# ImChouOWO/A-lightweight-Unsupervised-Feature-Extractor-

Hardware: NVIDIA B200
Metric: tracked frames/sec at N=64 boxes; ROIAlign achieved HBM GB/s vs B200 peak (higher is better)
Workload: dtype f32

## Files before the change

### a-lightweight-unsupervised-feature-extractor-_b200/csrc/app_cost_tc.cu

```cuda
#include <cuda_bf16.h>

#include "assoc_cost.cuh"

namespace b200 {
namespace {

constexpr int kRows = 128;
constexpr int kTrackRows = 32;
constexpr int kChunks = cost::kD / 8;
constexpr int kSplitBytes = kChunks * kRows * 16;
constexpr int kImageBytes = 3 * kSplitBytes;
constexpr int kLBO = kRows * 16;
constexpr int kSBO = 8 * 16;
constexpr int kTcSmem = 2 * kImageBytes + 64;

__device__ __forceinline__ void split3(float x, __nv_bfloat16* hi, __nv_bfloat16* mid, __nv_bfloat16* lo) {
    *hi = __float2bfloat16_rn(x);
    const float r1 = __fsub_rn(x, __bfloat162float(*hi));
    *mid = __float2bfloat16_rn(r1);
    const float r2 = __fsub_rn(r1, __bfloat162float(*mid));
    *lo = __float2bfloat16_rn(r2);
}

template <int RB>
__global__ void __launch_bounds__(256)
app_tc_prep_kernel(const float* __restrict__ bank, const int32_t* __restrict__ bank_len, const float* __restrict__ fallback,
                   const float* __restrict__ det, int M, int N, int T, unsigned char* __restrict__ imgA,
                   unsigned char* __restrict__ imgB, int m_tiles, int n_tiles) {
    const int lane = threadIdx.x & 31;
    const long long rowsA = (long long)m_tiles * kRows, rowsB = (long long)n_tiles * RB;
    for (long long item = (long long)blockIdx.x * 8 + (threadIdx.x >> 5); item < rowsA + rowsB; item += (long long)gridDim.x * 8) {
        float4 v = make_float4(0.0f, 0.0f, 0.0f, 0.0f);
        unsigned char* img;
        int row, tile_rows = kRows;
        if (item < rowsA) {
            const int m = (int)(item / kTrackRows), t = (int)(item % kTrackRows);
            img = imgA + (size_t)(item / kRows) * kImageBytes;
            row = (int)(item % kRows);
            if (m < M) {
                const int len = min(bank_len[m], T);
                if (t < len) v = reinterpret_cast<const float4*>(bank + ((size_t)m * T + t) * cost::kD)[lane];
                else if (len <= 0 && fallback && t == 0) v = reinterpret_cast<const float4*>(fallback + (size_t)m * cost::kD)[lane];
            }
        } else {
            const long long j = item - rowsA;
            img = imgB + (size_t)(j / RB) * (3 * kChunks * RB * 16);
            row = (int)(j % RB);
            tile_rows = RB;
            if (j < N) v = reinterpret_cast<const float4*>(det + (size_t)j * cost::kD)[lane];
        }
        v = cost::unit_row(v);
        __nv_bfloat16 h[3][4];
        split3(v.x, &h[0][0], &h[1][0], &h[2][0]);
        split3(v.y, &h[0][1], &h[1][1], &h[2][1]);
        split3(v.z, &h[0][2], &h[1][2], &h[2][2]);
        split3(v.w, &h[0][3], &h[1][3], &h[2][3]);
        unsigned char* dst = img + (size_t)(lane >> 1) * (tile_rows * 16) + (size_t)row * 16 + (lane & 1) * 8;
#pragma unroll
        for (int s = 0; s < 3; ++s)
            *reinterpret_cast<uint2*>(dst + (size_t)s * (kChunks * tile_rows * 16)) = *reinterpret_cast<const uint2*>(&h[s][0]);
    }
}

__device__ __forceinline__ unsigned smem_u32(const void* p) { return (unsigned)__cvta_generic_to_shared(p); }
__device__ __forceinline__ void tc_mbar_init(unsigned bar, unsigned count) {
    asm volatile("mbarrier.init.shared::cta.b64 [%0], %1;\n" ::"r"(bar), "r"(count) : "memory");
}
__device__ __forceinline__ void tc_mbar_expect_tx(unsigned bar, unsigned bytes) {
    asm volatile("mbarrier.arrive.expect_tx.shared::cta.b64 _, [%0], %1;\n" ::"r"(bar), "r"(bytes) : "memory");
}
__device__ __forceinline__ void tc_mbar_wait(unsigned bar, unsigned parity) {
    asm volatile(
        "{\n\t.reg .pred p;\n\t"
        "WAIT_%=:\n\t"
        "mbarrier.try_wait.parity.shared::cta.b64 p, [%0], %1;\n\t"
        "@p bra DONE_%=;\n\t"
        "bra WAIT_%=;\n\t"
        "DONE_%=:\n\t}\n" ::"r"(bar), "r"(parity) : "memory");
}
__device__ __forceinline__ void tc_bulk_load(unsigned dst, const void* src, unsigned bytes, unsigned bar) {
    asm volatile("cp.async.bulk.shared::cluster.global.mbarrier::complete_tx::bytes [%0], [%1], %2, [%3];\n"
                 ::"r"(dst), "l"(src), "r"(bytes), "r"(bar) : "memory");
}
__device__ __forceinline__ unsigned long long umma_desc(unsigned smem_addr, int lbo = kLBO) {
    return (unsigned long long)((smem_addr >> 4) & 0x3fffu) | ((unsigned long long)((lbo >> 4) & 0x3fff) << 16) |
           ((unsigned long long)((kSBO >> 4) & 0x3fff) << 32) | (1ull << 46);
}
constexpr unsigned kIdesc = (1u << 4) | (1u << 7) | (1u << 10) | ((unsigned)(kRows >> 3) << 17) | ((unsigned)(kRows >> 4) << 24);

__global__ void __launch_bounds__(128, 1)
app_tc_kernel(const unsigned char* __restrict__ imgA, const unsigned char* __restrict__ imgB,
              const int32_t* __restrict__ bank_len, int has_fallback, int M, int N, int T, int topk, int topk_mean,
              float* __restrict__ C_app, int ldc) {
    extern __shared__ __align__(128) unsigned char smem[];
    unsigned char* sA = smem;
    unsigned char* sB = smem + kImageBytes;
    const unsigned bar_load = smem_u32(smem + 2 * kImageBytes), bar_mma = bar_load + 8;
    unsigned* tmem_slot = reinterpret_cast<unsigned*>(smem + 2 * kImageBytes + 16);
    const int warp = threadIdx.x >> 5, lane = threadIdx.x & 31;
    const int tile_n = blockIdx.x, tile_m = blockIdx.y;

    if (warp == 0) {
        asm volatile("tcgen05.alloc.cta_group::1.sync.aligned.shared::cta.b32 [%0], %1;\n" ::"r"(smem_u32(tmem_slot)), "r"(128u) : "memory");
        asm volatile("tcgen05.relinquish_alloc_permit.cta_group::1.sync.aligned;\n" ::: "memory");
    }
    if (threadIdx.x == 32) {
        tc_mbar_init(bar_load, 1);
        tc_mbar_init(bar_mma, 1);
        asm volatile("fence.mbarrier_init.release.cluster;\n" ::: "memory");
    }
    asm volatile("tcgen05.fence::before_thread_sync;\n" ::: "memory");
    __syncthreads();
    asm volatile("tcgen05.fence::after_thread_sync;\n" ::: "memory");
    const unsigned tmem = *tmem_slot;

    if (threadIdx.x == 0) {
        tc_mbar_expect_tx(bar_load, 2u * kImageBytes);
        tc_bulk_load(smem_u32(sA), imgA + (size_t)tile_m * kImageBytes, kImageBytes, bar_load);
        tc_bulk_load(smem_u32(sB), imgB + (size_t)tile_n * kImageBytes, kImageBytes, bar_load);
        tc_mbar_wait(bar_load, 0);
        asm volatile("tcgen05.fence::after_thread_sync;\n" ::: "memory");
        const int pa[6] = {2, 0, 1, 1, 0, 0}, pb[6] = {0, 2, 1, 0, 1, 0};
        unsigned accumulate = 0;
#pragma unroll
        for (int p = 0; p < 6; ++p) {
            const unsigned a0 = smem_u32(sA) + pa[p] * kSplitBytes, b0 = smem_u32(sB) + pb[p] * kSplitBytes;
#pragma unroll
            for (int ks = 0; ks < kChunks / 2; ++ks) {
                const unsigned long long da = umma_desc(a0 + ks * 2 * kLBO), db = umma_desc(b0 + ks * 2 * kLBO);
                asm volatile(
                    "{\n\t.reg .pred p;\n\t"
                    "setp.ne.b32 p, %4, 0;\n\t"
                    "tcgen05.mma.cta_group::1.kind::f16 [%0], %1, %2, %3, p;\n\t}\n"
                    ::"r"(tmem), "l"(da), "l"(db), "r"(kIdesc), "r"(accumulate) : "memory");
                accumulate = 1;
            }
        }
        asm volatile("tcgen05.commit.cta_group::1.mbarrier::arrive::one.shared::cluster.b64 [%0];\n" ::"r"(bar_mma) : "memory");
    }
    __syncwarp();
    tc_mbar_wait(bar_mma, 0);
    asm volatile("tcgen05.fence::after_thread_sync;\n" ::: "memory");

    const int m = tile_m * (kRows / kTrackRows) + warp;
    int len = 0;
    if (m < M) {
        len = min(bank_len[m], T);
        if (len <= 0 && has_fallback) len = 1;
    }
    const int kk = topk_mean ? min(topk, len) : min(1, len);
    const float kNegInf = -__int_as_float(0x7f800000);
    float* tile = reinterpret_cast<float*>(smem) + warp * (32 * 33);
    for (int c0 = 0; c0 < kRows; c0 += 32) {
        unsigned r[32];
        const unsigned taddr = tmem + ((unsigned)(warp * 32) << 16) + (unsigned)c0;
        asm volatile(
            "tcgen05.ld.sync.aligned.32x32b.x32.b32"
            "{%0, %1, %2, %3, %4, %5, %6, %7, %8, %9, %10, %11, %12, %13, %14, %15,"
            " %16, %17, %18, %19, %20, %21, %22, %23, %24, %25, %26, %27, %28, %29, %30, %31}, [%32];\n"
            : "=r"(r[0]), "=r"(r[1]), "=r"(r[2]), "=r"(r[3]), "=r"(r[4]), "=r"(r[5]), "=r"(r[6]), "=r"(r[7]), "=r"(r[8]),
              "=r"(r[9]), "=r"(r[10]), "=r"(r[11]), "=r"(r[12]), "=r"(r[13]), "=r"(r[14]), "=r"(r[15]), "=r"(r[16]),
              "=r"(r[17]), "=r"(r[18]), "=r"(r[19]), "=r"(r[20]), "=r"(r[21]), "=r"(r[22]), "=r"(r[23]), "=r"(r[24]),
              "=r"(r[25]), "=r"(r[26]), "=r"(r[27]), "=r"(r[28]), "=r"(r[29]), "=r"(r[30]), "=r"(r[31])
            : "r"(taddr)
            : "memory");
        asm volatile("tcgen05.wait::ld.sync.aligned;\n" ::: "memory");
        __syncwarp();
#pragma unroll
        for (int j = 0; j < 32; ++j) tile[lane * 33 + j] = __uint_as_float(r[j]);
        __syncwarp();
        float c = 1.0f;
        if (kk > 0 && kk <= 5) {
            float t0 = kNegInf, t1 = kNegInf, t2 = kNegInf, t3 = kNegInf, t4 = kNegInf;
#pragma unroll
            for (int t = 0; t < 32; ++t) {
                float x = t < len ? tile[t * 33 + lane] : kNegInf;
                float hi;
                hi = fmaxf(t0, x); x = fminf(t0, x); t0 = hi;
                hi = fmaxf(t1, x); x = fminf(t1, x); t1 = hi;
                hi = fmaxf(t2, x); x = fminf(t2, x); t2 = hi;
                hi = fmaxf(t3, x); x = fminf(t3, x); t3 = hi;
                t4 = fmaxf(t4, x);
            }
            float sum = t0;
            if (kk > 1) sum = __fadd_rn(sum, t1);
            if (kk > 2) sum = __fadd_rn(sum, t2);
            if (kk > 3) sum = __fadd_rn(sum, t3);
            if (kk > 4) sum = __fadd_rn(sum, t4);
            c = __fsub_rn(1.0f, __fdiv_rn(sum, (float)kk));
        } else if (kk > 5) {
            unsigned taken = 0u;
            float sum = 0.0f;
            for (int q = 0; q < kk; ++q) {
                float best = kNegInf;
                int arg = 0;
                for (int t = 0; t < len; ++t) {
                    const float x = tile[t * 33 + lane];
                    if (!((taken >> t) & 1u) && x > best) { best = x; arg = t; }
                }
                taken |= 1u << arg;
                sum = __fadd_rn(sum, best);
            }
            c = __fsub_rn(1.0f, __fdiv_rn(sum, (float)kk));
        }
        const int n = tile_n * kRows + c0 + lane;
        if (m < M && n < N) C_app[(size_t)m * ldc + n] = c;
    }
    asm volatile("tcgen05.fence::before_thread_sync;\n" ::: "memory");
    __syncthreads();
    if (warp == 0) asm volatile("tcgen05.dealloc.cta_group::1.sync.aligned.b32 %0, %1;\n" ::"r"(tmem), "r"(128u) : "memory");
}

constexpr int kWalkCols = 64;
constexpr int kWalkLBO = kWalkCols * 16;
constexpr int kWalkSplitBytes = kChunks * kWalkCols * 16;
constexpr int kWalkImageBytes = 3 * kWalkSplitBytes;
constexpr int kWalkEpiWarps = 8;
constexpr int kWalkThreads = (kWalkEpiWarps + 1) * 32;
constexpr int kWalkScratch = kWalkEpiWarps * 32 * 33 * 4;
constexpr int kWalkSmem = kImageBytes + 2 * kWalkImageBytes + kWalkScratch + 96;
constexpr unsigned kIdescWalk = (1u << 4) | (1u << 7) | (1u << 10) | ((unsigned)(kWalkCols >> 3) << 17) | ((unsigned)(kRows >> 4) << 24);

__device__ __forceinline__ void tc_mbar_arrive(unsigned bar) {
    asm volatile("mbarrier.arrive.shared::cta.b64 _, [%0];\n" ::"r"(bar) : "memory");
}

__global__ void __launch_bounds__(kWalkThreads, 1)
app_tc_walk_kernel(const unsigned char* __restrict__ imgA, const unsigned char* __restrict__ imgB,
                   const int32_t* __restrict__ bank_len, int has_fallback, int M, int N, int T, int topk, int topk_mean,
                   float* __restrict__ C_app, int ldc, int n_steps) {
    extern __shared__ __align__(128) unsigned char smem[];
    unsigned char* sA = smem;
    unsigned char* sB = smem + kImageBytes;
    float* scratch = reinterpret_cast<float*>(smem + kImageBytes + 2 * kWalkImageBytes);
    const unsigned bar0 = smem_u32(smem + kImageBytes + 2 * kWalkImageBytes + kWalkScratch);
    unsigned* tmem_slot = reinterpret_cast<unsigned*>(smem + kImageBytes + 2 * kWalkImageBytes + kWalkScratch + 72);
    unsigned rank, nrank;
    asm volatile("mov.u32 %0, %%cluster_ctarank;" : "=r"(rank));
    asm volatile("mov.u32 %0, %%cluster_nctarank;" : "=r"(nrank));
    const unsigned short cta_mask = (unsigned short)((1u << nrank) - 1u);

    const int tid = threadIdx.x, warp = tid >> 5, lane = tid & 31;
    const int tile_m = blockIdx.x;
    const int first_tile = (int)((unsigned)tile_m / nrank) % n_steps;

    if (warp == 0) {
        asm volatile("tcgen05.alloc.cta_group::1.sync.aligned.shared::cta.b32 [%0], %1;\n" ::"r"(smem_u32(tmem_slot)), "r"(128u) : "memory");
        asm volatile("tcgen05.relinquish_alloc_permit.cta_group::1.sync.aligned;\n" ::: "memory");
    }
    if (tid == 32) {
        tc_mbar_init(bar0, 1);
        tc_mbar_init(bar0 + 8, 1); tc_mbar_init(bar0 + 16, 1);
        tc_mbar_init(bar0 + 24, 1); tc_mbar_init(bar0 + 32, 1);
        tc_mbar_init(bar0 + 40, kWalkEpiWarps); tc_mbar_init(bar0 + 48, kWalkEpiWarps);
        tc_mbar_init(bar0 + 56, nrank); tc_mbar_init(bar0 + 64, nrank);
        asm volatile("fence.mbarrier_init.release.cluster;\n" ::: "memory");
    }
    asm volatile("tcgen05.fence::before_thread_sync;\n" ::: "memory");
    __syncthreads();
    if (nrank > 1)
        asm volatile("barrier.cluster.arrive.release.aligned;\n\tbarrier.cluster.wait.acquire.aligned;" ::: "memory");
    asm volatile("tcgen05.fence::after_thread_sync;\n" ::: "memory");
    const unsigned tmem = *tmem_slot;

    if (warp == kWalkEpiWarps) {
        const bool leader = lane == 0;
        const unsigned tm = __shfl_sync(0xffffffffu, tmem, 0);
        auto load_b = [&](int step) {
            const int buf = step & 1;
            const int tile_n = (first_tile + step) % n_steps;
            tc_mbar_expect_tx(bar0 + 8 + 8 * buf, (unsigned)kWalkImageBytes);
            if (nrank > 1) {
                const unsigned part = (unsigned)kWalkImageBytes / nrank;
                const unsigned dst = smem_u32(sB + buf * kWalkImageBytes) + rank * part;
                const unsigned char* src = imgB + (size_t)tile_n * kWalkImageBytes + (size_t)rank * part;
                asm volatile("cp.async.bulk.shared::cluster.global.mbarrier::complete_tx::bytes.multicast::cluster [%0], [%1], %2, [%3], %4;\n"
                             ::"r"(dst), "l"(src), "r"(part), "r"(bar0 + 8 + 8 * buf), "h"(cta_mask) : "memory");
            } else {
                tc_bulk_load(smem_u32(sB + buf * kWalkImageBytes), imgB + (size_t)tile_n * kWalkImageBytes, kWalkImageBytes,
                             bar0 + 8 + 8 * buf);
            }
        };
        if (leader) {
            tc_mbar_expect_tx(bar0, (unsigned)kImageBytes);
            tc_bulk_load(smem_u32(sA), imgA + (size_t)tile_m * kImageBytes, kImageBytes, bar0);
            load_b(0);
            if (n_steps > 1) load_b(1);
        }
        __syncwarp();
        tc_mbar_wait(bar0, 0);
        const unsigned long long dA = umma_desc(smem_u32(sA));
        for (int step = 0; step < n_steps; ++step) {
            const int buf = step & 1;
            const unsigned use = (unsigned)((step >> 1) & 1);
            if (step >= 2) tc_mbar_wait(bar0 + 40 + 8 * buf, use ^ 1u);
            tc_mbar_wait(bar0 + 8 + 8 * buf, use);
            asm volatile("tcgen05.fence::after_thread_sync;\n" ::: "memory");
            const int pa[6] = {2, 0, 1, 1, 0, 0}, pb[6] = {0, 2, 1, 0, 1, 0};
            const unsigned acc = tm + (unsigned)(buf * kWalkCols);
            const unsigned long long dB = umma_desc(smem_u32(sB + buf * kWalkImageBytes), kWalkLBO);
            if (leader) {
                unsigned accumulate = 0;
#pragma unroll
                for (int p = 0; p < 6; ++p) {
#pragma unroll
                    for (int ks = 0; ks < kChunks / 2; ++ks) {
                        const unsigned long long da = dA + (unsigned long long)((pa[p] * kSplitBytes + ks * 2 * kLBO) >> 4);
                        const unsigned long long db = dB + (unsigned long long)((pb[p] * kWalkSplitBytes + ks * 2 * kWalkLBO) >> 4);
                        asm volatile(
                            "{\n\t.reg .pred p;\n\t"
                            "setp.ne.b32 p, %4, 0;\n\t"
                            "tcgen05.mma.cta_group::1.kind::f16 [%0], %1, %2, %3, p;\n\t}\n"
                            ::"r"(acc), "l"(da), "l"(db), "r"(kIdescWalk), "r"(accumulate) : "memory");
                        accumulate = 1;
                    }
                }
                asm volatile("tcgen05.commit.cta_group::1.mbarrier::arrive::one.shared::cluster.b64 [%0];\n"
                             ::"r"(bar0 + 24 + 8 * buf) : "memory");
                if (nrank > 1)
                    asm volatile("tcgen05.commit.cta_group::1.mbarrier::arrive::one.shared::cluster.multicast::cluster.b64 [%0], %1;\n"
                                 ::"r"(bar0 + 56 + 8 * buf), "h"(cta_mask) : "memory");
            }
            __syncwarp();
            if (step >= 1 && step + 1 < n_steps) {
                if (nrank > 1) tc_mbar_wait(bar0 + 56 + 8 * (buf ^ 1), (unsigned)(((step - 1) >> 1) & 1));
                else tc_mbar_wait(bar0 + 24 + 8 * (buf ^ 1), (unsigned)(((step - 1) >> 1) & 1));
                if (leader) load_b(step + 1);
                __syncwarp();
            }
        }
    } else {
        const int q = warp & 3, half = warp >> 2;
        const int m = tile_m * (kRows / kTrackRows) + q;
        int len = 0;
        if (m < M) {
            len = min(bank_len[m], T);
            if (len <= 0 && has_fallback) len = 1;
        }
        const int kk = topk_mean ? min(topk, len) : min(1, len);
        const float kNegInf = -__int_as_float(0x7f800000);
        float* tile = scratch + warp * (32 * 33);
        for (int step = 0; step < n_steps; ++step) {
            const int buf = step & 1;
            tc_mbar_wait(bar0 + 24 + 8 * buf, (unsigned)((step >> 1) & 1));
            asm volatile("tcgen05.fence::after_thread_sync;\n" ::: "memory");
            unsigned r[32];
            const unsigned taddr = tmem + ((unsigned)(q * 32) << 16) + (unsigned)(buf * kWalkCols + half * 32);
            asm volatile(
                "tcgen05.ld.sync.aligned.32x32b.x32.b32"
                "{%0, %1, %2, %3, %4, %5, %6, %7, %8, %9, %10, %11, %12, %13, %14, %15,"
                " %16, %17, %18, %19, %20, %21, %22, %23, %24, %25, %26, %27, %28, %29, %30, %31}, [%32];\n"
                : "=r"(r[0]), "=r"(r[1]), "=r"(r[2]), "=r"(r[3]), "=r"(r[4]), "=r"(r[5]), "=r"(r[6]), "=r"(r[7]), "=r"(r[8]),
                  "=r"(r[9]), "=r"(r[10]), "=r"(r[11]), "=r"(r[12]), "=r"(r[13]), "=r"(r[14]), "=r"(r[15]), "=r"(r[16]),
                  "=r"(r[17]), "=r"(r[18]), "=r"(r[19]), "=r"(r[20]), "=r"(r[21]), "=r"(r[22]), "=r"(r[23]), "=r"(r[24]),
                  "=r"(r[25]), "=r"(r[26]), "=r"(r[27]), "=r"(r[28]), "=r"(r[29]), "=r"(r[30]), "=r"(r[31])
                : "r"(taddr)
                : "memory");
            asm volatile("tcgen05.wait::ld.sync.aligned;\n" ::: "memory");
            asm volatile("tcgen05.fence::before_thread_sync;\n" ::: "memory");
            __syncwarp();
            if (lane == 0) tc_mbar_arrive(bar0 + 40 + 8 * buf);
#pragma unroll
            for (int j = 0; j < 32; ++j) tile[lane * 33 + j] = __uint_as_float(r[j]);
            __syncwarp();
            float c = 1.0f;
            if (kk > 0 && kk <= 5) {
                float t0 = kNegInf, t1 = kNegInf, t2 = kNegInf, t3 = kNegInf, t4 = kNegInf;
#pragma unroll
                for (int t = 0; t < 32; ++t) {
                    float x = t < len ? tile[t * 33 + lane] : kNegInf;
                    float hi;
                    hi = fmaxf(t0, x); x = fminf(t0, x); t0 = hi;
                    hi = fmaxf(t1, x); x = fminf(t1, x); t1 = hi;
                    hi = fmaxf(t2, x); x = fminf(t2, x); t2 = hi;
                    hi = fmaxf(t3, x); x = fminf(t3, x); t3 = hi;
                    t4 = fmaxf(t4, x);
                }
                float sum = t0;
                if (kk > 1) sum = __fadd_rn(sum, t1);
                if (kk > 2) sum = __fadd_rn(sum, t2);
                if (kk > 3) sum = __fadd_rn(sum, t3);
                if (kk > 4) sum = __fadd_rn(sum, t4);
                c = __fsub_rn(1.0f, __fdiv_rn(sum, (float)kk));
            } else if (kk > 5) {
                unsigned taken = 0u;
                float sum = 0.0f;
                for (int qq = 0; qq < kk; ++qq) {
                    float best = kNegInf;
                    int arg = 0;
                    for (int t = 0; t < len; ++t) {
                        const float x = tile[t * 33 + lane];
                        if (!((taken >> t) & 1u) && x > best) { best = x; arg = t; }
                    }
                    taken |= 1u << arg;
                    sum = __fadd_rn(sum, best);
                }
                c = __fsub_rn(1.0f, __fdiv_rn(sum, (float)kk));
            }
            const int n = ((first_tile + step) % n_steps) * kWalkCols + half * 32 + lane;
            if (m < M && n < N) C_app[(size_t)m * ldc + n] = c;
        }
    }
    asm volatile("tcgen05.fence::before_thread_sync;\n" ::: "memory");
    __syncthreads();
    if (nrank > 1)
        asm volatile("barrier.cluster.arrive.release.aligned;\n\tbarrier.cluster.wait.acquire.aligned;" ::: "memory");
    if (warp == 0) asm volatile("tcgen05.dealloc.cta_group::1.sync.aligned.b32 %0, %1;\n" ::"r"(tmem), "r"(128u) : "memory");
}

}

int app_cost_tc(const float* bank, const int32_t* bank_len, const float* fallback, const float* det, int M, int N, int T,
                int topk, int use_topk_mean, float* C_app, int ldc, cudaStream_t st) {
    if (T > kTrackRows || (long long)M * N < 64 * 64) return 1;
    static bool configured[64];
    int dev = 0;
    if (cudaGetDevice(&dev) != cudaSuccess || dev < 0 || dev >= 64) dev = 0;
    if (!configured[dev]) {
        B200_CUDA(cudaFuncSetAttribute(app_tc_kernel, cudaFuncAttributeMaxDynamicSharedMemorySize, kTcSmem));
        B200_CUDA(cudaFuncSetAttribute(app_tc_walk_kernel, cudaFuncAttributeMaxDynamicSharedMemorySize, kWalkSmem));
        configured[dev] = true;
    }
    const int m_tiles = (M * kTrackRows + kRows - 1) / kRows;
    bool walk = m_tiles >= 100;
    if (const char* e = getenv("B200TRACK_TC_KERNEL")) walk = atoi(e) == 2;
    const int rb = walk ? kWalkCols : kRows;
    const int n_tiles = (N + rb - 1) / rb;
    const size_t imgB_bytes = (size_t)n_tiles * (walk ? kWalkImageBytes : kImageBytes);
    cudaMemPool_t pool = nullptr;
    int rc = scratch_pool(&pool);
    if (rc) return rc;
    unsigned char* img = nullptr;
    B200_CUDA(cudaMallocFromPoolAsync(reinterpret_cast<void**>(&img), (size_t)m_tiles * kImageBytes + imgB_bytes, pool, st));
    unsigned char* imgA = img;
    unsigned char* imgB = img + (size_t)m_tiles * kImageBytes;
    const long long rows = (long long)m_tiles * kRows + (long long)n_tiles * rb;
    const unsigned blocks = (unsigned)((rows + 7) / 8 < 148 * 8 ? (rows + 7) / 8 : 148 * 8);
    if (walk) app_tc_prep_kernel<kWalkCols><<<blocks, 256, 0, st>>>(bank, bank_len, fallback, det, M, N, T, imgA, imgB, m_tiles, n_tiles);
    else app_tc_prep_kernel<kRows><<<blocks, 256, 0, st>>>(bank, bank_len, fallback, det, M, N, T, imgA, imgB, m_tiles, n_tiles);
    rc = check_launch("app_tc_prep_kernel");
    if (rc == B200_OK) {
        if (walk) {
            int cl = 1;
            if (const char* e = getenv("B200TRACK_TC_CLUSTER")) cl = (atoi(e) == 2 && m_tiles % 2 == 0) ? 2 : 1;
            cudaLaunchConfig_t cfg = {};
            cfg.gridDim = dim3((unsigned)m_tiles);
            cfg.blockDim = dim3(kWalkThreads);
            cfg.dynamicSmemBytes = kWalkSmem;
            cfg.stream = st;
            cudaLaunchAttribute attr[1];
            attr[0].id = cudaLaunchAttributeClusterDimension;
            attr[0].val.clusterDim.x = cl; attr[0].val.clusterDim.y = 1; attr[0].val.clusterDim.z = 1;
            cfg.attrs = attr;
            cfg.numAttrs = 1;
            (void)cudaLaunchKernelEx(&cfg, app_tc_walk_kernel, (const unsigned char*)imgA, (const unsigned char*)imgB, bank_len,
                                     (int)(fallback != nullptr), M, N, T, topk, use_topk_mean, C_app, ldc, n_tiles);
            rc = check_launch("app_tc_walk_kernel");
        } else {
            app_tc_kernel<<<dim3(n_tiles, m_tiles), 128, kTcSmem, st>>>(imgA, imgB, bank_len, fallback != nullptr, M, N, T, topk,
                                                                       use_topk_mean, C_app, ldc);
            rc = check_launch("app_tc_kernel");
        }
    }
    B200_CUDA(cudaFreeAsync(img, st));
    return rc;
}

}
```

### a-lightweight-unsupervised-feature-extractor-_b200/csrc/common.cuh

```cuda
#pragma once
#include <cuda_runtime.h>
#include <stdint.h>
#include <stdio.h>

#include <atomic>

#include "b200track.h"

namespace b200 {

extern thread_local char g_err[512];
extern std::atomic<int64_t> g_launches;

int fail(int code, const char* fmt, ...);
int scratch_pool(cudaMemPool_t* out);

inline int check_launch(const char* what) {
    g_launches.fetch_add(1, std::memory_order_relaxed);
    cudaError_t e = cudaGetLastError();
    if (e != cudaSuccess) return fail(B200_ECUDA, "%s: %s", what, cudaGetErrorString(e));
    return B200_OK;
}

#define B200_CUDA(expr)                                                                  \
    do {                                                                                 \
        cudaError_t _e = (expr);                                                         \
        if (_e != cudaSuccess)                                                           \
            return ::b200::fail(B200_ECUDA, "%s: %s", #expr, cudaGetErrorString(_e));    \
    } while (0)

#define B200_REQUIRE(cond, ...)                                                          \
    do {                                                                                 \
        if (!(cond)) return ::b200::fail(B200_EINVAL, __VA_ARGS__);                      \
    } while (0)

inline cudaStream_t as_stream(void* s) { return reinterpret_cast<cudaStream_t>(s); }

constexpr int kWarp = 32;
constexpr int kSMs = 148;

__device__ __forceinline__ float warp_sum(float v) {
#pragma unroll
    for (int o = 16; o > 0; o >>= 1) v += __shfl_xor_sync(0xffffffffu, v, o);
    return v;
}
__device__ __forceinline__ int warp_min(int v) {
#pragma unroll
    for (int o = 16; o > 0; o >>= 1) v = min(v, __shfl_xor_sync(0xffffffffu, v, o));
    return v;
}
__device__ __forceinline__ int warp_max(int v) {
#pragma unroll
    for (int o = 16; o > 0; o >>= 1) v = max(v, __shfl_xor_sync(0xffffffffu, v, o));
    return v;
}


#ifdef B200_TRK_TIMING
static __device__ unsigned long long g_span[128];
__device__ __forceinline__ unsigned long long gtime() {
    unsigned long long t;
    asm volatile("mov.u64 %0, %%globaltimer;" : "=l"(t));
    return t;
}
#define B200_SPAN_BEGIN(k) do { if (threadIdx.x == 0) atomicMin(&::b200::g_span[2 * (k)], ::b200::gtime()); } while (0)
#define B200_SPAN_END(k) do { if (threadIdx.x == 0) atomicMax(&::b200::g_span[2 * (k) + 1], ::b200::gtime()); } while (0)
#define B200_SPAN_GETTER(name)                                                                          \
    extern "C" int name(unsigned long long* out64, int reset) {                                         \
        if (out64 && cudaMemcpyFromSymbol(out64, ::b200::g_span, sizeof(unsigned long long) * 128) != cudaSuccess) return -2; \
        if (reset) {                                                                                    \
            unsigned long long init[128];                                                                \
            for (int i = 0; i < 128; ++i) init[i] = (i & 1) ? 0ull : ~0ull;                              \
            if (cudaMemcpyToSymbol(::b200::g_span, init, sizeof(init)) != cudaSuccess) return -2;       \
        }                                                                                               \
        return 0;                                                                                       \
    }
#else
#define B200_SPAN_GETTER(name)
#define B200_SPAN_BEGIN(k) do { } while (0)
#define B200_SPAN_END(k) do { } while (0)
#endif

}
```

### a-lightweight-unsupervised-feature-extractor-_b200/csrc/kalman.cuh

```cuda
#pragma once
#include "common.cuh"

namespace b200 {
namespace kf {

__device__ __forceinline__ void box_to_z(const double* b, float* z) {
    const double w = fmax(1.0, b[2] - b[0]), h = fmax(1.0, b[3] - b[1]);
    z[0] = (float)(b[0] + 0.5 * w);
    z[1] = (float)(b[1] + 0.5 * h);
    z[2] = (float)(w / h);
    z[3] = (float)h;
}

__device__ __forceinline__ void x_to_box(const double* x, double* b) {
    const double h = fmax(x[3], 1.0), a = fmax(x[2], 1e-3), w = fmax(a * h, 1.0);
    b[0] = x[0] - 0.5 * w;
    b[1] = x[1] - 0.5 * h;
    b[2] = x[0] + 0.5 * w;
    b[3] = x[1] + 0.5 * h;
}

__device__ __forceinline__ void init_state(const double* box, double* x, double* P) {
    float z[4];
    box_to_z(box, z);
#pragma unroll
    for (int i = 0; i < 4; ++i) { x[i] = (double)z[i]; x[i + 4] = 0.0; }
#pragma unroll
    for (int i = 0; i < 64; ++i) P[i] = 0.0;
#pragma unroll
    for (int i = 0; i < 4; ++i) { P[i * 9] = 10.0; P[(i + 4) * 9] = 1000.0; }
}

template <typename TX, typename TP>
__device__ __forceinline__ void predict_t(double* x, double* P, const float* q) {
#pragma unroll
    for (int i = 0; i < 4; ++i) x[i] = (double)((TX)x[i] + (TX)x[i + 4]);
#pragma unroll
    for (int i = 0; i < 4; ++i)
#pragma unroll
        for (int j = 0; j < 8; ++j) P[i * 8 + j] = (double)((TP)P[i * 8 + j] + (TP)P[(i + 4) * 8 + j]);
#pragma unroll
    for (int i = 0; i < 8; ++i)
#pragma unroll
        for (int j = 0; j < 4; ++j) P[i * 8 + j] = (double)((TP)P[i * 8 + j] + (TP)P[i * 8 + j + 4]);
#pragma unroll
    for (int i = 0; i < 8; ++i) P[i * 9] = (double)((TP)P[i * 9] + (TP)q[i]);
}

__device__ __forceinline__ void predict(double* x, double* P, int stage, const float* q) {
    if (stage == 0) predict_t<float, float>(x, P, q);
    else if (stage == 1) predict_t<float, double>(x, P, q);
    else predict_t<double, double>(x, P, q);
}

template <typename T>
__device__ __forceinline__ void inv4(const T* S, T* SI) {
    T a[4][4], b[4][4], rinv[4];
#pragma unroll
    for (int i = 0; i < 4; ++i)
#pragma unroll
        for (int j = 0; j < 4; ++j) { a[i][j] = S[i * 4 + j]; b[i][j] = (i == j) ? (T)1 : (T)0; }
#pragma unroll
    for (int j = 0; j < 4; ++j) {
        int p = j;
        T best = fabs(a[j][j]);
#pragma unroll
        for (int i = j + 1; i < 4; ++i) {
            const T v = fabs(a[i][j]);
            if (v > best) { best = v; p = i; }
        }
#pragma unroll
        for (int i = j + 1; i < 4; ++i)
            if (p == i) {
#pragma unroll
                for (int k = 0; k < 4; ++k) {
                    T t = a[j][k]; a[j][k] = a[i][k]; a[i][k] = t;
                    t = b[j][k]; b[j][k] = b[i][k]; b[i][k] = t;
                }
            }
        rinv[j] = (T)1 / a[j][j];
#pragma unroll
        for (int i = j + 1; i < 4; ++i) {
            a[i][j] *= rinv[j];
#pragma unroll
            for (int k = j + 1; k < 4; ++k) a[i][k] -= a[i][j] * a[j][k];
        }
    }
#pragma unroll
    for (int c = 0; c < 4; ++c) {
#pragma unroll
        for (int i = 1; i < 4; ++i)
#pragma unroll
            for (int k = 0; k < i; ++k) b[i][c] -= a[i][k] * b[k][c];
#pragma unroll
        for (int i = 3; i >= 0; --i) {
#pragma unroll
            for (int k = i + 1; k < 4; ++k) b[i][c] -= a[i][k] * b[k][c];
            b[i][c] *= rinv[i];
        }
    }
#pragma unroll
    for (int i = 0; i < 4; ++i)
#pragma unroll
        for (int j = 0; j < 4; ++j) SI[i * 4 + j] = b[i][j];
}

template <typename A, typename B> struct Promote { using type = double; };
template <> struct Promote<float, float> { using type = float; };

template <typename TX, typename TP>
__device__ __forceinline__ void update_t(double* x, double* P, const float* z, const float* r) {
    using TXN = typename Promote<TX, TP>::type;
    TX y[4];
#pragma unroll
    for (int i = 0; i < 4; ++i) y[i] = (TX)z[i] - (TX)x[i];
    TP S[16], SI[16], K[32];
#pragma unroll
    for (int i = 0; i < 4; ++i)
#pragma unroll
        for (int j = 0; j < 4; ++j) S[i * 4 + j] = (TP)P[i * 8 + j] + (i == j ? (TP)r[i] : (TP)0);
    inv4<TP>(S, SI);
#pragma unroll
    for (int i = 0; i < 8; ++i)
#pragma unroll
        for (int j = 0; j < 4; ++j) {
            TP s = (TP)P[i * 8] * SI[j];
#pragma unroll
            for (int k = 1; k < 4; ++k) s = fma((TP)P[i * 8 + k], SI[k * 4 + j], s);
            K[i * 4 + j] = s;
        }
#pragma unroll
    for (int i = 0; i < 8; ++i) {
        TXN s = (TXN)K[i * 4] * (TXN)y[0];
#pragma unroll
        for (int k = 1; k < 4; ++k) s = fma((TXN)K[i * 4 + k], (TXN)y[k], s);
        x[i] = (double)((TXN)(TX)x[i] + s);
    }
    double ikd[4];
#pragma unroll
    for (int i = 0; i < 4; ++i) ikd[i] = 1.0 - (double)K[i * 4 + i];
#define B200_IK(i, k) ((i) == (k) ? ikd[(k)] : -(double)K[(i) * 4 + (k)])
#pragma unroll
    for (int i = 4; i < 8; ++i)
#pragma unroll
        for (int j = 0; j < 8; ++j) {
            double s = B200_IK(i, 0) * P[j];
#pragma unroll
            for (int k = 1; k < 4; ++k) s = fma(B200_IK(i, k), P[k * 8 + j], s);
            P[i * 8 + j] = s + P[i * 8 + j];
        }
#pragma unroll
    for (int j = 0; j < 8; ++j) {
        const double p0 = P[j], p1 = P[8 + j], p2 = P[16 + j], p3 = P[24 + j];
#pragma unroll
        for (int i = 0; i < 4; ++i)
            P[i * 8 + j] = fma(B200_IK(i, 3), p3, fma(B200_IK(i, 2), p2, fma(B200_IK(i, 1), p1, B200_IK(i, 0) * p0)));
    }
#pragma unroll
    for (int i = 0; i < 8; ++i) {
        const double a0 = P[i * 8], a1 = P[i * 8 + 1], a2 = P[i * 8 + 2], a3 = P[i * 8 + 3];
#pragma unroll
        for (int j = 0; j < 8; ++j) {
            const double s = fma(a3, B200_IK(j, 3), fma(a2, B200_IK(j, 2), fma(a1, B200_IK(j, 1), a0 * B200_IK(j, 0))));
            TP d = (K[i * 4] * (TP)r[0]) * K[j * 4];
#pragma unroll
            for (int k = 1; k < 4; ++k) d = fma(K[i * 4 + k] * (TP)r[k], K[j * 4 + k], d);
            P[i * 8 + j] = (j < 4 ? s : s + P[i * 8 + j]) + (double)d;
        }
    }
#undef B200_IK
}

__device__ __forceinline__ int update(double* x, double* P, int stage, const float* z, const float* r) {
    if (stage == 0) update_t<float, float>(x, P, z, r);
    else if (stage == 1) update_t<float, double>(x, P, z, r);
    else update_t<double, double>(x, P, z, r);
    return stage < 2 ? stage + 1 : 2;
}

struct Gate {
    double SI[16];
    double xs[4];
    int stage;
};

__device__ __forceinline__ void gate_prepare(const double* x, const double* P, int stage, const float* r,
                                             Gate* g) {
    g->stage = stage;
#pragma unroll
    for (int i = 0; i < 4; ++i) g->xs[i] = x[i];
    if (stage == 0) {
        float S[16], SI[16];
#pragma unroll
        for (int i = 0; i < 4; ++i)
#pragma unroll
            for (int j = 0; j < 4; ++j) {
                const float hph = (float)P[i * 8 + j] + (i == j ? r[i] : 0.0f);
                S[i * 4 + j] = hph + (i == j ? 1e-9f : 0.0f);
            }
        inv4<float>(S, SI);
#pragma unroll
        for (int i = 0; i < 16; ++i) g->SI[i] = (double)SI[i];
    } else {
        double S[16];
#pragma unroll
        for (int i = 0; i < 4; ++i)
#pragma unroll
            for (int j = 0; j < 4; ++j) {
                const double hph = P[i * 8 + j] + (i == j ? (double)r[i] : 0.0);
                S[i * 4 + j] = hph + (i == j ? (double)1e-9f : 0.0);
            }
        inv4<double>(S, g->SI);
    }
}

__device__ __forceinline__ double gate_d2(const double* SI, const double* xs, int stage, const float* z) {
    if (stage == 0) {
        float y[4], t[4];
#pragma unroll
        for (int i = 0; i < 4; ++i) y[i] = z[i] - (float)xs[i];
#pragma unroll
        for (int j = 0; j < 4; ++j) {
            float s = y[0] * (float)SI[j];
#pragma unroll
            for (int i = 1; i < 4; ++i) s = fmaf(y[i], (float)SI[i * 4 + j], s);
            t[j] = s;
        }
        float d = t[0] * y[0];
#pragma unroll
        for (int j = 1; j < 4; ++j) d = fmaf(t[j], y[j], d);
        return (double)d;
    }
    double y[4], t[4];
#pragma unroll
    for (int i = 0; i < 4; ++i)
        y[i] = stage == 1 ? (double)(z[i] - (float)xs[i]) : (double)z[i] - xs[i];
#pragma unroll
    for (int j = 0; j < 4; ++j) {
        double s = y[0] * SI[j];
#pragma unroll
        for (int i = 1; i < 4; ++i) s = fma(y[i], SI[i * 4 + j], s);
        t[j] = s;
    }
    double d = t[0] * y[0];
#pragma unroll
    for (int j = 1; j < 4; ++j) d = fma(t[j], y[j], d);
    return d;
}

template <typename TX, typename TP>
__device__ __forceinline__ double update_rows_t(double* gx, double* gP, const float* z, const float* r, double* sP,
                                                double* sK, int i, unsigned mask, int new_stage, bool want_d2) {
    using TXN = typename Promote<TX, TP>::type;
    double Pr[8];
    {
        const double2* p2 = reinterpret_cast<const double2*>(gP + i * 8);
#pragma unroll
        for (int k = 0; k < 4; ++k) { const double2 v = p2[k]; Pr[2 * k] = v.x; Pr[2 * k + 1] = v.y; }
    }
#pragma unroll
    for (int j = 0; j < 8; ++j) sP[i * 8 + j] = Pr[j];
    double xg[4];
#pragma unroll
    for (int k = 0; k < 4; ++k) xg[k] = gx[k];
    const double xi = gx[i];
    __syncwarp(mask);
    TP S[16], SI[16], Kr[4];
#pragma unroll
    for (int a = 0; a < 4; ++a)
#pragma unroll
        for (int b = 0; b < 4; ++b) S[a * 4 + b] = (TP)sP[a * 8 + b] + (a == b ? (TP)r[a] : (TP)0);
    inv4<TP>(S, SI);
#pragma unroll
    for (int j = 0; j < 4; ++j) {
        TP acc = (TP)Pr[0] * SI[j];
#pragma unroll
        for (int k = 1; k < 4; ++k) acc = fma((TP)Pr[k], SI[k * 4 + j], acc);
        Kr[j] = acc;
    }
    TX y[4];
#pragma unroll
    for (int k = 0; k < 4; ++k) y[k] = (TX)z[k] - (TX)xg[k];
    TXN sx = (TXN)Kr[0] * (TXN)y[0];
#pragma unroll
    for (int k = 1; k < 4; ++k) sx = fma((TXN)Kr[k], (TXN)y[k], sx);
    const double xn = (double)((TXN)(TX)xi + sx);
#pragma unroll
    for (int j = 0; j < 4; ++j) sK[i * 4 + j] = (double)Kr[j];
    __syncwarp(mask);
    gx[i] = xn;
    double ik[4], A[8];
#pragma unroll
    for (int k = 0; k < 4; ++k) ik[k] = (i == k) ? 1.0 - (double)Kr[k] : -(double)Kr[k];
#pragma unroll
    for (int j = 0; j < 8; ++j) {
        double a = ik[0] * sP[j];
#pragma unroll
        for (int k = 1; k < 4; ++k) a = fma(ik[k], sP[k * 8 + j], a);
        A[j] = i >= 4 ? a + Pr[j] : a;
    }
    double Pn[8];
#pragma unroll
    for (int j = 0; j < 8; ++j) {
        double ikj[4];
#pragma unroll
        for (int k = 0; k < 4; ++k) ikj[k] = (j == k) ? 1.0 - sK[j * 4 + k] : -sK[j * 4 + k];
        const double b = fma(A[3], ikj[3], fma(A[2], ikj[2], fma(A[1], ikj[1], A[0] * ikj[0])));
        TP dd = (Kr[0] * (TP)r[0]) * (TP)sK[j * 4];
#pragma unroll
        for (int k = 1; k < 4; ++k) dd = fma(Kr[k] * (TP)r[k], (TP)sK[j * 4 + k], dd);
        Pn[j] = (j < 4 ? b : b + A[j]) + (double)dd;
    }
    {
        double2* p2 = reinterpret_cast<double2*>(gP + i * 8);
#pragma unroll
        for (int k = 0; k < 4; ++k) p2[k] = make_double2(Pn[2 * k], Pn[2 * k + 1]);
    }
    if (!want_d2) return 0.0;
    __syncwarp(mask);
    if (i < 4) {
#pragma unroll
        for (int j = 0; j < 4; ++j) sP[i * 8 + j] = Pn[j];
        sK[i] = xn;
    }
    __syncwarp(mask);
    Gate g;
    double x4[4];
#pragma unroll
    for (int k = 0; k < 4; ++k) x4[k] = sK[k];
    gate_prepare(x4, sP, new_stage, r, &g);
    return gate_d2(g.SI, g.xs, new_stage, z);
}

}
}
```

### a-lightweight-unsupervised-feature-extractor-_b200/csrc/roi_align.cu

```cuda
#include <cuda.h>
#include <cuda_fp16.h>

#include "common.cuh"
#include <type_traits>

namespace b200 {
namespace {

#ifndef B200_ROI_WARPS
#define B200_ROI_WARPS 2
#endif
constexpr int kWarpsPerCta = B200_ROI_WARPS;
constexpr int kFootCap = 8;
constexpr int kCellCap = kFootCap * kFootCap;

template <typename T> __device__ __forceinline__ float ldf(const T* p);
template <> __device__ __forceinline__ float ldf<float>(const float* p) { return __ldg(p); }
template <> __device__ __forceinline__ float ldf<__half>(const __half* p) { return __half2float(__ldg(p)); }
__device__ __forceinline__ float to_f32(float v) { return v; }
__device__ __forceinline__ float to_f32(__half v) { return __half2float(v); }
template <typename T> __device__ __forceinline__ T from_f(float v);
template <> __device__ __forceinline__ float from_f<float>(float v) { return v; }
template <> __device__ __forceinline__ __half from_f<__half>(float v) { return __float2half_rn(v); }

// ... 421 lines not shown
    }
}

template <int PH, int PW, bool NHWC, typename T, bool PREP, bool OCL>
__global__ void __launch_bounds__(kWarpsPerCta * 32, (B200_ROI_MIN_CTAS * 2 + kWarpsPerCta - 1) / kWarpsPerCta)
roi_align_tile_kernel(const T* __restrict__ feat, int B, int C, int H, int W,
                      const float* __restrict__ rois, long long K, float scale, int sr, int aligned,
                      T* __restrict__ out, int ctiles, const RoiPrep* __restrict__ prep,
                      const float* __restrict__ prep_tabs) {
    using L = TileSmem<PH, PW>;
    extern __shared__ __align__(16) float smem[];
    const int warp = threadIdx.x >> 5, lane = threadIdx.x & 31;
    const long long wi = (long long)blockIdx.x * kWarpsPerCta + warp;
    if (wi >= K * ctiles) return;
    const int span_slot = (int)((reinterpret_cast<uintptr_t>(rois) / (size_t)(K * 20)) & 7);
    B200_SPAN_BEGIN(span_slot);
    float* sMain = smem + (size_t)warp * L::kFloatsPerWarp;
    const unsigned wi32 = (unsigned)wi;
    const long long k = wi32 / (unsigned)ctiles;
    const int c0 = (int)(wi32 % (unsigned)ctiles) * 32;
    process_tile<PH, PW, NHWC, T, PREP, OCL>(feat, B, C, H, W, rois, scale, sr, aligned, out, k, c0, min(32, C - c0),
                                             prep, prep_tabs, sMain, sMain + L::kMainFloats, lane);
    B200_SPAN_END(span_slot);
}

#ifndef B200_ROI_MULTI_TILES
#define B200_ROI_MULTI_TILES 8
#endif
template <int PH, int PW, bool NHWC, typename T, bool OCL>
__global__ void __launch_bounds__(kWarpsPerCta * 32, (B200_ROI_MIN_CTAS * 2 + kWarpsPerCta - 1) / kWarpsPerCta)
roi_align_multi_kernel(const T* __restrict__ feat, int B, int C, int H, int W, const float* __restrict__ rois,
                       long long K, float scale, int sr, int aligned, T* __restrict__ out, int ctiles,
                       const RoiPrep* __restrict__ prep, const float* __restrict__ prep_tabs, int group_warps,
                       int tiles_per_warp) {
    using L = TileSmem<PH, PW>;
    extern __shared__ __align__(16) float smem[];
    const int warp = threadIdx.x >> 5, lane = threadIdx.x & 31;
    const unsigned gw = blockIdx.x * kWarpsPerCta + warp, grp = gw / (unsigned)group_warps;
    const unsigned stride = (unsigned)group_warps, window = stride * (unsigned)tiles_per_warp;
    unsigned t = grp * window + (gw - grp * stride);
    const unsigned total = (unsigned)min((long long)(grp + 1) * window, K * ctiles);
    if (t >= total) return;
    asm volatile("griddepcontrol.wait;" ::: "memory");
    const int span_slot = (int)((reinterpret_cast<uintptr_t>(rois) / (size_t)(K * 20)) & 7);
    B200_SPAN_BEGIN(span_slot);
    float* sMain = smem + (size_t)warp * L::kFloatsPerWarp;
    unsigned k = t / (unsigned)ctiles;
    int4 h0 = reinterpret_cast<const int4*>(prep + k)[0], h1 = reinterpret_cast<const int4*>(prep + k)[1];
    bool pending = false;
    for (;;) {
        const unsigned tn = t + stride;
        const bool have_next = tn < total;
        unsigned kn = 0;
        int4 n0 = make_int4(0, 0, 0, 0), n1 = n0;
        if (have_next) {
            kn = tn / (unsigned)ctiles;
            n0 = reinterpret_cast<const int4*>(prep + kn)[0];
            n1 = reinterpret_cast<const int4*>(prep + kn)[1];
        }
        const int c0 = (int)(t - k * (unsigned)ctiles) * 32;
        process_tile<PH, PW, NHWC, T, true, OCL, true>(feat, B, C, H, W, rois, scale, sr, aligned, out, (long long)k, c0,
                                                       min(32, C - c0), prep, prep_tabs, sMain, sMain + L::kMainFloats,
                                                       lane, h0, h1, &pending);
        if (!have_next) break;
        t = tn; k = kn; h0 = n0; h1 = n1;
    }
    if (pending && lane == 0) bulk_store_wait_read();
    B200_SPAN_END(span_slot);
}

constexpr int kPipeWarps = 2;
#ifndef B200_ROI_PIPE_TILES
#define B200_ROI_PIPE_TILES 8
#endif
constexpr int kPipeTilesPerWarp = B200_ROI_PIPE_TILES;

template <int PH, int PW>
struct PipeSmem {
    using L = TileSmem<PH, PW>;
    static constexpr int kBufFloats = kCellCap * 32 + L::kTabFloats;
    static constexpr int kFloatsPerWarp = 2 * kBufFloats;
    static constexpr int kBytesPerCta = kFloatsPerWarp * 4 * kPipeWarps;
    static_assert(kFloatsPerWarp >= L::kFloatsPerWarp, "the fallback path needs an output tile + tables");
};

template <int PH, int PW, typename T>
__device__ __forceinline__ void pipe_issue(const T* __restrict__ feat, int C, int H, int W, const int4 h0,
                                           const int4 h1, long long k, int c0, int cn, bool vec16,
                                           const float* __restrict__ prep_tabs, unsigned sv, int lane) {
    using L = TileSmem<PH, PW>;
    constexpr int kEs = (int)sizeof(T), kLpc = 32 * kEs / 16, kCpi = 32 / kLpc;
    const int b = h0.x, ymin = h0.y, xmin = h0.z, FY = h0.w, FX = h1.x;
    const float* tsrc = prep_tabs + (size_t)k * L::kTabFloats;
    for (int i = lane; i < L::kTabFloats / 4; i += 32) cp_async16_s(sv + 4u * (kCellCap * 32) + 16u * i, tsrc + 4 * i);
    const int cells = FY * FX;
    if (vec16 && cn == 32) {
        int m = lane / kLpc, x = m, r = 0;
        while (x >= FX && r < FY) { x -= FX; ++r; }
        const T* src = feat + (((size_t)b * H + ymin + r) * W + xmin + x) * C + c0 + (lane % kLpc) * (16 / kEs);
        const size_t step = (size_t)kCpi * C, wrap = (size_t)(W - FX) * C;
        unsigned dst = sv + (unsigned)(32 * kEs) * m + 16u * (lane % kLpc);
        for (; m < cells; m += kCpi, dst += (unsigned)(32 * kEs * kCpi)) {
            cp_async16_s(dst, src);
            x += kCpi;
            src += step;
            while (x >= FX) { x -= FX; src += wrap; }
        }
    } else if (kEs == 4 && lane < cn) {
        const T* row = feat + (((size_t)b * H + ymin) * W + xmin) * C + c0 + lane;
        unsigned dst = sv + 4u * lane;
        for (int r = 0; r < FY; ++r, row += (size_t)W * C) {
            const T* src = row;
#pragma unroll 4
            for (int x = 0; x < FX; ++x, src += C, dst += 128) cp_async4_s(dst, src);
        }
    }
}

template <typename T>
__device__ __forceinline__ bool pipe_can_stage(const int4 rec1, bool vec16, int cn) {
    return rec1.y != 0 && (sizeof(T) == 4 || (vec16 && cn == 32));
}

template <int PH, int PW, bool OCL, typename T>
__global__ void __launch_bounds__(kPipeWarps * 32, (B200_ROI_MIN_CTAS * 2 + kPipeWarps - 1) / kPipeWarps)
roi_align_pipe_kernel(const T* __restrict__ feat, int B, int C, int H, int W, const float* __restrict__ rois,
                      long long K, float scale, int sr, int aligned, T* __restrict__ out, int ctiles,
                      const RoiPrep* __restrict__ prep, const float* __restrict__ prep_tabs, int group_warps,
                      int tiles_per_warp) {
    using L = TileSmem<PH, PW>;
    using P = PipeSmem<PH, PW>;
    constexpr int PHP = L::kPHP, NB = PH * PW, kEs = (int)sizeof(T);
    static_assert(OCL || (NB * kEs) % (kEs == 4 ? 16 : 4) == 0, "vector stores of a lane's output row");
    extern __shared__ __align__(16) float smem[];
    const int warp = threadIdx.x >> 5, lane = threadIdx.x & 31;
    float* base = smem + (size_t)warp * P::kFloatsPerWarp;
    const unsigned sbase = (unsigned)__cvta_generic_to_shared(base);
    const unsigned gw = blockIdx.x * kPipeWarps + warp, grp = gw / (unsigned)group_warps;
    const unsigned stride = (unsigned)group_warps, window = stride * (unsigned)tiles_per_warp;
    unsigned t = grp * window + (gw - grp * stride);
    const unsigned total = (unsigned)min((long long)(grp + 1) * window, K * ctiles);
    if (t >= total) return;
    asm volatile("griddepcontrol.wait;" ::: "memory");
    const int span_slot = (int)((reinterpret_cast<uintptr_t>(rois) / (size_t)(K * 20)) & 7);
    B200_SPAN_BEGIN(span_slot);

    unsigned ka = t / (unsigned)ctiles;
    int ca = (int)(t - ka * (unsigned)ctiles) * 32;
    int4 a0 = reinterpret_cast<const int4*>(prep + ka)[0], a1 = reinterpret_cast<const int4*>(prep + ka)[1];
    const bool vec16 = ((C * kEs) & 15) == 0 && (reinterpret_cast<uintptr_t>(feat) & 15) == 0;
    if (pipe_can_stage<T>(a1, vec16, min(32, C - ca)))
        pipe_issue<PH, PW, T>(feat, C, H, W, a0, a1, ka, ca, min(32, C - ca), vec16, prep_tabs, sbase, lane);
    asm volatile("cp.async.commit_group;\n" ::: "memory");
    unsigned tn = t + stride, kn = 0;
    int cnx = 0;
    int4 n0 = make_int4(0, 0, 0, 0), n1 = n0;
    if (tn < total) {
        kn = tn / (unsigned)ctiles;
        cnx = (int)(tn - kn * (unsigned)ctiles) * 32;
        n0 = reinterpret_cast<const int4*>(prep + kn)[0];
        n1 = reinterpret_cast<const int4*>(prep + kn)[1];
    }
    int par = 0;
    for (;;) {
        const bool have_next = tn < total;
        const int cn = min(32, C - ca);
        if (!pipe_can_stage<T>(a1, vec16, cn)) {
            process_tile<PH, PW, true, T, false, OCL>(feat, B, C, H, W, rois, scale, sr, aligned, out, (long long)ka,
                                                      ca, cn, nullptr, nullptr, base, base + L::kMainFloats, lane);
            __syncwarp();
        }
        if (have_next && pipe_can_stage<T>(n1, vec16, min(32, C - cnx)))
            pipe_issue<PH, PW, T>(feat, C, H, W, n0, n1, kn, cnx, min(32, C - cnx), vec16, prep_tabs,
                                  sbase + 4u * (unsigned)((par ^ 1) * P::kBufFloats), lane);
        asm volatile("cp.async.commit_group;\n" ::: "memory");
        const unsigned tm = tn + stride;
        unsigned km = 0;
        int cm = 0;
        int4 m0 = make_int4(0, 0, 0, 0), m1 = m0;
        auto load_after_next = [&]() {
            if (have_next && tm < total) {
                km = tm / (unsigned)ctiles;
                cm = (int)(tm - km * (unsigned)ctiles) * 32;
                m0 = reinterpret_cast<const int4*>(prep + km)[0];
                m1 = reinterpret_cast<const int4*>(prep + km)[1];
            }
        };
        if (pipe_can_stage<T>(a1, vec16, cn)) {
            asm volatile("cp.async.wait_group 1;\n" ::: "memory");
            __syncwarp();
            const T* sV = reinterpret_cast<const T*>(base + par * P::kBufFloats);
            const float* sWy = base + par * P::kBufFloats + kCellCap * 32;
            const int FY = a0.w, FX = a1.x;
            float acc[PH][PW];
#pragma unroll
            for (int a = 0; a < PH; ++a)
#pragma unroll
                for (int bq = 0; bq < PW; ++bq) acc[a][bq] = 0.0f;
            separable_accumulate<PH, PW>(acc, sWy, sWy + kFootCap * PHP, FY, FX, [&](int r, int x) {
                return to_f32(sV[(r * FX + x) * 32 + lane]);
            });
            load_after_next();
            if (OCL) {
                T* gl = out + (size_t)ka * NB * C + ca + lane;
                if (lane < cn) {
#pragma unroll
                    for (int a = 0; a < PH; ++a)
#pragma unroll
                        for (int bq = 0; bq < PW; ++bq) gl[(size_t)(a * PW + bq) * C] = from_f<T>(acc[a][bq]);
                }
            }
            __syncwarp();
            T* so = reinterpret_cast<T*>(base + par * P::kBufFloats);
#pragma unroll
            for (int h = 0; h < (OCL ? 0 : 2); ++h) {
                if ((lane >> 4) == h) {
                    if (kEs == 4) {
                        float4* row = reinterpret_cast<float4*>(so + (lane & 15) * NB);
#pragma unroll
                        for (int q = 0; q < NB / 4; ++q)
                            row[q] = make_float4(acc[(4 * q) / PW][(4 * q) % PW], acc[(4 * q + 1) / PW][(4 * q + 1) % PW],
                                                 acc[(4 * q + 2) / PW][(4 * q + 2) % PW],
                                                 acc[(4 * q + 3) / PW][(4 * q + 3) % PW]);
                    } else {
                        __half2* row = reinterpret_cast<__half2*>(so + (lane & 15) * NB);
#pragma unroll
                        for (int q = 0; q < NB / 2; ++q)
                            row[q] = __floats2half2_rn(acc[(2 * q) / PW][(2 * q) % PW], acc[(2 * q + 1) / PW][(2 * q + 1) % PW]);
                    }
                }
                __syncwarp();
                const int nch = min(16, cn - 16 * h);
                float4* g4 = reinterpret_cast<float4*>(out + ((size_t)ka * C + ca + 16 * h) * NB);
                const float4* s4 = reinterpret_cast<const float4*>(so);
                if (nch == 16) {
                    constexpr int kN4 = 16 * NB * kEs / 16, kIt = (kN4 + 31) / 32;
#pragma unroll
                    for (int i0 = 0; i0 < kIt; i0 += 4) {
                        float4 v[4];
#pragma unroll
                        for (int u = 0; u < 4; ++u)
                            if (i0 + u < kIt && (32 * (i0 + u + 1) <= kN4 || lane + 32 * (i0 + u) < kN4))
                                v[u] = s4[lane + 32 * (i0 + u)];
#pragma unroll
                        for (int u = 0; u < 4; ++u)
                            if (i0 + u < kIt && (32 * (i0 + u + 1) <= kN4 || lane + 32 * (i0 + u) < kN4))
                                __stcs(g4 + lane + 32 * (i0 + u), v[u]);
                    }
                } else {
                    for (int i = lane; i < nch * NB * kEs / 16; i += 32) __stcs(g4 + i, s4[i]);
                }
                __syncwarp();
            }
            __syncwarp();
        } else {
            load_after_next();
        }
        if (!have_next) break;
        t = tn; ka = kn; ca = cnx; a0 = n0; a1 = n1;
        tn = tm; kn = km; cnx = cm; n0 = m0; n1 = m1;
        par ^= 1;
    }
    B200_SPAN_END(span_slot);
}


constexpr int kTmaRows = 5;
constexpr int kTmaCols = 8;
constexpr int kTmaRowBytes = kTmaCols * 4 * 32;
constexpr int kTmaVRows = 10;
constexpr int kTmaVBytes = kTmaVRows * kTmaRowBytes;
struct TmaMaps {
    CUtensorMap m[3];
};
__device__ __forceinline__ int tma_box_rows(int rows) { return rows <= 1 ? 1 : rows <= 3 ? 3 : 5; }
#ifndef B200_ROI_TMA_WARPS
#define B200_ROI_TMA_WARPS 2
#endif
#ifndef B200_ROI_TMA_CTAS
#define B200_ROI_TMA_CTAS 3
#endif
#ifndef B200_ROI_TMA_TILES
#define B200_ROI_TMA_TILES 16
#endif
#ifndef B200_ROI_TMA_REGS
#define B200_ROI_TMA_REGS 216
#endif
#ifndef B200_ROI_TMA_MAX_CTAS
#define B200_ROI_TMA_MAX_CTAS 0
#endif
constexpr int kTmaWarps = B200_ROI_TMA_WARPS;

template <int PH, int PW>
struct TmaSmem {
    using L = TileSmem<PH, PW>;
    static constexpr int kTabBytes = L::kTabFloats * 4;
    static constexpr int kOutBytes = L::kMainFloats * 4;
    static constexpr int kOffTab = kTmaVBytes, kOffOut = kOffTab + 2 * kTabBytes, kOffBar = kOffOut + kOutBytes;
    static constexpr int kBytesPerWarp = (kOffBar + 16 + 127) & ~127;
    static constexpr int kBytesPerCta = kBytesPerWarp * kTmaWarps;
    static_assert(kTabBytes % 16 == 0 && kOffOut % 16 == 0 && kOffBar % 8 == 0, "bulk-copy alignment");
};

__device__ __forceinline__ void mbar_init(unsigned bar, unsigned count) {
    asm volatile("mbarrier.init.shared::cta.b64 [%0], %1;\n" ::"r"(bar), "r"(count) : "memory");
}
__device__ __forceinline__ void mbar_expect_tx(unsigned bar, unsigned bytes) {
    asm volatile("mbarrier.arrive.expect_tx.shared::cta.b64 _, [%0], %1;\n" ::"r"(bar), "r"(bytes) : "memory");
}
__device__ __forceinline__ void mbar_wait(unsigned bar, unsigned parity) {
    asm volatile(
        "{\n\t.reg .pred p;\n\t"
        "WAIT_%=:\n\t"
        "mbarrier.try_wait.parity.shared::cta.b64 p, [%0], %1;\n\t"
        "@p bra DONE_%=;\n\t"
        "bra WAIT_%=;\n\t"
        "DONE_%=:\n\t}\n" ::"r"(bar), "r"(parity) : "memory");
}
__device__ __forceinline__ void tma_box_4d(unsigned dst, const CUtensorMap* tm, int x, int y, int c, int b, unsigned bar) {
#if B200_ROI_L2_HINT >= 2
    asm volatile("cp.async.bulk.tensor.4d.shared::cluster.global.tile.mbarrier::complete_tx::bytes.L2::cache_hint [%0], [%1, {%2, %3, %4, %5}], [%6], %7;\n"
                 ::"r"(dst), "l"(tm), "r"(x), "r"(y), "r"(c), "r"(b), "r"(bar), "l"(l2_evict_first_policy()) : "memory");
#else
    asm volatile("cp.async.bulk.tensor.4d.shared::cluster.global.tile.mbarrier::complete_tx::bytes [%0], [%1, {%2, %3, %4, %5}], [%6];\n"
                 ::"r"(dst), "l"(tm), "r"(x), "r"(y), "r"(c), "r"(b), "r"(bar) : "memory");
#endif
}
__device__ __forceinline__ void bulk_load(unsigned dst, const void* src, unsigned bytes, unsigned bar) {
    asm volatile("cp.async.bulk.shared::cluster.global.mbarrier::complete_tx::bytes [%0], [%1], %2, [%3];\n"
                 ::"r"(dst), "l"(src), "r"(bytes), "r"(bar) : "memory");
}

__device__ __forceinline__ int tma_tile_rows(const int4 h0, const int4 h1) {
    const int FY = h0.w, FX = h1.x;
    if (FY == 0 || FX == 0) return 0;
    return FY > kTmaRows ? kTmaRows + tma_box_rows(FY - kTmaRows) : tma_box_rows(FY);
}

__device__ __forceinline__ bool elect_one() {
    unsigned p;
    asm volatile("{\n\t.reg .pred P;\n\telect.sync _|P, 0xffffffff;\n\tselp.u32 %0, 1, 0, P;\n\t}\n" : "=r"(p)::"memory");
    return p != 0;
}
__device__ __forceinline__ int bcast0(int v) { return __shfl_sync(0xffffffffu, v, 0); }

template <int PH, int PW, typename T>
__device__ __forceinline__ void tma_issue(const TmaMaps* tm, const int4 h0, const int4 h1, unsigned k, int c0,
                                          const float* __restrict__ prep_tabs, unsigned sv, unsigned stab, unsigned bar) {
    using S = TmaSmem<PH, PW>;
    const int b = bcast0(h0.x), ymin = bcast0(h0.y), xmin = bcast0(h0.z), FY = bcast0(h0.w), FX = bcast0(h1.x);
    const unsigned ku = (unsigned)bcast0((int)k);
    const int cu = bcast0(c0);
    const unsigned svu = (unsigned)bcast0((int)sv), stabu = (unsigned)bcast0((int)stab), baru = (unsigned)bcast0((int)bar);
    const bool any = FY != 0 && FX != 0;
    const int r0 = FY > kTmaRows ? kTmaRows : tma_box_rows(FY);
    const int r1 = FY > kTmaRows ? tma_box_rows(FY - kTmaRows) : 0;
    if (elect_one()) {
#ifdef B200_ROI_TMA_NOLOAD
        mbar_expect_tx(baru, (unsigned)S::kTabBytes);
        bulk_load(stabu, prep_tabs + (size_t)ku * S::L::kTabFloats, S::kTabBytes, baru);
        if (false) {
#else
        mbar_expect_tx(baru, (unsigned)(S::kTabBytes + (any ? (r0 + r1) * kTmaRowBytes : 0)));
        bulk_load(stabu, prep_tabs + (size_t)ku * S::L::kTabFloats, S::kTabBytes, baru);
        if (any) {
#endif
            tma_box_4d(svu, &tm->m[r0 >> 1], xmin, ymin, cu, b, baru);
            if (r1) tma_box_4d(svu + kTmaRows * kTmaRowBytes, &tm->m[r1 >> 1], xmin, ymin + kTmaRows, cu, b, baru);
        }
    }
    __syncwarp();
}

template <int PH, int PW, typename T>
__device__ __forceinline__ void tma_accumulate(float (&acc)[PH][PW], const unsigned char* sV, const float* sWy,
                                               const float* sWx, int FY, int FX, int xmask, int lane) {
    static_assert(sizeof(T) == 4, "float32 maps only");
    constexpr int PHP = (PH + 3) & ~3, PWP = (PW + 3) & ~3;
    const int nrb = FY > kTmaRows ? 2 : 1, ncb = FX > 4 ? 2 : 1;
    for (int rb = 0; rb < nrb; ++rb) {
        const int rows = FY - rb * kTmaRows;
        const int brow = rb ? tma_box_rows(rows) : (nrb == 2 ? kTmaRows : tma_box_rows(rows));
        const unsigned char* mine = sV + rb * (kTmaRows * kTmaRowBytes) + lane * (brow * 32);
        const float* wy0 = sWy + rb * kTmaRows * PHP;
        for (int cb = 0; cb < ncb; ++cb) {
            float v[kTmaRows][4];
#pragma unroll
            for (int i = 0; i < kTmaRows; ++i) {
                float4 q = make_float4(0.0f, 0.0f, 0.0f, 0.0f);
                if (i < rows) q = *reinterpret_cast<const float4*>(mine + i * 32 + cb * 16);
                v[i][0] = q.x; v[i][1] = q.y; v[i][2] = q.z; v[i][3] = q.w;
            }
            const int bits = (xmask >> (4 * cb)) & 15;
#pragma unroll
            for (int xi = 0; xi < 4; ++xi) {
                if ((bits >> xi) & 1) {
                    float ty[PH];
#pragma unroll
                    for (int a = 0; a < PH; ++a) ty[a] = 0.0f;
#pragma unroll
                    for (int i = 0; i < kTmaRows; ++i) {
                        const int r = (rb * kTmaRows + i < kFootCap) ? i : 0;
                        const float4* w4 = reinterpret_cast<const float4*>(wy0 + r * PHP);
#pragma unroll
                        for (int q = 0; q < PHP / 4; ++q) {
                            const float4 w = w4[q];
                            if (4 * q + 0 < PH) ty[4 * q + 0] = fmaf(w.x, v[i][xi], ty[4 * q + 0]);
                            if (4 * q + 1 < PH) ty[4 * q + 1] = fmaf(w.y, v[i][xi], ty[4 * q + 1]);
                            if (4 * q + 2 < PH) ty[4 * q + 2] = fmaf(w.z, v[i][xi], ty[4 * q + 2]);
                            if (4 * q + 3 < PH) ty[4 * q + 3] = fmaf(w.w, v[i][xi], ty[4 * q + 3]);
                        }
                    }
                    const float4* w4 = reinterpret_cast<const float4*>(sWx + (4 * cb + xi) * PWP);
#pragma unroll
                    for (int q = 0; q < PWP / 4; ++q) {
                        const float4 w = w4[q];
                        const float wv[4] = {w.x, w.y, w.z, w.w};
#pragma unroll
                        for (int e = 0; e < 4; ++e)
                            if (4 * q + e < PW) {
#pragma unroll
                                for (int a2 = 0; a2 < PH; ++a2) acc[a2][4 * q + e] = fmaf(wv[e], ty[a2], acc[a2][4 * q + e]);
                            }
                    }
                }
            }
        }
    }
}

template <int PH, int PW, typename T, bool OCL>
__global__ void __maxnreg__(B200_ROI_TMA_REGS)
roi_align_tma_kernel(const __grid_constant__ TmaMaps tmap, const T* __restrict__ feat, int B, int C, int H, int W,
                     const float* __restrict__ rois, long long K, float scale, int sr, int aligned, T* __restrict__ out,
                     int ctiles, const RoiPrep* __restrict__ prep, const float* __restrict__ prep_tabs, int group_warps,
                     int tiles_per_warp) {
    using L = TileSmem<PH, PW>;
    using S = TmaSmem<PH, PW>;
    constexpr int PHP = L::kPHP, NB = PH * PW;
    extern __shared__ __align__(128) unsigned char smem_tma[];
    const int warp = __shfl_sync(0xffffffffu, (int)(threadIdx.x >> 5), 0), lane = threadIdx.x & 31;
    unsigned char* base = smem_tma + (size_t)warp * S::kBytesPerWarp;
    const unsigned sbase = (unsigned)__cvta_generic_to_shared(base);
    const unsigned sbar = sbase + S::kOffBar;
    float* sOut = reinterpret_cast<float*>(base + S::kOffOut);
    const unsigned gw = blockIdx.x * kTmaWarps + warp, grp = gw / (unsigned)group_warps;
    const unsigned stride = (unsigned)group_warps, window = stride * (unsigned)tiles_per_warp;
    unsigned t = grp * window + (gw - grp * stride);
    const unsigned total = (unsigned)min((long long)(grp + 1) * window, K * ctiles);
    if (t >= total) return;
    asm volatile("griddepcontrol.wait;" ::: "memory");
    const int span_slot = (int)((reinterpret_cast<uintptr_t>(rois) / (size_t)(K * 20)) & 7);
    B200_SPAN_BEGIN(span_slot);
    if (lane == 0) {
        mbar_init(sbar, 1);
        mbar_init(sbar + 8, 1);
        asm volatile("fence.mbarrier_init.release.cluster;\n" ::: "memory");
    }
    __syncwarp();

    unsigned ka = t / (unsigned)ctiles;
    int ca = (int)(t - ka * (unsigned)ctiles) * 32;
    int4 a0 = reinterpret_cast<const int4*>(prep + ka)[0], a1 = reinterpret_cast<const int4*>(prep + ka)[1];
    unsigned tn = t + stride, kn = 0;
    int cnx = 0;
    int4 n0 = make_int4(0, 0, 0, 0), n1 = n0;
    if (tn < total) {
        kn = tn / (unsigned)ctiles;
        cnx = (int)(tn - kn * (unsigned)ctiles) * 32;
        n0 = reinterpret_cast<const int4*>(prep + kn)[0];
        n1 = reinterpret_cast<const int4*>(prep + kn)[1];
    }
    int par = 0;
    unsigned phase = 0;
    bool pending = false;
    bool cur_issued = false;
    auto v_off = [&](int p, int nr) { return p ? (unsigned)(kTmaVBytes - nr * kTmaRowBytes) : 0u; };
    if (a1.y) {
        tma_issue<PH, PW, T>(&tmap, a0, a1, ka, ca, prep_tabs, sbase + v_off(0, tma_tile_rows(a0, a1)),
                             sbase + S::kOffTab, sbar);
        cur_issued = true;
    }
    for (;;) {
        const bool have_next = tn < total;
        const int cn = min(32, C - ca);
        const int nba = a1.y ? tma_tile_rows(a0, a1) : 0;
        const int nbn = (have_next && n1.y) ? tma_tile_rows(n0, n1) : 0;
        bool next_issued = false;
        if (have_next && n1.y && nba + nbn <= kTmaVRows) {
            tma_issue<PH, PW, T>(&tmap, n0, n1, kn, cnx, prep_tabs, sbase + v_off(par ^ 1, nbn),
                                 sbase + S::kOffTab + (par ^ 1) * S::kTabBytes, sbar + 8 * (par ^ 1));
            next_issued = true;
        }
        const unsigned tm = tn + stride;
        unsigned km = 0;
        int cm = 0;
        int4 m0 = make_int4(0, 0, 0, 0), m1 = m0;
        auto load_after_next = [&]() {
            if (have_next && tm < total) {
                km = tm / (unsigned)ctiles;
                cm = (int)(tm - km * (unsigned)ctiles) * 32;
                m0 = reinterpret_cast<const int4*>(prep + km)[0];
                m1 = reinterpret_cast<const int4*>(prep + km)[1];
            }
        };
        if (a1.y) {
            if (!cur_issued) {
                tma_issue<PH, PW, T>(&tmap, a0, a1, ka, ca, prep_tabs, sbase + v_off(par, nba),
                                     sbase + S::kOffTab + par * S::kTabBytes, sbar + 8 * par);
            }
            mbar_wait(sbar + 8 * par, (phase >> par) & 1u);
            phase ^= 1u << par;
            const float* sWy = reinterpret_cast<const float*>(base + S::kOffTab + par * S::kTabBytes);
            const int FY = a0.w, FX = a1.x;
            float acc[PH][PW];
#pragma unroll
            for (int a = 0; a < PH; ++a)
#pragma unroll
                for (int bq = 0; bq < PW; ++bq) acc[a][bq] = 0.0f;
            if (nba) tma_accumulate<PH, PW, T>(acc, base + v_off(par, nba), sWy, sWy + kFootCap * PHP, FY, FX, a1.z, lane);
            load_after_next();
            __syncwarp();
            if (have_next && n1.y && !next_issued && nbn <= kTmaVRows) {
                tma_issue<PH, PW, T>(&tmap, n0, n1, kn, cnx, prep_tabs, sbase + v_off(par ^ 1, nbn),
                                     sbase + S::kOffTab + (par ^ 1) * S::kTabBytes, sbar + 8 * (par ^ 1));
                next_issued = true;
            }
            if (OCL) {
                T* gl = out + (size_t)ka * NB * C + ca + lane;
                if (lane < cn) {
#pragma unroll
                    for (int a = 0; a < PH; ++a)
#pragma unroll
                        for (int bq = 0; bq < PW; ++bq) gl[(size_t)(a * PW + bq) * C] = from_f<T>(acc[a][bq]);
                }
            } else {
                if (pending && lane == 0) bulk_store_wait_read();
                pending = false;
                __syncwarp();
                if (sizeof(T) == 4) {
                    float* myrow = sOut + lane * NB;
                    if ((NB & 3) == 0) {
#pragma unroll
                        for (int q = 0; q < NB / 4; ++q)
                            reinterpret_cast<float4*>(myrow)[q] =
                                make_float4(acc[(4 * q) / PW][(4 * q) % PW], acc[(4 * q + 1) / PW][(4 * q + 1) % PW],
                                            acc[(4 * q + 2) / PW][(4 * q + 2) % PW], acc[(4 * q + 3) / PW][(4 * q + 3) % PW]);
                    } else {
#pragma unroll
                        for (int i = 0; i < NB; ++i) myrow[i] = acc[i / PW][i % PW];
                    }
                } else {
                    __half* myrow = reinterpret_cast<__half*>(sOut) + lane * NB;
                    if ((NB & 1) == 0) {
#pragma unroll
                        for (int q = 0; q < NB / 2; ++q)
                            reinterpret_cast<__half2*>(myrow)[q] = __floats2half2_rn(acc[(2 * q) / PW][(2 * q) % PW],
                                                                                     acc[(2 * q + 1) / PW][(2 * q + 1) % PW]);
                    } else {
#pragma unroll
                        for (int i = 0; i < NB; ++i) myrow[i] = __float2half_rn(acc[i / PW][i % PW]);
                    }
                }
                T* gdst = out + ((size_t)ka * C + ca) * NB;
                const unsigned bytes = (unsigned)cn * NB * (unsigned)sizeof(T);
                if (((reinterpret_cast<uintptr_t>(gdst) & 15) == 0) && (bytes & 15u) == 0) {
                    asm volatile("fence.proxy.async.shared::cta;\n" ::: "memory");
                    __syncwarp();
                    if (lane == 0) bulk_store_issue(gdst, sOut, bytes);
                    pending = true;
                } else {
                    __syncwarp();
                    const T* tile = reinterpret_cast<const T*>(sOut);
                    for (int i = lane; i < cn * NB; i += 32) gdst[i] = tile[i];
                    __syncwarp();
                }
            }
        } else {
            process_tile<PH, PW, false, T, true, OCL, true>(feat, B, C, H, W, rois, scale, sr, aligned, out, (long long)ka, ca,
                                                            cn, prep, prep_tabs, sOut,
                                                            reinterpret_cast<float*>(base + S::kOffTab + par * S::kTabBytes),
                                                            lane, a0, a1, &pending);
            load_after_next();
            __syncwarp();
            if (have_next && n1.y && !next_issued && nbn <= kTmaVRows) {
                tma_issue<PH, PW, T>(&tmap, n0, n1, kn, cnx, prep_tabs, sbase + v_off(par ^ 1, nbn),
                                     sbase + S::kOffTab + (par ^ 1) * S::kTabBytes, sbar + 8 * (par ^ 1));
                next_issued = true;
            }
        }
        if (!have_next) break;
        t = tn; ka = kn; ca = cnx; a0 = n0; a1 = n1;
        tn = tm; kn = km; cnx = cm; n0 = m0; n1 = m1;
        cur_issued = next_issued;
        par ^= 1;
    }
    if (pending && lane == 0) bulk_store_wait_read();
    B200_SPAN_END(span_slot);
}

template <bool NHWC, typename T>
__global__ void __launch_bounds__(256)
roi_align_generic_kernel(const T* __restrict__ feat, int B, int C, int H, int W,
                         const float* __restrict__ rois, long long total, int PH, int PW, float scale,
                         int sr, int aligned, T* __restrict__ out, int out_cl) {
    for (long long idx = (long long)blockIdx.x * blockDim.x + threadIdx.x; idx < total;
         idx += (long long)gridDim.x * blockDim.x) {
        int pw, ph, c;
        if (out_cl) {
            c = (int)(idx % C); pw = (int)((idx / C) % PW); ph = (int)((idx / ((long long)C * PW)) % PH);
        } else {
            pw = (int)(idx % PW); ph = (int)((idx / PW) % PH); c = (int)((idx / ((long long)PW * PH)) % C);
        }
        const long long k = idx / ((long long)PW * PH * C);
        const Geom g = roi_geometry(rois + 5 * k, scale, sr, aligned, PH, PW);
        float s = 0.0f;
        if (g.b >= 0 && g.b < B) {
            const size_t ps = NHWC ? (size_t)C : 1;
            const T* base = feat + (NHWC ? (size_t)g.b * H * W * C + c : ((size_t)g.b * C + c) * H * W);
            for (int iy = 0; iy < g.gh; ++iy) {
                const Tap ty = make_tap(sample_pos(g.sh, ph, g.bh, iy, g.gh), H);
                for (int ix = 0; ix < g.gw; ++ix) {
                    const Tap tx = make_tap(sample_pos(g.sw, pw, g.bw, ix, g.gw), W);
                    if (ty.valid && tx.valid) {
                        const float v1 = ldf<T>(base + ((size_t)ty.lo * W + tx.lo) * ps);
                        const float v2 = ldf<T>(base + ((size_t)ty.lo * W + tx.hi) * ps);
                        const float v3 = ldf<T>(base + ((size_t)ty.hi * W + tx.lo) * ps);
                        const float v4 = ldf<T>(base + ((size_t)ty.hi * W + tx.hi) * ps);
                        s += ty.wlo * tx.wlo * v1 + ty.wlo * tx.whi * v2 + ty.whi * tx.wlo * v3 +
                             ty.whi * tx.whi * v4;
                    }
                }
            }
// ... 313 lines not shown
```

### a-lightweight-unsupervised-feature-extractor-_b200/csrc/tracker.cu

```cuda
#include <stdlib.h>
#include <string.h>

#include <new>

#include "assoc_cost.cuh"
#include "kalman.cuh"
#include "lsap.cuh"

namespace b200 {
namespace trk {

struct Span {
    int k;
    __device__ explicit Span(int kk) : k(kk) { B200_SPAN_BEGIN(k); }
    __device__ ~Span() { B200_SPAN_END(k); }
};

#ifdef B200_TRK_TIMING
__device__ long long g_timing[32];
#define TRK_STAMP(k) do { __syncthreads(); if (threadIdx.x == 0 && blockIdx.x == 0) g_timing[k] = clock64(); } while (0)
#define TRK_GSTAMP(k) do { __syncthreads(); if (threadIdx.x == 0 && blockIdx.x == 0 && blockIdx.y == 0) g_timing[16 + (k)] = (long long)::b200::gtime(); } while (0)
#else
#define TRK_STAMP(k) do { } while (0)
#define TRK_GSTAMP(k) do { } while (0)
#endif

#define TRK_PDL_PROLOGUE()                                        \
    do {                                                          \
        asm volatile("griddepcontrol.launch_dependents;");        \
        asm volatile("griddepcontrol.wait;" ::: "memory");        \
    } while (0)

constexpr int kThreads = 256;
constexpr int kHdr = 8;
enum { H_NLIVE = 0, H_NEXT = 1, H_NFREE = 2 };
enum { C_M1 = 0, C_M2 = 1, C_NU = 2, C_MODE = 3, C_NMATCH = 4, C_NUT = 5, C_STATUS = 6 };
enum { MODE_SKIP = 0, MODE_EMPTY = 1, MODE_NORMAL = 2, MODE_FAILED = 3 };
enum { R_NMATCH = 0, R_NUT = 1, R_NUD = 2, R_NLIVE = 3, R_NEXT = 4, R_STATUS = 5, R_M1 = 6, R_M2 = 7, R_HDR = 8 };

struct Dev {
    int S, MT, MD, HIST, res_stride;
    double *kf_x, *kf_P, *last_bbox, *last_conf, *last_cost;
    uint8_t* kf_stage;
    float *ema, *bank;
    int *bank_len, *bank_head, *tid, *miss, *age, *last_frame, *order, *free_list, *hdr;
    float *det_unit, *det_z, *det_boxf, *det_conff, *prev_boxf, *prev_conff, *C1, *C1T, *C2, *C2T;
    double* gate_SI;
    int* row_fc;
    float* row_fv;
    int *rows_main, *rows_reid, *cnt, *ud1, *det_used, *m_row, *m_det, *m_app, *tmp;
    int* born;
    int2 *work1, *work2;
    int* wcount;
    int *upd_slot, *upd_det;
    float* upd_cost;
    uint8_t* upd_flag;
    cost::PairWeights pw;
    double maha_thr, cost_max, conf_update_min, cost_update_max, reid_only_cost_max, init_conf_min;
    float ema_a, ema_b;
    int topk, max_age, lost_reid_after;
    const int* n_det;
    const double *boxes, *confs;
    const float* embs;
    const int* frame_id;
    int* result;
};

__device__ __forceinline__ int* res_matches(const Dev& d, int* res) { return res + R_HDR; }
__device__ __forceinline__ int* res_ut(const Dev& d, int* res) { return res + R_HDR + 2 * d.MD; }
__device__ __forceinline__ int* res_ud(const Dev& d, int* res) { return res + R_HDR + 2 * d.MD + d.MT; }

template <typename Pred, typename Emit>
__device__ inline int block_compact(int n, Pred pred, Emit emit, int* scratch) {
    int base = 0;
    const int lane = threadIdx.x & 31, w = threadIdx.x >> 5, nw = blockDim.x >> 5;
    for (int i0 = 0; i0 < n; i0 += blockDim.x) {
        const int i = i0 + threadIdx.x;
        const bool p = i < n && pred(i);
        const unsigned m = __ballot_sync(0xffffffffu, p);
        if (lane == 0) scratch[w] = __popc(m);
        __syncthreads();
        int off = 0, tot = 0;
        for (int k = 0; k < nw; ++k) {
            const int c = scratch[k];
            if (k < w) off += c;
            tot += c;
        }
        if (p) emit(base + off + __popc(m & ((1u << lane) - 1u)), i);
        base += tot;
        __syncthreads();
    }
    return base;
}

__device__ __forceinline__ void load_kf(const Dev& d, size_t slot, double* x, double* P) {
    const double2* px = reinterpret_cast<const double2*>(d.kf_x + slot * 8);
    const double2* pP = reinterpret_cast<const double2*>(d.kf_P + slot * 64);
#pragma unroll
    for (int k = 0; k < 4; ++k) { const double2 v = px[k]; x[2 * k] = v.x; x[2 * k + 1] = v.y; }
#pragma unroll
    for (int k = 0; k < 32; ++k) { const double2 v = pP[k]; P[2 * k] = v.x; P[2 * k + 1] = v.y; }
}
__device__ __forceinline__ void store_kf(const Dev& d, size_t slot, const double* x, const double* P) {
    double2* px = reinterpret_cast<double2*>(d.kf_x + slot * 8);
    double2* pP = reinterpret_cast<double2*>(d.kf_P + slot * 64);
#pragma unroll
    for (int k = 0; k < 4; ++k) px[k] = make_double2(x[2 * k], x[2 * k + 1]);
#pragma unroll
    for (int k = 0; k < 32; ++k) pP[k] = make_double2(P[2 * k], P[2 * k + 1]);
}

__device__ inline void purge(const Dev& d, int s, int nl, int* scratch) {
    int* order = d.order + (size_t)s * d.MT;
    int* tmp = d.tmp + (size_t)s * d.MT;
    int* fl = d.free_list + (size_t)s * d.MT;
    int* hdr = d.hdr + s * kHdr;
    const size_t sb = (size_t)s * d.MT;
    for (int i = threadIdx.x; i < nl; i += blockDim.x) tmp[i] = order[i];
    __syncthreads();
    const int nfree = hdr[H_NFREE];
    const int keep = block_compact(nl, [&](int i) { return d.miss[sb + tmp[i]] <= d.max_age; },
                                   [&](int pos, int i) { order[pos] = tmp[i]; }, scratch);
    const int dead = block_compact(nl, [&](int i) { return d.miss[sb + tmp[i]] > d.max_age; },
                                   [&](int pos, int i) { fl[nfree + pos] = tmp[i]; }, scratch);
    if (threadIdx.x == 0) { hdr[H_NLIVE] = keep; hdr[H_NFREE] = nfree + dead; }
    __syncthreads();
}

__device__ inline void enqueue_cost_work(int2* work, int* counter, int s, int M, int N, int* scratch) {
    const int tiles = (N + cost::kTileN - 1) / cost::kTileN, total = M * tiles;
    if (total <= 0) return;
    __syncthreads();
    if (threadIdx.x == 0) scratch[0] = atomicAdd(counter, total);
    __syncthreads();
    const int base = scratch[0];
    for (int i = threadIdx.x; i < total; i += blockDim.x) work[base + i] = make_int2(s, (i / tiles) * 64 + i % tiles);
}

__device__ inline void prep_detections(const Dev& d, int s, int n, int part = 0, int nparts = 1) {
    const size_t db = (size_t)s * d.MD;
    const int tid = threadIdx.x;
    const int nw = blockDim.x >> 5, nt = blockDim.x;
    for (int j = part * nw + (tid >> 5); j < n; j += nparts * nw) {
        const float4 v = reinterpret_cast<const float4*>(d.embs + (db + j) * cost::kD)[tid & 31];
        reinterpret_cast<float4*>(d.det_unit + (db + j) * cost::kD)[tid & 31] = cost::unit_row(v);
    }
    for (int j = part * nt + tid; j < n; j += nparts * nt) {
        double b[4];
        float z[4];
#pragma unroll
        for (int k = 0; k < 4; ++k) { b[k] = d.boxes[(db + j) * 4 + k]; d.det_boxf[(db + j) * 4 + k] = (float)b[k]; }
        kf::box_to_z(b, z);
#pragma unroll
        for (int k = 0; k < 4; ++k) d.det_z[(db + j) * 4 + k] = z[k];
        d.det_conff[db + j] = (float)d.confs[db + j];
        d.det_used[db + j] = 0;
    }
}

__device__ inline void predict_slot(const Dev& d, size_t slot) {
    const float q[8] = {1.f, 1.f, 1.f, 1.f, 100.f, 100.f, 100.f, 100.f};
    const float rdiag[4] = {1.f, 1.f, 1.f, 1.f};
    double x[8], P[64], b[4];
    load_kf(d, slot, x, P);
    const int st = d.kf_stage[slot];
    kf::predict(x, P, st, q);
    store_kf(d, slot, x, P);
    kf::x_to_box(x, b);
#pragma unroll
    for (int k = 0; k < 4; ++k) { d.last_bbox[slot * 4 + k] = b[k]; d.prev_boxf[slot * 4 + k] = (float)b[k]; }
    d.prev_conff[slot] = (float)d.last_conf[slot];
    kf::Gate g;
    kf::gate_prepare(x, P, st, rdiag, &g);
#pragma unroll
    for (int k = 0; k < 16; ++k) d.gate_SI[slot * 16 + k] = g.SI[k];
}

__global__ void __launch_bounds__(kThreads) begin_kernel(Dev d) {
    Span span((d.frame_id[0] & 7) * 6 + 0);
    __shared__ int scratch[kThreads / 32];
    const int s = blockIdx.x, tid = threadIdx.x;
    int* hdr = d.hdr + s * kHdr;
    int* cnt = d.cnt + s * kHdr;
    int* res = d.result + (size_t)s * d.res_stride;
    const size_t sb = (size_t)s * d.MT, db = (size_t)s * d.MD;
    const int n = d.n_det[s], nl = hdr[H_NLIVE];
    int* order = d.order + sb;
    if (blockIdx.y == 1) {
        if (n <= 0) return;
        prep_detections(d, s, n);
        return;
    }
    if (s == 0 && tid == 0) d.wcount[2] = 0;
    if (n < 0) {
        if (tid == 0) {
            cnt[C_MODE] = MODE_SKIP;
            res[R_NMATCH] = res[R_NUT] = res[R_NUD] = res[R_STATUS] = res[R_M1] = res[R_M2] = 0;
            res[R_NLIVE] = nl;
            res[R_NEXT] = hdr[H_NEXT];
        }
        return;
    }
    if (n == 0) {
        int* ut = res_ut(d, res);
        for (int p = tid; p < nl; p += blockDim.x) {
            const size_t slot = sb + order[p];
            d.miss[slot] += 1;
            ut[p] = d.tid[slot];
        }
        __syncthreads();
        purge(d, s, nl, scratch);
        if (tid == 0) {
            cnt[C_MODE] = MODE_EMPTY;
            res[R_NMATCH] = 0; res[R_NUT] = nl; res[R_NUD] = 0; res[R_STATUS] = 0; res[R_M1] = res[R_M2] = 0;
            res[R_NLIVE] = hdr[H_NLIVE];
            res[R_NEXT] = hdr[H_NEXT];
        }
        return;
    }
    for (int p = tid; p < nl; p += blockDim.x) predict_slot(d, sb + order[p]);
    int* rm = d.rows_main + sb;
    int* rr = d.rows_reid + sb;
    const int M1 = block_compact(nl, [&](int i) { return d.miss[sb + order[i]] <= d.lost_reid_after; },
                                 [&](int pos, int i) { rm[pos] = order[i]; }, scratch);
    const int M2 = block_compact(nl, [&](int i) { return d.miss[sb + order[i]] > d.lost_reid_after; },
                                 [&](int pos, int i) { rr[pos] = order[i]; }, scratch);
    if (tid == 0) {
        cnt[C_M1] = M1; cnt[C_M2] = M2; cnt[C_NU] = 0; cnt[C_MODE] = MODE_NORMAL;
        cnt[C_NMATCH] = 0; cnt[C_NUT] = 0; cnt[C_STATUS] = 0;
    }
    enqueue_cost_work(d.work1, d.wcount + 0, s, M1, 1, scratch);
}

__device__ inline void cost2_item(const Dev& d, int s, int r, int j0, float* smem, int* s_idx) {
    const int tid = threadIdx.x, warp = tid >> 5, lane = tid & 31;
    const int N = d.cnt[s * kHdr + C_NU];
    const size_t sb = (size_t)s * d.MT, db = (size_t)s * d.MD;
    const size_t slot = sb + d.rows_reid[sb + r];
    int T = d.bank_len[slot];
    const float* rows = d.bank + slot * d.HIST * cost::kD;
    if (T <= 0) { rows = d.ema + slot * cost::kD; T = 1; }
    if (tid < cost::kTileN) {
        const int j = j0 + tid;
        s_idx[tid] = j < N ? d.ud1[db + j] : 0;
    }
    __syncthreads();
    const int tc = cost::bank_cap(T);
    float* sBank = smem;
    float* sDet = sBank + tc * cost::kD;
    float* sSim = sDet + cost::kTileN * cost::kDetStride;
    for (int t = warp; t < tc; t += cost::kThreads / 32) {
        float4 v = make_float4(0, 0, 0, 0);
        if (t < T) v = cost::unit_row(reinterpret_cast<const float4*>(rows + (size_t)t * cost::kD)[lane]);
        reinterpret_cast<float4*>(sBank + t * cost::kD)[lane] = v;
    }
    for (int j = warp; j < cost::kTileN; j += cost::kThreads / 32) {
        float4 v = make_float4(0, 0, 0, 0);
        if (j0 + j < N) v = reinterpret_cast<const float4*>(d.det_unit + (db + s_idx[j]) * cost::kD)[lane];
        reinterpret_cast<float4*>(sDet + j * cost::kDetStride)[lane] = v;
    }
    __syncthreads();
    const float c_app = cost::sims_and_topk(sBank, sDet, sSim, tc, T, d.topk, true);
    const int j = j0 + tid;
    if (tid < cost::kTileN && j < N) {
        d.C2[(sb + r) * d.MD + j] = c_app;
        d.C2T[(db + j) * d.MT + r] = c_app;
    }
}

__global__ void __launch_bounds__(cost::kThreads) cost2_kernel(Dev d) {
    Span span((d.frame_id[0] & 7) * 6 + 3);
    TRK_PDL_PROLOGUE();
    extern __shared__ __align__(16) float smem[];
    __shared__ int s_idx[cost::kTileN];
    const int total = d.wcount[1];
    for (int wi = blockIdx.x; wi < total; wi += gridDim.x) {
        const int2 item = d.work2[wi];
        cost2_item(d, item.x, item.y >> 6, (item.y & 63) * cost::kTileN, smem, s_idx);
    }
}

struct RowMin {
    float m = __builtin_huge_valf(), first = 0.0f;
    int mj = -1, cnt = 0, bad = 0;
    __device__ __forceinline__ void see(float c, int j) {
        if (c != c || c == -__builtin_huge_valf()) bad = 1;
        if (c < m) { m = c; mj = j; cnt = 1; first = c; }
        else if (c == m) ++cnt;
    }
    __device__ __forceinline__ void finish(int* fc, float* fv, int lane) const {
        const unsigned kFull = 0xffffffffu;
        const unsigned bits = (unsigned)__float_as_int(m + 0.0f);
        const unsigned key = bits ^ ((unsigned)((int)bits >> 31) | 0x80000000u);
        const unsigned kmin = __reduce_min_sync(kFull, key);
        const unsigned eq = __ballot_sync(kFull, key == kmin && mj >= 0);
        const bool any_bad = __any_sync(kFull, bad);
        const int total = __reduce_add_sync(kFull, (key == kmin && mj >= 0) ? cnt : 0);
        if (any_bad) { if (lane == 0) *fc = -2; return; }
        if (eq && lane == __ffs(eq) - 1) {
            *fc = (total == 1 && m < __builtin_huge_valf()) ? mj : -1;
            *fv = first;
        }
        if (!eq && lane == 0) *fc = -1;
    }
};

#ifndef B200_COST1_WARPS
#define B200_COST1_WARPS 4
#endif
constexpr int kCost1Warps = B200_COST1_WARPS;

__device__ __forceinline__ unsigned fkey(float f) {
    const unsigned b = __float_as_uint(f);
    return b ^ ((b >> 31) ? 0xffffffffu : 0x80000000u);
}

__global__ void __launch_bounds__(kCost1Warps * 32) cost1_sparse_kernel(Dev d) {
    Span span((d.frame_id[0] & 7) * 6 + 1);
    TRK_PDL_PROLOGUE();
    const int total = d.wcount[0];
    const int warp = threadIdx.x >> 5, lane = threadIdx.x & 31;
    const float kNegInf = -__int_as_float(0x7f800000);
    for (int wi = blockIdx.x * kCost1Warps + warp; wi < total; wi += gridDim.x * kCost1Warps) {
        const int2 item = d.work1[wi];
        const int s = item.x, r = item.y >> 6;
        const int N = d.n_det[s];
        const size_t sb = (size_t)s * d.MT, db = (size_t)s * d.MD;
        const size_t slot = sb + d.rows_main[sb + r];
        int T = d.bank_len[slot];
        const float* rows = d.bank + slot * d.HIST * cost::kD;
        if (T <= 0) { rows = d.ema + slot * cost::kD; T = 1; }
        const int kk = min(d.topk, T);
        double SI[16], xs[4];
#pragma unroll
        for (int k = 0; k < 16; ++k) SI[k] = d.gate_SI[slot * 16 + k];
#pragma unroll
        for (int k = 0; k < 4; ++k) xs[k] = d.kf_x[slot * 8 + k];
        const int stage = d.kf_stage[slot];
        float pb[4];
#pragma unroll
        for (int k = 0; k < 4; ++k) pb[k] = d.prev_boxf[slot * 4 + k];
        const float pconf = d.prev_conff[slot];
        float inv0 = 0.0f, inv1 = 0.0f;
        bool have_norm = false;
        RowMin rmin;
        for (int j0 = 0; j0 < N; j0 += 32) {
            const int j = j0 + lane;
            bool alive = false;
            if (j < N) alive = !(kf::gate_d2(SI, xs, stage, d.det_z + (db + j) * 4) > d.maha_thr);
            unsigned todo = __ballot_sync(0xffffffffu, alive);
            float c_app = 0.0f;
            while (todo) {
                const int jl = __ffs(todo) - 1;
                todo &= todo - 1;
                const float4 dv = reinterpret_cast<const float4*>(d.det_unit + (db + j0 + jl) * cost::kD)[lane];
                float s0 = kNegInf, s1 = kNegInf;
                for (int t0 = 0; t0 < T; t0 += 8) {
                    float4 bv[8];
#pragma unroll
                    for (int u = 0; u < 8; ++u)
                        if (t0 + u < T) bv[u] = reinterpret_cast<const float4*>(rows + (size_t)(t0 + u) * cost::kD)[lane];
#pragma unroll
                    for (int u = 0; u < 8; ++u) {
                        const int t = t0 + u;
                        if (t >= T) break;
                        float p = bv[u].x * dv.x;
                        p = fmaf(bv[u].y, dv.y, p); p = fmaf(bv[u].z, dv.z, p); p = fmaf(bv[u].w, dv.w, p);
                        p = warp_sum(p);
                        if (!have_norm) {
                            float q = bv[u].x * bv[u].x;
                            q = fmaf(bv[u].y, bv[u].y, q); q = fmaf(bv[u].z, bv[u].z, q); q = fmaf(bv[u].w, bv[u].w, q);
                            q = warp_sum(q);
                            const float iv = __fdiv_rn(1.0f, __fadd_rn(sqrtf(q), 1e-12f));
                            if (lane == (t & 31)) { if (t < 32) inv0 = iv; else inv1 = iv; }
                        }
                        if (lane == (t & 31)) { if (t < 32) s0 = p; else s1 = p; }
                    }
                }
                have_norm = true;
                if (lane < T) s0 *= inv0;
                if (lane + 32 < T) s1 *= inv1;
                float sum = 0.0f;
                for (int q = 0; q < kk; ++q) {
                    const float mine = fmaxf(s0, s1);
                    const unsigned m = __reduce_max_sync(0xffffffffu, fkey(mine));
                    const unsigned who = __ballot_sync(0xffffffffu, fkey(mine) == m);
                    if (lane == __ffs(who) - 1) {
                        if (s0 >= s1) s0 = kNegInf; else s1 = kNegInf;
                    }
                    const unsigned bits = m ^ ((m >> 31) ? 0x80000000u : 0xffffffffu);
                    sum = __fadd_rn(sum, __uint_as_float(bits));
                }
                const float ca = __fsub_rn(1.0f, __fdiv_rn(sum, (float)kk));
                if (lane == jl) c_app = ca;
            }
            if (j < N) {
                float total_c = 1e9f;
                if (alive)
                    total_c = cost::pair_cost(pb, d.det_boxf + (db + j) * 4, pconf, d.det_conff[db + j], d.pw, c_app).total;
                d.C1[(sb + r) * d.MD + j] = total_c;
                d.C1T[(db + j) * d.MT + r] = total_c;
                rmin.see(total_c, j);
            }
        }
        rmin.finish(d.row_fc + sb + r, d.row_fv + sb + r, lane);
    }
}

__device__ __forceinline__ void transpose_reduce32(float (&p)[32]) {
    const int lane = threadIdx.x & 31;
#pragma unroll
    for (int o = 16; o > 0; o >>= 1) {
        const bool up = lane & o;
#pragma unroll
        for (int i = 0; i < o; ++i) {
            const float keep = up ? p[i + o] : p[i], send = up ? p[i] : p[i + o];
            p[i] = keep + __shfl_xor_sync(0xffffffffu, send, o);
        }
    }
}

template <bool FLY>
__device__ __forceinline__ void cost1_row32(const Dev& d, int s, int r, size_t slot, int N, int lane) {
    const float kNegInf = -__int_as_float(0x7f800000);
    const size_t sb = (size_t)s * d.MT, db = (size_t)s * d.MD;
    int T = d.bank_len[slot];
    const float* rows = d.bank + slot * d.HIST * cost::kD;
    if (T <= 0) { rows = d.ema + slot * cost::kD; T = 1; }
    const int kk = min(d.topk, T);
    double SI[16], xs[4];
#pragma unroll
    for (int k = 0; k < 16; ++k) SI[k] = d.gate_SI[slot * 16 + k];
#pragma unroll
    for (int k = 0; k < 4; ++k) xs[k] = d.kf_x[slot * 8 + k];
    const int stage = d.kf_stage[slot];
    float pb[4];
#pragma unroll
    for (int k = 0; k < 4; ++k) pb[k] = d.prev_boxf[slot * 4 + k];
    const float pconf = d.prev_conff[slot];
    float4 bv[32];
    float inv = 0.0f;
    bool have_bank = false;
    RowMin rmin;
    for (int j0 = 0; j0 < N; j0 += 32) {
        const int j = j0 + lane;
        bool alive = false;
        float zl[4], bf[4];
        float cf = 0.0f;
        if (j < N) {
            if (FLY) {
                double b[4];
#pragma unroll
                for (int k = 0; k < 4; ++k) { b[k] = d.boxes[(db + j) * 4 + k]; bf[k] = (float)b[k]; }
                kf::box_to_z(b, zl);
                cf = (float)d.confs[db + j];
                alive = !(kf::gate_d2(SI, xs, stage, zl) > d.maha_thr);
            } else {
                alive = !(kf::gate_d2(SI, xs, stage, d.det_z + (db + j) * 4) > d.maha_thr);
            }
        }
        unsigned todo = __ballot_sync(0xffffffffu, alive);
        float c_app = 0.0f;
        float4 dv_first = make_float4(0, 0, 0, 0);
        if (todo) {
            const int jf = __ffs(todo) - 1;
            if (FLY) dv_first = reinterpret_cast<const float4*>(d.embs + (db + j0 + jf) * cost::kD)[lane];
            else dv_first = reinterpret_cast<const float4*>(d.det_unit + (db + j0 + jf) * cost::kD)[lane];
        }
        if (todo && !have_bank) {
            float q[32];
#pragma unroll
            for (int t = 0; t < 32; ++t)
                bv[t] = t < T ? reinterpret_cast<const float4*>(rows + (size_t)t * cost::kD)[lane] : make_float4(0, 0, 0, 0);
#pragma unroll
            for (int t = 0; t < 32; ++t) {
                float a = bv[t].x * bv[t].x;
                a = fmaf(bv[t].y, bv[t].y, a); a = fmaf(bv[t].z, bv[t].z, a); a = fmaf(bv[t].w, bv[t].w, a);
                q[t] = a;
            }
            transpose_reduce32(q);
            inv = __fdiv_rn(1.0f, __fadd_rn(sqrtf(q[0]), 1e-12f));
            have_bank = true;
        }
        bool first = true;
        while (todo) {
            const int jl = __ffs(todo) - 1;
            todo &= todo - 1;
            float4 dv = dv_first;
            if (!first) {
                if (FLY) dv = reinterpret_cast<const float4*>(d.embs + (db + j0 + jl) * cost::kD)[lane];
                else dv = reinterpret_cast<const float4*>(d.det_unit + (db + j0 + jl) * cost::kD)[lane];
            }
            first = false;
            if (FLY) dv = cost::unit_row(dv);
            float p[32];
#pragma unroll
            for (int t = 0; t < 32; ++t) {
                float a = bv[t].x * dv.x;
                a = fmaf(bv[t].y, dv.y, a); a = fmaf(bv[t].z, dv.z, a); a = fmaf(bv[t].w, dv.w, a);
                p[t] = a;
            }
            transpose_reduce32(p);
            float sim = lane < T ? p[0] * inv : kNegInf;
            float sum = 0.0f;
            for (int q = 0; q < kk; ++q) {
                const unsigned m = __reduce_max_sync(0xffffffffu, fkey(sim));
                const unsigned who = __ballot_sync(0xffffffffu, fkey(sim) == m);
                if (lane == __ffs(who) - 1) sim = kNegInf;
                const unsigned bits = m ^ ((m >> 31) ? 0x80000000u : 0xffffffffu);
                sum = __fadd_rn(sum, __uint_as_float(bits));
            }
            const float ca = __fsub_rn(1.0f, __fdiv_rn(sum, (float)kk));
            if (lane == jl) c_app = ca;
        }
        if (j < N) {
            float total_c = 1e9f;
            if (alive) {
                if (FLY) total_c = cost::pair_cost(pb, bf, pconf, cf, d.pw, c_app).total;
                else total_c = cost::pair_cost(pb, d.det_boxf + (db + j) * 4, pconf, d.det_conff[db + j], d.pw, c_app).total;
            }
            d.C1[(sb + r) * d.MD + j] = total_c;
            d.C1T[(db + j) * d.MT + r] = total_c;
            rmin.see(total_c, j);
        }
    }
    rmin.finish(d.row_fc + sb + r, d.row_fv + sb + r, lane);
}

__global__ void __launch_bounds__(kCost1Warps * 32, 2) cost1_sparse32_kernel(Dev d) {
    Span span((d.frame_id[0] & 7) * 6 + 1);
    TRK_PDL_PROLOGUE();
    const int total = d.wcount[0];
    const int warp = threadIdx.x >> 5, lane = threadIdx.x & 31;
    for (int wi = blockIdx.x * kCost1Warps + warp; wi < total; wi += gridDim.x * kCost1Warps) {
        const int2 item = d.work1[wi];
        const int s = item.x, r = item.y >> 6;
        const size_t sb = (size_t)s * d.MT;
        cost1_row32<false>(d, s, r, sb + d.rows_main[sb + r], d.n_det[s], lane);
    }
}

__device__ inline void note_matches(const Dev& d, int s, int nm, const int* rows, const float* C, int ldc,
                                    const int* m_col, int reid_stage, int* scratch, int queue_base = -1) {
    if (nm <= 0) return;
    const size_t sb = (size_t)s * d.MT, db = (size_t)s * d.MD;
    const int frame = d.frame_id[s];
    int base = queue_base;
    if (queue_base < 0) {
        __syncthreads();
        if (threadIdx.x == 0) scratch[0] = atomicAdd(d.wcount + 2, nm);
        __syncthreads();
        base = scratch[0];
    }
    for (int qd = threadIdx.x; qd < nm; qd += blockDim.x) {
        const int r = d.m_row[sb + qd], j = d.m_det[sb + qd];
        const size_t slot = sb + rows[r];
        const float c = C[(size_t)r * ldc + m_col[qd]];
#pragma unroll
        for (int k = 0; k < 4; ++k) d.last_bbox[slot * 4 + k] = d.boxes[(db + j) * 4 + k];
        d.last_conf[slot] = d.confs[db + j];
        d.last_frame[slot] = frame;
        d.age[slot] += 1;
        d.miss[slot] = 0;
        d.last_cost[slot] = (double)c;
        d.upd_slot[base + qd] = (int)slot;
        d.upd_det[base + qd] = (int)(db + j);
        d.upd_cost[base + qd] = c;
        d.upd_flag[base + qd] = (uint8_t)reid_stage;
    }
}

constexpr int kUpdWarps = 4;

__device__ __forceinline__ void update_entries(const Dev& d, int first, int total, int wq, int nwq, double* scratch) {
    const int lane = threadIdx.x & 31, sub = lane & 7, grp = lane >> 3;
    double* sP = scratch + (size_t)grp * 96;
    double* sK = sP + 64;
    const float rdiag[4] = {1.f, 1.f, 1.f, 1.f};
    for (int w0 = wq * 4; w0 < total; w0 += nwq * 4) {
        const int idx = first + w0 + grp;
        const bool on = w0 + grp < total;
        size_t slot = 0, det = 0;
        int st = -1, reid = 0;
        double c = 0.0, conf = 0.0;
        if (on) {
            slot = (size_t)d.upd_slot[idx];
            det = (size_t)d.upd_det[idx];
            c = (double)d.upd_cost[idx];
            reid = d.upd_flag[idx];
            st = d.kf_stage[slot];
            conf = d.confs[det];
        }
        const float* z = d.det_z + det * 4;
        const double cmax = reid ? d.reid_only_cost_max : d.cost_update_max;
        int app = on && !(conf < d.conf_update_min) && !(c > cmax);
        const int nst = st < 2 ? st + 1 : 2;
        float4 e[4], o[4];
        size_t slots[4];
        int len[4], head[4];
#pragma unroll
        for (int u = 0; u < 4; ++u) {
            const bool on_u = __shfl_sync(0xffffffffu, (int)on, u * 8) != 0;
            const unsigned long long sl = __shfl_sync(0xffffffffu, (unsigned long long)slot, u * 8);
            const unsigned long long dt = __shfl_sync(0xffffffffu, (unsigned long long)det, u * 8);
            slots[u] = (size_t)sl;
            if (on_u) {
                e[u] = reinterpret_cast<const float4*>(d.det_unit + (size_t)dt * cost::kD)[lane];
                o[u] = reinterpret_cast<const float4*>(d.ema + slots[u] * cost::kD)[lane];
                len[u] = d.bank_len[slots[u]];
                head[u] = d.bank_head[slots[u]];
            }
        }
        double d2 = 0.0;
#pragma unroll
        for (int v = 0; v < 6; ++v) {
            const bool mine = on && st == (v >> 1) && reid == (v & 1);
            const unsigned mask = __ballot_sync(0xffffffffu, mine);
            if (mine) {
                double* gx = d.kf_x + slot * 8;
                double* gP = d.kf_P + slot * 64;
                const bool want = !(v & 1);
                if ((v >> 1) == 0) d2 = kf::update_rows_t<float, float>(gx, gP, z, rdiag, sP, sK, sub, mask, nst, want);
                else if ((v >> 1) == 1) d2 = kf::update_rows_t<float, double>(gx, gP, z, rdiag, sP, sK, sub, mask, nst, want);
                else d2 = kf::update_rows_t<double, double>(gx, gP, z, rdiag, sP, sK, sub, mask, nst, want);
            }
        }
        if (on && sub == 0) d.kf_stage[slot] = (uint8_t)nst;
        if (app && !reid && d2 > d.maha_thr) app = 0;
        bool go[4];
#pragma unroll
        for (int u = 0; u < 4; ++u) go[u] = __shfl_sync(0xffffffffu, app, u * 8) != 0;
#pragma unroll
        for (int u = 0; u < 4; ++u) {
            if (!go[u]) continue;
            float4 f;
            f.x = __fadd_rn(__fmul_rn(d.ema_a, o[u].x), __fmul_rn(d.ema_b, e[u].x));
            f.y = __fadd_rn(__fmul_rn(d.ema_a, o[u].y), __fmul_rn(d.ema_b, e[u].y));
            f.z = __fadd_rn(__fmul_rn(d.ema_a, o[u].z), __fmul_rn(d.ema_b, e[u].z));
            f.w = __fadd_rn(__fmul_rn(d.ema_a, o[u].w), __fmul_rn(d.ema_b, e[u].w));
            reinterpret_cast<float4*>(d.ema + slots[u] * cost::kD)[lane] = cost::unit_row(f);
            int pos;
            if (len[u] < d.HIST) { pos = head[u] + len[u]; if (pos >= d.HIST) pos -= d.HIST; ++len[u]; }
            else { pos = head[u]; head[u] = head[u] + 1 == d.HIST ? 0 : head[u] + 1; }
            reinterpret_cast<float4*>(d.bank + (slots[u] * d.HIST + pos) * cost::kD)[lane] = e[u];
            __syncwarp();
            if (lane == 0) { d.bank_len[slots[u]] = len[u]; d.bank_head[slots[u]] = head[u]; }
        }
        __syncwarp();
    }
}

__global__ void __launch_bounds__(kUpdWarps * 32) update_kernel(Dev d) {
    Span span((d.frame_id[0] & 7) * 6 + 5);
    TRK_PDL_PROLOGUE();
    __shared__ double scratch[kUpdWarps * 4 * 96];
    const int warp = threadIdx.x >> 5;
    update_entries(d, 0, d.wcount[2], blockIdx.x * kUpdWarps + warp, gridDim.x * kUpdWarps, scratch + (size_t)warp * 4 * 96);
}

__device__ inline int spawn_tracks(const Dev& d, int s, const int* born, int want) {
    const int tid = threadIdx.x;
    int* hdr = d.hdr + s * kHdr;
    int* cnt = d.cnt + s * kHdr;
    const size_t sb = (size_t)s * d.MT, db = (size_t)s * d.MD;
    const int nl = hdr[H_NLIVE], nfree = hdr[H_NFREE], next_id = hdr[H_NEXT];
    int* order = d.order + sb;
    const int* fl = d.free_list + sb;
    const int nb = min(want, nfree);
    const int frame = d.frame_id[s];
    __syncthreads();
    for (int b = tid; b < nb; b += blockDim.x) {
        const int j = born[b], sl = fl[nfree - 1 - b];
        const size_t slot = sb + sl;
        double x[8], P[64], box[4];
#pragma unroll
        for (int k = 0; k < 4; ++k) { box[k] = d.boxes[(db + j) * 4 + k]; d.last_bbox[slot * 4 + k] = box[k]; }
        kf::init_state(box, x, P);
        store_kf(d, slot, x, P);
        d.kf_stage[slot] = 0;
        d.last_conf[slot] = d.confs[db + j];
        d.last_cost[slot] = __longlong_as_double(0x7ff8000000000000LL);
        d.last_frame[slot] = frame;
        d.tid[slot] = next_id + b;
        d.miss[slot] = 0;
        d.age[slot] = 1;
        d.bank_len[slot] = 1;
        d.bank_head[slot] = 0;
        order[nl + b] = sl;
    }
    for (int i = tid; i < nb * (cost::kD / 4); i += blockDim.x) {
        const int b = i / (cost::kD / 4), k = i % (cost::kD / 4);
        const size_t slot = sb + fl[nfree - 1 - b];
        const float4 e = reinterpret_cast<const float4*>(d.det_unit + (db + born[b]) * cost::kD)[k];
        reinterpret_cast<float4*>(d.ema + slot * cost::kD)[k] = e;
        reinterpret_cast<float4*>(d.bank + slot * d.HIST * cost::kD)[k] = e;
    }
    __syncthreads();
    if (tid == 0) {
        hdr[H_NLIVE] = nl + nb;
        hdr[H_NFREE] = nfree - nb;
        hdr[H_NEXT] = next_id + nb;
        if (want > nb && cnt[C_STATUS] == 0) cnt[C_STATUS] = B200_ECAPACITY;
    }
    __syncthreads();
    return nb;
}

template <int STAGE, bool INLINE, bool OWNQ>
__device__ inline bool assign_body(const Dev& d, int s, unsigned char* smem_raw, int smem_matrix_floats) {
    __shared__ int scratch[kThreads / 32];
    __shared__ int s_rc;
    const int tid = threadIdx.x;
    int* cnt = d.cnt + s * kHdr;
    if (!INLINE && STAGE == 2 && s == 0 && tid == 0) { d.wcount[0] = 0; d.wcount[1] = 0; }
    int* hdr = d.hdr + s * kHdr;
    int* res = d.result + (size_t)s * d.res_stride;
    if (STAGE == 2 && cnt[C_MODE] == MODE_FAILED) {
        if (tid == 0) {
            res[R_NMATCH] = res[R_NUT] = res[R_NUD] = 0;
            res[R_NLIVE] = hdr[H_NLIVE]; res[R_NEXT] = hdr[H_NEXT]; res[R_STATUS] = cnt[C_STATUS];
            res[R_M1] = cnt[C_M1]; res[R_M2] = cnt[C_M2];
        }
        return true;
    }
    if (cnt[C_MODE] != MODE_NORMAL) return true;
    const size_t sb = (size_t)s * d.MT, db = (size_t)s * d.MD;
    const int M = STAGE == 1 ? cnt[C_M1] : cnt[C_M2];
    const int N = STAGE == 1 ? d.n_det[s] : cnt[C_NU];
    const int* rows = (STAGE == 1 ? d.rows_main : d.rows_reid) + sb;
    const float* C = (STAGE == 1 ? d.C1 : d.C2) + sb * d.MD;
    const float* CT = (STAGE == 1 ? d.C1T : d.C2T) + db * d.MT;
    const double cmax = STAGE == 1 ? d.cost_max : d.reid_only_cost_max;
    const int match0 = STAGE == 1 ? 0 : cnt[C_NMATCH], ut0 = STAGE == 1 ? 0 : cnt[C_NUT];
    int* out_m = res_matches(d, res);
    int* out_ut = res_ut(d, res);
    int* m_col = d.tmp + sb;
    int n_match = 0, n_ut = 0, n_left = N;
    bool failed = false;
    if (STAGE == 1) TRK_STAMP(0);

    if (M > 0 && N > 0) {
        const bool tall = M > N;
        const int R = tall ? N : M, Cc = tall ? M : N;
        const float* costp = tall ? CT : C;
        const int ld = tall ? d.MT : d.MD;
        const lsap::Work w = lsap::carve(smem_raw, R, Cc);
        float* stage = (size_t)R * Cc <= (size_t)smem_matrix_floats
                           ? reinterpret_cast<float*>(smem_raw + lsap::work_bytes(R, Cc)) : nullptr;
        const bool pre = STAGE == 1 && !tall;
        const int rc = lsap::solve_block(costp, R, Cc, ld, w, stage, pre ? d.row_fc + sb : nullptr,
                                         pre ? d.row_fv + sb : nullptr);
        if (tid == 0) s_rc = rc;
        __syncthreads();
        if (STAGE == 1) TRK_STAMP(1);
        if (s_rc != B200_OK) {
            failed = true;
            if (tid == 0) { cnt[C_STATUS] = s_rc; if (STAGE == 1) cnt[C_MODE] = MODE_FAILED; }
        } else {
            const int* col = tall ? w.r4c : w.c4r;
            auto is_match = [&](int r) {
                const int j = col[r];
                return j >= 0 && (double)C[(size_t)r * d.MD + j] <= cmax;
            };
            n_match = block_compact(M, is_match, [&](int pos, int r) {
                const int jl = col[r], j = STAGE == 1 ? jl : d.ud1[db + jl];
                d.m_row[sb + pos] = r;
                d.m_det[sb + pos] = j;
                m_col[pos] = jl;
                d.det_used[db + j] = 1;
                out_m[2 * (match0 + pos)] = d.tid[sb + rows[r]];
                out_m[2 * (match0 + pos) + 1] = j;
            }, scratch);
            n_ut = block_compact(M, [&](int r) { return !is_match(r); }, [&](int pos, int r) {
                const size_t slot = sb + rows[r];
                d.miss[slot] += 1;
                out_ut[ut0 + pos] = d.tid[slot];
            }, scratch);
            __syncthreads();
            note_matches(d, s, n_match, rows, C, d.MD, m_col, STAGE == 2, scratch, OWNQ ? (int)sb + match0 : -1);
        }
    } else if (M > 0) {
        for (int r = tid; r < M; r += blockDim.x) {
            const size_t slot = sb + rows[r];
            d.miss[slot] += 1;
            out_ut[ut0 + r] = d.tid[slot];
        }
        n_ut = M;
        __syncthreads();
    }

    if (STAGE == 1) {
        if (failed) {
            if (tid == 0) { cnt[C_NU] = 0; cnt[C_NMATCH] = 0; cnt[C_NUT] = 0; }
            return true;
        }
        n_left = block_compact(N, [&](int j) { return d.det_used[db + j] == 0; },
                               [&](int pos, int j) { d.ud1[db + pos] = j; }, scratch);
        if (tid == 0) { cnt[C_NU] = n_left; cnt[C_NMATCH] = n_match; cnt[C_NUT] = n_ut; }
        if (!INLINE) enqueue_cost_work(d.work2, d.wcount + 1, s, n_left > 0 ? cnt[C_M2] : 0, n_left, scratch);
        TRK_STAMP(5);
        __syncthreads();
        return false;
    }

    if (failed) {
        if (tid == 0) {
            res[R_NMATCH] = match0; res[R_NUT] = ut0; res[R_NUD] = 0;
            res[R_NLIVE] = hdr[H_NLIVE]; res[R_NEXT] = hdr[H_NEXT]; res[R_STATUS] = cnt[C_STATUS];
            res[R_M1] = cnt[C_M1]; res[R_M2] = cnt[C_M2];
        }
        return true;
    }
    int* out_ud = res_ud(d, res);
    n_left = block_compact(N, [&](int jl) { return d.det_used[db + d.ud1[db + jl]] == 0; },
                           [&](int pos, int jl) { out_ud[pos] = d.ud1[db + jl]; }, scratch);
    int* born = d.born + db;
    const int want = block_compact(n_left, [&](int k) { return !(d.confs[db + out_ud[k]] < d.init_conf_min); },
                                   [&](int pos, int k) { born[pos] = out_ud[k]; }, scratch);
    const int nl = hdr[H_NLIVE];
    const int nb = spawn_tracks(d, s, born, want);
    purge(d, s, nl + nb, scratch);
    if (tid == 0) {
        res[R_NMATCH] = match0 + n_match;
        res[R_NUT] = ut0 + n_ut;
        res[R_NUD] = n_left;
        res[R_NLIVE] = hdr[H_NLIVE];
        res[R_NEXT] = hdr[H_NEXT];
        res[R_STATUS] = cnt[C_STATUS];
        res[R_M1] = cnt[C_M1];
        res[R_M2] = cnt[C_M2];
    }
    return true;
}

template <int STAGE>
__global__ void __launch_bounds__(kThreads) assign_kernel(Dev d, int smem_matrix_floats) {
    Span span((d.frame_id[0] & 7) * 6 + (STAGE == 1 ? 2 : 4));
    TRK_PDL_PROLOGUE();
    extern __shared__ __align__(16) unsigned char smem_raw[];
    assign_body<STAGE, false, false>(d, blockIdx.x, smem_raw, smem_matrix_floats);
}

#ifndef B200_TRK_FRONT_WARPS
#define B200_TRK_FRONT_WARPS 4
#endif
constexpr int kFrontWarps = B200_TRK_FRONT_WARPS;

__global__ void __launch_bounds__(kFrontWarps * 32, 2) front_kernel(Dev d) {
    Span span((d.frame_id[0] & 7) * 6 + 0);
    extern __shared__ __align__(16) int s_rows[];
    __shared__ int scratch[kThreads / 32];
    const int s = blockIdx.y, g = blockIdx.x, G = gridDim.x, tid = threadIdx.x, warp = tid >> 5, lane = tid & 31;
    TRK_GSTAMP(0);
    int* hdr = d.hdr + s * kHdr;
    int* cnt = d.cnt + s * kHdr;
    int* res = d.result + (size_t)s * d.res_stride;
    const size_t sb = (size_t)s * d.MT;
    const int n = d.n_det[s], nl = hdr[H_NLIVE];
    const int* order = d.order + sb;
    if (s == 0 && g == 0 && tid == 0) d.wcount[2] = 0;
    if (n < 0) {
        if (g == 0 && tid == 0) {
            cnt[C_MODE] = MODE_SKIP;
            res[R_NMATCH] = res[R_NUT] = res[R_NUD] = res[R_STATUS] = res[R_M1] = res[R_M2] = 0;
            res[R_NLIVE] = nl;
            res[R_NEXT] = hdr[H_NEXT];
        }
        return;
    }
    if (n == 0) {
        if (g != 0) return;
        int* ut = res_ut(d, res);
        for (int p = tid; p < nl; p += blockDim.x) {
            const size_t slot = sb + order[p];
            d.miss[slot] += 1;
            ut[p] = d.tid[slot];
        }
        __syncthreads();
        purge(d, s, nl, scratch);
        if (tid == 0) {
            cnt[C_MODE] = MODE_EMPTY;
            res[R_NMATCH] = 0; res[R_NUT] = nl; res[R_NUD] = 0; res[R_STATUS] = 0; res[R_M1] = res[R_M2] = 0;
            res[R_NLIVE] = hdr[H_NLIVE];
            res[R_NEXT] = hdr[H_NEXT];
        }
        return;
    }
    int* rm = s_rows;
    int* rr = s_rows + d.MT;
    const int M1 = block_compact(nl, [&](int i) { return d.miss[sb + order[i]] <= d.lost_reid_after; },
                                 [&](int pos, int i) { rm[pos] = order[i]; }, scratch);
    const int M2 = block_compact(nl, [&](int i) { return d.miss[sb + order[i]] > d.lost_reid_after; },
                                 [&](int pos, int i) { rr[pos] = order[i]; }, scratch);
    if (g == 0) {
        for (int i = tid; i < M1; i += blockDim.x) d.rows_main[sb + i] = rm[i];
        for (int i = tid; i < M2; i += blockDim.x) d.rows_reid[sb + i] = rr[i];
        if (tid == 0) {
            cnt[C_M1] = M1; cnt[C_M2] = M2; cnt[C_NU] = 0; cnt[C_MODE] = MODE_NORMAL;
            cnt[C_NMATCH] = 0; cnt[C_NUT] = 0; cnt[C_STATUS] = 0;
        }
    }
    TRK_GSTAMP(1);
    prep_detections(d, s, n, g, G);
    const int own1 = M1 > g ? (M1 - g + G - 1) / G : 0, own2 = M2 > g ? (M2 - g + G - 1) / G : 0;
    for (int i = tid; i < own1 + own2; i += blockDim.x)
        predict_slot(d, sb + (i < own1 ? rm[g + i * G] : rr[g + (i - own1) * G]));
    __syncthreads();
    TRK_GSTAMP(2);
    for (int i = warp; i < own1; i += kFrontWarps) {
        const int r = g + i * G;
        cost1_row32<true>(d, s, r, sb + rm[r], n, lane);
    }
    TRK_GSTAMP(3);
}

#ifndef B200_TRK_BACK_CLUSTER
#define B200_TRK_BACK_CLUSTER 4
#endif
constexpr int kBackCluster = B200_TRK_BACK_CLUSTER;

__device__ __forceinline__ unsigned cluster_ctarank() {
    unsigned r;
    asm volatile("mov.u32 %0, %%cluster_ctarank;" : "=r"(r));
    return r;
}
__device__ __forceinline__ unsigned cluster_nctarank() {
    unsigned r;
    asm volatile("mov.u32 %0, %%cluster_nctarank;" : "=r"(r));
    return r;
}
__device__ __forceinline__ void cluster_sync_all() {
    asm volatile("barrier.cluster.arrive.release.aligned;\n\tbarrier.cluster.wait.acquire.aligned;" ::: "memory");
}

template <bool UPDATES>
__global__ void __launch_bounds__(kThreads, UPDATES ? 1 : 2) back_kernel(Dev d, int smem_matrix_floats) {
    Span span((d.frame_id[0] & 7) * 6 + 2);
    TRK_PDL_PROLOGUE();
    extern __shared__ __align__(16) unsigned char smem_raw[];
    __shared__ int s_idx[cost::kTileN];
    const unsigned rank = cluster_ctarank(), nrank = cluster_nctarank();
    const int s = blockIdx.x / nrank, tid = threadIdx.x;
    const int* cnt = d.cnt + s * kHdr;
    TRK_GSTAMP(4);
    if (rank == 0) {
        if (!assign_body<1, true, UPDATES>(d, s, smem_raw, smem_matrix_floats)) {
            TRK_GSTAMP(5);
            const int M2 = cnt[C_M2], NU = cnt[C_NU];
            if (M2 > 0 && NU > 0) {
                const int tiles = (NU + cost::kTileN - 1) / cost::kTileN;
                for (int it = 0; it < M2 * tiles; ++it)
                    cost2_item(d, s, it / tiles, (it % tiles) * cost::kTileN, reinterpret_cast<float*>(smem_raw), s_idx);
            }
            __syncthreads();
        }
        TRK_GSTAMP(6);
        assign_body<2, true, UPDATES>(d, s, smem_raw, smem_matrix_floats);
        __syncthreads();
        TRK_GSTAMP(7);
    }
    if (!UPDATES) return;
    if (nrank > 1) cluster_sync_all();
    if (cnt[C_MODE] != MODE_NORMAL) return;
    const int total = d.result[(size_t)s * d.res_stride + R_NMATCH];
    const int warp = tid >> 5;
    update_entries(d, (int)((size_t)s * d.MT), total, (int)rank * (kThreads / 32) + warp, (int)nrank * (kThreads / 32),
                   reinterpret_cast<double*>(smem_raw) + (size_t)warp * 4 * 96);
    TRK_GSTAMP(8);
}


__device__ inline int find_slot(const Dev& d, int s, int nl, int track_id) {
    const size_t sb = (size_t)s * d.MT;
    int lo = 0, hi = nl - 1;
    while (lo <= hi) {
        const int mid = (lo + hi) >> 1, sl = d.order[sb + mid], t = d.tid[sb + sl];
        if (t == track_id) return sl;
        if (t < track_id) lo = mid + 1; else hi = mid - 1;
    }
    return -1;
}

__global__ void __launch_bounds__(kThreads) op_predict_kernel(Dev d, int s) {
    const size_t sb = (size_t)s * d.MT;
    const int nl = d.hdr[s * kHdr + H_NLIVE];
    for (int p = threadIdx.x; p < nl; p += blockDim.x) predict_slot(d, sb + d.order[sb + p]);
}

__global__ void __launch_bounds__(kThreads) op_mark_missed_kernel(Dev d, int s, const int* tids, int n) {
    const size_t sb = (size_t)s * d.MT;
    const int nl = d.hdr[s * kHdr + H_NLIVE];
    if (threadIdx.x == 0)
        for (int i = 0; i < n; ++i) {
            const int sl = find_slot(d, s, nl, tids[i]);
            if (sl >= 0) d.miss[sb + sl] += 1;
        }
}

__global__ void __launch_bounds__(kThreads) op_purge_kernel(Dev d, int s) {
    __shared__ int scratch[kThreads / 32];
    purge(d, s, d.hdr[s * kHdr + H_NLIVE], scratch);
}

__global__ void __launch_bounds__(kThreads) op_create_kernel(Dev d, int s, const int* det_ids, int n_ids, int n_det, int* out) {
    __shared__ int scratch[kThreads / 32];
    const size_t db = (size_t)s * d.MD;
    if (threadIdx.x == 0) d.cnt[s * kHdr + C_STATUS] = 0;
    prep_detections(d, s, n_det);
    __syncthreads();
    int* born = d.born + db;
    const int want = block_compact(n_ids, [&](int k) { return !(d.confs[db + det_ids[k]] < d.init_conf_min); },
                                   [&](int pos, int k) { born[pos] = det_ids[k]; }, scratch);
    const int nb = spawn_tracks(d, s, born, want);
    if (threadIdx.x == 0) { out[0] = nb; out[1] = d.cnt[s * kHdr + C_STATUS]; }
}

__global__ void __launch_bounds__(kThreads) op_queue_matches_kernel(Dev d, int s, const int* tids, const int* dets,
                                                                     const float* costs, int n, int n_det, int* out) {
    const size_t sb = (size_t)s * d.MT, db = (size_t)s * d.MD;
    const int nl = d.hdr[s * kHdr + H_NLIVE], frame = d.frame_id[s];
    __shared__ int bad;
    if (threadIdx.x == 0) bad = 0;
    prep_detections(d, s, n_det);
    __syncthreads();
    for (int q = threadIdx.x; q < n; q += blockDim.x)
        if (find_slot(d, s, nl, tids[q]) < 0 || dets[q] < 0 || dets[q] >= n_det) bad = 1;
    __syncthreads();
    if (bad) {
        if (threadIdx.x == 0) { out[1] = B200_EINVAL; d.wcount[2] = 0; }
        return;
    }
    for (int q = threadIdx.x; q < n; q += blockDim.x) {
        const size_t slot = sb + find_slot(d, s, nl, tids[q]);
        const int j = dets[q];
#pragma unroll
        for (int k = 0; k < 4; ++k) d.last_bbox[slot * 4 + k] = d.boxes[(db + j) * 4 + k];
        d.last_conf[slot] = d.confs[db + j];
        d.last_frame[slot] = frame;
        d.age[slot] += 1;
        d.miss[slot] = 0;
        d.last_cost[slot] = (double)costs[q];
        d.upd_slot[q] = (int)slot;
        d.upd_det[q] = (int)(db + j);
        d.upd_cost[q] = costs[q];
        d.upd_flag[q] = 0;
    }
    if (threadIdx.x == 0) { out[1] = 0; d.wcount[2] = n; }
}

__global__ void export_kernel(Dev d, int s, int* ids, double* x, double* P, uint8_t* stage, float* ema, float* bank,
                              int* bank_len, int* miss, int* age, double* last_bbox, double* last_conf,
                              double* last_cost) {
    const size_t sb = (size_t)s * d.MT;
    const int nl = d.hdr[s * kHdr + H_NLIVE];
    for (int p = blockIdx.x; p < nl; p += gridDim.x) {
        const size_t slot = sb + d.order[sb + p];
        const int t = threadIdx.x;
        if (t == 0) {
            ids[p] = d.tid[slot]; stage[p] = d.kf_stage[slot]; bank_len[p] = d.bank_len[slot];
            miss[p] = d.miss[slot]; age[p] = d.age[slot]; last_conf[p] = d.last_conf[slot];
            last_cost[p] = d.last_cost[slot];
        }
        if (t < 8) x[(size_t)p * 8 + t] = d.kf_x[slot * 8 + t];
        if (t < 4) last_bbox[(size_t)p * 4 + t] = d.last_bbox[slot * 4 + t];
        if (t < 64) P[(size_t)p * 64 + t] = d.kf_P[slot * 64 + t];
        if (t < cost::kD) ema[(size_t)p * cost::kD + t] = d.ema[slot * cost::kD + t];
        const int len = d.bank_len[slot], head = d.bank_head[slot];
        for (int i = t; i < d.HIST * cost::kD; i += blockDim.x) {
            const int row = i / cost::kD, k = i % cost::kD;
            bank[((size_t)p * d.HIST + row) * cost::kD + k] =
                row < len ? d.bank[(slot * d.HIST + (head + row) % d.HIST) * cost::kD + k] : 0.0f;
        }
    }
}

__global__ void import_finish_kernel(Dev d, int s, int n, int next_id) {
    const size_t sb = (size_t)s * d.MT;
    for (int i = threadIdx.x; i < d.MT; i += blockDim.x) {
        if (i < n) { d.order[sb + i] = i; d.bank_head[sb + i] = 0; d.last_frame[sb + i] = 0; }
        if (i < d.MT - n) d.free_list[sb + i] = d.MT - 1 - i;
    }
    if (threadIdx.x == 0) {
        d.hdr[s * kHdr + H_NLIVE] = n;
        d.hdr[s * kHdr + H_NEXT] = next_id;
        d.hdr[s * kHdr + H_NFREE] = d.MT - n;
    }
}

__global__ void reset_kernel(Dev d) {
    const int s = blockIdx.x;
    for (int i = threadIdx.x; i < d.MT; i += blockDim.x) d.free_list[(size_t)s * d.MT + i] = d.MT - 1 - i;
    if (threadIdx.x == 0) {
        d.hdr[s * kHdr + H_NLIVE] = 0;
        d.hdr[s * kHdr + H_NEXT] = 0;
        d.hdr[s * kHdr + H_NFREE] = d.MT;
        if (s == 0) { d.wcount[0] = 0; d.wcount[1] = 0; d.wcount[2] = 0; }
    }
}

}
}

using namespace b200;

struct b200_tracker {
    trk::Dev d;
    void* arena = nullptr;
    static constexpr int kRing = 4;
    void* pinned = nullptr;
    size_t in_bytes = 0, res_bytes = 0, slot_bytes = 0;
    cudaEvent_t done[kRing] = {};
    void* ring_dev = nullptr;
    cudaStream_t up_stream = nullptr, down_stream = nullptr;
    cudaEvent_t up[kRing] = {}, ran[kRing] = {};
    long long ticket_of[kRing] = {-1, -1, -1, -1};
    long long next_ticket = 0;
    int* in_ndet = nullptr; int* in_frame = nullptr; double* in_boxes = nullptr; double* in_confs = nullptr;
    float* in_embs = nullptr; int* dev_result = nullptr;
    int ctl_threads = 256;
#ifndef B200_TRK_BEGIN_THREADS
#define B200_TRK_BEGIN_THREADS 256
#endif
    int begin_threads = B200_TRK_BEGIN_THREADS;
    int cost_grid = 0, cost1_grid = 0, upd_grid = 0;
    size_t assign_smem = 0;
    int smem_matrix_floats = 0;
    int chain = 6;
    int front_resident = 0;
    size_t front_smem = 0, back_smem = 0;
};

namespace {

struct Carver {
    size_t off = 0;
    template <typename T> size_t take(size_t n) {
        off = (off + 255) & ~(size_t)255;
        const size_t at = off;
        off += n * sizeof(T);
        return at;
    }
};

}

extern "C" int b200_tracker_create(b200_tracker** out, int n_streams, int max_tracks, int max_dets,
                                   const b200_tracker_conf* conf) {
    B200_REQUIRE(out && conf, "tracker_create: null pointer");
    B200_REQUIRE(n_streams >= 1 && n_streams <= 65535, "tracker_create: n_streams %d out of range", n_streams);
    B200_REQUIRE(max_tracks >= 1 && max_tracks <= 4096 && max_dets >= 1 && max_dets <= 4096 && n_streams * (long long)max_tracks < (1 << 25),
                 "tracker_create: capacities out of range (tracks %d, dets %d)", max_tracks, max_dets);
    B200_REQUIRE(conf->hist_max >= 1 && conf->hist_max <= cost::kMaxBank, "tracker_create: hist_max %d outside [1,%d]",
                 conf->hist_max, cost::kMaxBank);
    B200_REQUIRE(conf->emb_top_k >= 1, "tracker_create: emb_top_k must be >= 1");
    b200_tracker* t = new (std::nothrow) b200_tracker();
    B200_REQUIRE(t, "tracker_create: out of host memory");
    trk::Dev& d = t->d;
    memset(&d, 0, sizeof(d));
    const size_t S = n_streams, MT = max_tracks, MD = max_dets, H = conf->hist_max;
    d.S = n_streams; d.MT = max_tracks; d.MD = max_dets; d.HIST = conf->hist_max;
    d.res_stride = trk::R_HDR + 2 * max_dets + max_tracks + max_dets;
    Carver c;
#define TAKE(field, T, n) const size_t o_##field = c.take<T>(n)
    TAKE(kf_x, double, S * MT * 8); TAKE(kf_P, double, S * MT * 64); TAKE(last_bbox, double, S * MT * 4);
    TAKE(last_conf, double, S * MT); TAKE(last_cost, double, S * MT); TAKE(kf_stage, uint8_t, S * MT);
    TAKE(ema, float, S * MT * 128); TAKE(bank, float, S * MT * H * 128);
    TAKE(bank_len, int, S * MT); TAKE(bank_head, int, S * MT); TAKE(tid, int, S * MT); TAKE(miss, int, S * MT);
    TAKE(age, int, S * MT); TAKE(last_frame, int, S * MT); TAKE(order, int, S * MT); TAKE(free_list, int, S * MT);
    TAKE(hdr, int, S * trk::kHdr);
    TAKE(det_unit, float, S * MD * 128); TAKE(det_z, float, S * MD * 4); TAKE(det_boxf, float, S * MD * 4);
    TAKE(det_conff, float, S * MD); TAKE(prev_boxf, float, S * MT * 4); TAKE(prev_conff, float, S * MT);
    TAKE(C1, float, S * MT * MD); TAKE(C1T, float, S * MT * MD); TAKE(C2, float, S * MT * MD);
    TAKE(C2T, float, S * MT * MD); TAKE(gate_SI, double, S * MT * 16);
    TAKE(row_fc, int, S * MT); TAKE(row_fv, float, S * MT);
    TAKE(rows_main, int, S * MT); TAKE(rows_reid, int, S * MT); TAKE(cnt, int, S * trk::kHdr);
    TAKE(ud1, int, S * MD); TAKE(det_used, int, S * MD); TAKE(m_row, int, S * MT); TAKE(m_det, int, S * MT);
    TAKE(m_app, int, S * MT); TAKE(tmp, int, S * MT); TAKE(born, int, S * MD);
    const size_t tiles_max = (MD + cost::kTileN - 1) / cost::kTileN;
    TAKE(work1, int2, S * MT * tiles_max); TAKE(work2, int2, S * MT * tiles_max); TAKE(wcount, int, 4);
    TAKE(upd_slot, int, S * MT); TAKE(upd_det, int, S * MT); TAKE(upd_cost, float, S * MT); TAKE(upd_flag, uint8_t, S * MT);
    const size_t o_in = c.take<double>(0);
    TAKE(in_ndet, int, S); TAKE(in_frame, int, S); TAKE(in_boxes, double, S * MD * 4); TAKE(in_confs, double, S * MD);
    TAKE(in_embs, float, S * MD * 128);
    const size_t in_end = c.off;
    TAKE(result, int, S * (size_t)d.res_stride);
#undef TAKE
    cudaError_t e = cudaMalloc(&t->arena, c.off);
    if (e != cudaSuccess) {
        delete t;
        return fail(B200_ECUDA, "tracker_create: cudaMalloc(%zu bytes): %s", c.off, cudaGetErrorString(e));
    }
    char* base = static_cast<char*>(t->arena);
    cudaMemset(base, 0, c.off);
#define PTR(field, T) d.field = reinterpret_cast<T*>(base + o_##field)
    PTR(kf_x, double); PTR(kf_P, double); PTR(last_bbox, double); PTR(last_conf, double); PTR(last_cost, double);
    PTR(kf_stage, uint8_t); PTR(ema, float); PTR(bank, float); PTR(bank_len, int); PTR(bank_head, int); PTR(tid, int);
    PTR(miss, int); PTR(age, int); PTR(last_frame, int); PTR(order, int); PTR(free_list, int); PTR(hdr, int);
    PTR(det_unit, float); PTR(det_z, float); PTR(det_boxf, float); PTR(det_conff, float); PTR(prev_boxf, float);
    PTR(prev_conff, float); PTR(C1, float); PTR(C1T, float); PTR(C2, float); PTR(C2T, float); PTR(gate_SI, double);
    PTR(row_fc, int); PTR(row_fv, float);
    PTR(rows_main, int); PTR(rows_reid, int); PTR(cnt, int); PTR(ud1, int); PTR(det_used, int); PTR(m_row, int);
    PTR(m_det, int); PTR(m_app, int); PTR(tmp, int); PTR(born, int); PTR(work1, int2); PTR(work2, int2); PTR(wcount, int);
    PTR(upd_slot, int); PTR(upd_det, int); PTR(upd_cost, float); PTR(upd_flag, uint8_t);
#undef PTR
    t->in_ndet = reinterpret_cast<int*>(base + o_in_ndet);
    t->in_frame = reinterpret_cast<int*>(base + o_in_frame);
    t->in_boxes = reinterpret_cast<double*>(base + o_in_boxes);
    t->in_confs = reinterpret_cast<double*>(base + o_in_confs);
    t->in_embs = reinterpret_cast<float*>(base + o_in_embs);
    t->dev_result = reinterpret_cast<int*>(base + o_result);
    t->in_bytes = in_end - o_in;
    t->res_bytes = S * (size_t)d.res_stride * sizeof(int);
    t->slot_bytes = ((t->in_bytes + 255) & ~(size_t)255) + ((t->res_bytes + 255) & ~(size_t)255);
    e = cudaMallocHost(&t->pinned, t->slot_bytes * b200_tracker::kRing);
    if (e == cudaSuccess) e = cudaMalloc(&t->ring_dev, t->slot_bytes * b200_tracker::kRing);
    if (e == cudaSuccess) e = cudaStreamCreateWithFlags(&t->up_stream, cudaStreamNonBlocking);
    if (e == cudaSuccess) e = cudaStreamCreateWithFlags(&t->down_stream, cudaStreamNonBlocking);
    for (int i = 0; e == cudaSuccess && i < b200_tracker::kRing; ++i) {
        e = cudaEventCreateWithFlags(&t->done[i], cudaEventDisableTiming);
        if (e == cudaSuccess) e = cudaEventCreateWithFlags(&t->up[i], cudaEventDisableTiming);
        if (e == cudaSuccess) e = cudaEventCreateWithFlags(&t->ran[i], cudaEventDisableTiming);
    }
    if (e != cudaSuccess) {
        b200_tracker_destroy(t);
        return fail(B200_ECUDA, "tracker_create: host ring / streams: %s", cudaGetErrorString(e));
    }
    d.pw = cost::PairWeights{(float)conf->w_app, (float)conf->w_bbox, (float)conf->w_conf, (float)conf->alpha,
                             (float)conf->beta, 1e-6f};
    d.maha_thr = conf->maha_thr; d.cost_max = conf->cost_max; d.conf_update_min = conf->conf_update_min;
    d.cost_update_max = conf->cost_update_max; d.reid_only_cost_max = conf->reid_only_cost_max;
    d.init_conf_min = conf->init_conf_min;
    d.ema_a = (float)conf->ema_alpha;
    d.ema_b = (float)(1.0 - conf->ema_alpha);
    d.topk = conf->emb_top_k; d.max_age = conf->max_age; d.lost_reid_after = conf->lost_reid_after;
    const int Rm = max_tracks < max_dets ? max_tracks : max_dets, Cm = max_tracks < max_dets ? max_dets : max_tracks;
    const size_t wb = lsap::work_bytes(Rm, Cm), budget = 200 * 1024;
    if (wb > budget) {
        b200_tracker_destroy(t);
        return fail(B200_EINVAL, "tracker_create: %d x %d exceeds the assignment kernel's shared memory", max_tracks, max_dets);
    }
    size_t mat = (size_t)Rm * Cm * sizeof(float);
    if (wb + mat > budget) mat = budget - wb;
    if (max_tracks <= 1024 && max_dets <= 256 && mat > 32 * 1024) mat = 32 * 1024;
    t->smem_matrix_floats = (int)(mat / sizeof(float));
    t->assign_smem = wb + mat;
    cudaFuncSetAttribute(trk::assign_kernel<1>, cudaFuncAttributeMaxDynamicSharedMemorySize, (int)budget);
    cudaFuncSetAttribute(trk::assign_kernel<2>, cudaFuncAttributeMaxDynamicSharedMemorySize, (int)budget);
    cudaFuncSetAttribute(trk::cost2_kernel, cudaFuncAttributeMaxDynamicSharedMemorySize, (int)cost::smem_bytes(cost::kMaxBank));
    trk::reset_kernel<<<n_streams, 128>>>(d);
    e = cudaDeviceSynchronize();
    if (e != cudaSuccess) {
        b200_tracker_destroy(t);
        return fail(B200_ECUDA, "tracker_create: %s", cudaGetErrorString(e));
    }
    g_launches.fetch_add(1);
    {
        int per_sm = 1, sms = kSMs, devid = 0;
        cudaGetDevice(&devid);
        cudaDeviceGetAttribute(&sms, cudaDevAttrMultiProcessorCount, devid);
        cudaOccupancyMaxActiveBlocksPerMultiprocessor(&per_sm, trk::cost2_kernel, cost::kThreads,
                                                      cost::smem_bytes(d.HIST));
        t->cost_grid = sms * (per_sm > 0 ? per_sm : 1);
        per_sm = 1;
        if (d.HIST <= 32)
            cudaOccupancyMaxActiveBlocksPerMultiprocessor(&per_sm, trk::cost1_sparse32_kernel, trk::kCost1Warps * 32, 0);
        else
            cudaOccupancyMaxActiveBlocksPerMultiprocessor(&per_sm, trk::cost1_sparse_kernel, trk::kCost1Warps * 32, 0);
        t->cost1_grid = sms * (per_sm > 0 ? per_sm : 1);
        t->upd_grid = sms * 2;
        const bool fits = max_tracks <= 512 && max_dets <= 256 && d.HIST <= 32;
        t->chain = !fits ? 6 : n_streams <= 8 ? 2 : 3;
        if (const char* e = getenv("B200TRACK_CHAIN")) {
            const int want = atoi(e);
            if (want == 6 || (fits && (want == 2 || want == 3))) t->chain = want;
        }
        if (t->chain != 6) {
            t->front_smem = sizeof(int) * 2 * (size_t)max_tracks;
            size_t bs = t->assign_smem;
            if (cost::smem_bytes(d.HIST) > bs) bs = cost::smem_bytes(d.HIST);
            if (sizeof(double) * (trk::kThreads / 32) * 4 * 96 > bs) bs = sizeof(double) * (trk::kThreads / 32) * 4 * 96;
            t->back_smem = bs;
            cudaFuncSetAttribute(trk::back_kernel<true>, cudaFuncAttributeMaxDynamicSharedMemorySize, (int)budget);
            cudaFuncSetAttribute(trk::back_kernel<false>, cudaFuncAttributeMaxDynamicSharedMemorySize, (int)budget);
            per_sm = 1;
            cudaOccupancyMaxActiveBlocksPerMultiprocessor(&per_sm, trk::front_kernel, trk::kFrontWarps * 32, t->front_smem);
            t->front_resident = sms * (per_sm > 0 ? per_sm : 1);
            if (const char* e = getenv("B200TRACK_FRONT_CTAS")) t->front_resident = atoi(e) > 0 ? atoi(e) : t->front_resident;
            if (const char* e = getenv("B200TRACK_UPD_CTAS")) t->upd_grid = atoi(e) > 0 ? atoi(e) : t->upd_grid;
        }
    }
    *out = t;
    return B200_OK;
}

extern "C" void b200_tracker_destroy(b200_tracker* t) {
    if (!t) return;
    if (t->up_stream) { cudaStreamSynchronize(t->up_stream); cudaStreamDestroy(t->up_stream); }
    if (t->down_stream) { cudaStreamSynchronize(t->down_stream); cudaStreamDestroy(t->down_stream); }
    for (int i = 0; i < b200_tracker::kRing; ++i) {
        if (t->done[i]) cudaEventDestroy(t->done[i]);
        if (t->up[i]) cudaEventDestroy(t->up[i]);
        if (t->ran[i]) cudaEventDestroy(t->ran[i]);
    }
    cudaFreeHost(t->pinned);
    cudaFree(t->ring_dev);
    cudaFree(t->arena);
    delete t;
}

extern "C" int b200_tracker_reset(b200_tracker* t, void* stream) {
    B200_REQUIRE(t, "tracker_reset: null handle");
    trk::reset_kernel<<<t->d.S, 128, 0, as_stream(stream)>>>(t->d);
    return check_launch("reset_kernel");
}

extern "C" int b200_tracker_result_stride(const b200_tracker* t) { return t ? t->d.res_stride : 0; }

extern "C" int b200_tracker_live_counts(b200_tracker* t, int32_t* n_live_host, int32_t* next_id_host, void* stream) {
    B200_REQUIRE(t, "tracker_live_counts: null handle");
    cudaStream_t st = as_stream(stream);
    const int S = t->d.S;
    int* h = static_cast<int*>(malloc(sizeof(int) * trk::kHdr * (size_t)S));
    B200_REQUIRE(h, "tracker_live_counts: out of host memory");
    cudaError_t e = cudaMemcpyAsync(h, t->d.hdr, sizeof(int) * trk::kHdr * (size_t)S, cudaMemcpyDeviceToHost, st);
    if (e == cudaSuccess) e = cudaStreamSynchronize(st);
    if (e != cudaSuccess) {
        free(h);
        return fail(B200_ECUDA, "tracker_live_counts: %s", cudaGetErrorString(e));
    }
    for (int s = 0; s < S; ++s) {
        if (n_live_host) n_live_host[s] = h[s * trk::kHdr + trk::H_NLIVE];
        if (next_id_host) next_id_host[s] = h[s * trk::kHdr + trk::H_NEXT];
    }
    free(h);
    return B200_OK;
}

extern "C" int b200_tracker_step(b200_tracker* t, const int32_t* n_det, const double* boxes, const double* confs,
                                 const float* embs, const int32_t* frame_id, int32_t* result, void* stream) {
    B200_REQUIRE(t && n_det && boxes && confs && embs && frame_id && result, "tracker_step: null pointer");
    cudaStream_t st = as_stream(stream);
    trk::Dev d = t->d;
    d.n_det = n_det; d.boxes = boxes; d.confs = confs; d.embs = embs; d.frame_id = frame_id; d.result = result;
    const size_t csm = cost::smem_bytes(d.HIST);
    const int cost_grid = t->cost_grid;
    int rc;
    if (t->chain != 6) {
        int G = t->front_resident / d.S;
        const int gmax = (d.MT + 3) / 4;
        G = G < 1 ? 1 : G > gmax ? gmax : G;
        trk::front_kernel<<<dim3(G, d.S), trk::kFrontWarps * 32, t->front_smem, st>>>(d);
        if ((rc = check_launch("trk front_kernel"))) return rc;
        if (t->chain == 3) {
            trk::back_kernel<false><<<d.S, trk::kThreads, t->assign_smem > cost::smem_bytes(d.HIST) ? t->assign_smem
                                                                                                    : cost::smem_bytes(d.HIST), st>>>(
                d, t->smem_matrix_floats);
            if ((rc = check_launch("trk back_kernel<false>"))) return rc;
            trk::update_kernel<<<t->upd_grid, trk::kUpdWarps * 32, 0, st>>>(d);
            return check_launch("trk update_kernel");
        }
        const bool few = d.S <= 8;
        const int cl = few ? trk::kBackCluster : 1;
        cudaLaunchConfig_t cfg = {};
        cfg.gridDim = dim3(d.S * cl); cfg.blockDim = dim3(trk::kThreads); cfg.dynamicSmemBytes = t->back_smem; cfg.stream = st;
        cudaLaunchAttribute attr[2];
        attr[0].id = cudaLaunchAttributeProgrammaticStreamSerialization;
        attr[0].val.programmaticStreamSerializationAllowed = 1;
        attr[1].id = cudaLaunchAttributeClusterDimension;
        attr[1].val.clusterDim.x = cl; attr[1].val.clusterDim.y = 1; attr[1].val.clusterDim.z = 1;
        cfg.attrs = attr;
        cfg.numAttrs = few ? 2 : 0;
        (void)cudaLaunchKernelEx(&cfg, trk::back_kernel<true>, d, t->smem_matrix_floats);
        return check_launch("trk back_kernel");
    }
    trk::begin_kernel<<<dim3(d.S, 2), t->begin_threads, 0, st>>>(d);
    rc = check_launch("trk begin_kernel");
    if (rc) return rc;
    const bool pdl = d.S <= 8;
    auto launch = [&](auto kern, dim3 grid, dim3 block, size_t smem, auto... args) {
        cudaLaunchConfig_t cfg = {};
        cfg.gridDim = grid; cfg.blockDim = block; cfg.dynamicSmemBytes = smem; cfg.stream = st;
        cudaLaunchAttribute attr[1];
        attr[0].id = cudaLaunchAttributeProgrammaticStreamSerialization;
        attr[0].val.programmaticStreamSerializationAllowed = 1;
        cfg.attrs = attr;
        cfg.numAttrs = pdl ? 1 : 0;
        (void)cudaLaunchKernelEx(&cfg, kern, args...);
    };
    if (d.HIST <= 32) launch(trk::cost1_sparse32_kernel, dim3(t->cost1_grid), dim3(trk::kCost1Warps * 32), 0, d);
    else launch(trk::cost1_sparse_kernel, dim3(t->cost1_grid), dim3(trk::kCost1Warps * 32), 0, d);
    if ((rc = check_launch("trk cost1_sparse_kernel"))) return rc;
    launch(trk::assign_kernel<1>, dim3(d.S), dim3(t->ctl_threads), t->assign_smem, d, t->smem_matrix_floats);
    if ((rc = check_launch("trk assign_kernel<1>"))) return rc;
    launch(trk::cost2_kernel, dim3(cost_grid), dim3(cost::kThreads), csm, d);
    if ((rc = check_launch("trk cost2_kernel"))) return rc;
    launch(trk::assign_kernel<2>, dim3(d.S), dim3(t->ctl_threads), t->assign_smem, d, t->smem_matrix_floats);
    if ((rc = check_launch("trk assign_kernel<2>"))) return rc;
    launch(trk::update_kernel, dim3(t->upd_grid), dim3(trk::kUpdWarps * 32), 0, d);
    if ((rc = check_launch("trk update_kernel"))) return rc;
    return B200_OK;
}

namespace {
int step_host_submit(b200_tracker* t, const int32_t* n_det_host, const double* boxes_host, const double* confs_host,
                     const float* embs_host, const int32_t* frame_id_host, int64_t* ticket, void* stream, bool direct,
                     bool inline_dma = false) {
    B200_REQUIRE(t && n_det_host && frame_id_host && ticket, "tracker_step_host_async: null pointer");
    cudaStream_t st = as_stream(stream);
    const trk::Dev& d = t->d;
    const int slot = (int)(t->next_ticket % b200_tracker::kRing);
    if (t->ticket_of[slot] >= 0) B200_CUDA(cudaEventSynchronize(t->done[slot]));
    char* pin = static_cast<char*>(t->pinned) + (size_t)slot * t->slot_bytes;
    char* dev_in = reinterpret_cast<char*>(t->in_ndet);
    auto host_of = [&](const void* dev_ptr) { return pin + (reinterpret_cast<const char*>(dev_ptr) - dev_in); };
    int* h_ndet = reinterpret_cast<int*>(host_of(t->in_ndet));
    int* h_frame = reinterpret_cast<int*>(host_of(t->in_frame));
    double* h_boxes = reinterpret_cast<double*>(host_of(t->in_boxes));
    double* h_confs = reinterpret_cast<double*>(host_of(t->in_confs));
    float* h_embs = reinterpret_cast<float*>(host_of(t->in_embs));
    bool dense = true;
    int n_max = 0;
    for (int s = 0; s < d.S; ++s) {
        const int n = n_det_host[s];
        B200_REQUIRE(n <= d.MD, "tracker_step_host: stream %d has %d detections, capacity %d", s, n, d.MD);
        h_ndet[s] = n;
        h_frame[s] = frame_id_host[s];
        if (n != d.MD) dense = false;
        if (n > n_max) n_max = n;
        if (n > 0) B200_REQUIRE(boxes_host && confs_host && embs_host, "tracker_step_host: null detection arrays");
    }
    char* dslot = static_cast<char*>(t->ring_dev) + (size_t)slot * t->slot_bytes;
    auto dev_of = [&](const void* base_ptr) { return dslot + (reinterpret_cast<const char*>(base_ptr) - dev_in); };
    int* d_ndet = reinterpret_cast<int*>(dev_of(t->in_ndet));
    int* d_frame = reinterpret_cast<int*>(dev_of(t->in_frame));
    double* d_boxes = reinterpret_cast<double*>(dev_of(t->in_boxes));
    double* d_confs = reinterpret_cast<double*>(dev_of(t->in_confs));
    float* d_embs = reinterpret_cast<float*>(dev_of(t->in_embs));
    int* d_res = reinterpret_cast<int*>(dslot + ((t->in_bytes + 255) & ~(size_t)255));
    cudaStream_t up = inline_dma ? st : t->up_stream, down = inline_dma ? st : t->down_stream;
    if (direct) {
        const void* arrs[3] = {boxes_host, confs_host, embs_host};
        for (int k = 0; k < 3 && n_max > 0; ++k) {
            cudaPointerAttributes pa = {};
            const cudaError_t e = cudaPointerGetAttributes(&pa, arrs[k]);
            if (e != cudaSuccess) cudaGetLastError();
            B200_REQUIRE(e == cudaSuccess && pa.type == cudaMemoryTypeHost,
                         "tracker_step_pinned_async: the detection arrays must be page-locked host memory "
                         "(cudaHostAlloc / cudaHostRegister / torch pin_memory)");
        }
        B200_CUDA(cudaMemcpyAsync(d_ndet, h_ndet, sizeof(int) * d.S, cudaMemcpyHostToDevice, up));
        B200_CUDA(cudaMemcpyAsync(d_frame, h_frame, sizeof(int) * d.S, cudaMemcpyHostToDevice, up));
        if (n_max > 0) {
            B200_CUDA(cudaMemcpyAsync(d_boxes, boxes_host, sizeof(double) * 4 * (size_t)d.S * d.MD, cudaMemcpyHostToDevice, up));
            B200_CUDA(cudaMemcpyAsync(d_confs, confs_host, sizeof(double) * (size_t)d.S * d.MD, cudaMemcpyHostToDevice, up));
            B200_CUDA(cudaMemcpyAsync(d_embs, embs_host, sizeof(float) * 128 * (size_t)d.S * d.MD, cudaMemcpyHostToDevice, up));
        }
    } else {
        if (dense) {
            memcpy(h_boxes, boxes_host, sizeof(double) * 4 * (size_t)d.S * d.MD);
            memcpy(h_confs, confs_host, sizeof(double) * (size_t)d.S * d.MD);
            memcpy(h_embs, embs_host, sizeof(float) * 128 * (size_t)d.S * d.MD);
        } else {
            for (int s = 0; s < d.S; ++s) {
                const int n = n_det_host[s];
                if (n <= 0) continue;
                memcpy(h_boxes + (size_t)s * d.MD * 4, boxes_host + (size_t)s * d.MD * 4, sizeof(double) * 4 * n);
                memcpy(h_confs + (size_t)s * d.MD, confs_host + (size_t)s * d.MD, sizeof(double) * n);
                memcpy(h_embs + (size_t)s * d.MD * 128, embs_host + (size_t)s * d.MD * 128, sizeof(float) * 128 * n);
            }
        }
        B200_CUDA(cudaMemcpyAsync(dslot, pin, t->in_bytes, cudaMemcpyHostToDevice, up));
    }
    if (!inline_dma) {
        B200_CUDA(cudaEventRecord(t->up[slot], up));
        B200_CUDA(cudaStreamWaitEvent(st, t->up[slot], 0));
    }
    const int rc = b200_tracker_step(t, d_ndet, d_boxes, d_confs, d_embs, d_frame, d_res, stream);
    if (rc) return rc;
    if (!inline_dma) {
        B200_CUDA(cudaEventRecord(t->ran[slot], st));
        B200_CUDA(cudaStreamWaitEvent(down, t->ran[slot], 0));
    }
    char* h_res = pin + ((t->in_bytes + 255) & ~(size_t)255);
    B200_CUDA(cudaMemcpyAsync(h_res, d_res, t->res_bytes, cudaMemcpyDeviceToHost, down));
    B200_CUDA(cudaEventRecord(t->done[slot], down));
    t->ticket_of[slot] = t->next_ticket;
    *ticket = t->next_ticket++;
    return B200_OK;
}
}

extern "C" int b200_tracker_step_host_async(b200_tracker* t, const int32_t* n_det_host, const double* boxes_host,
                                            const double* confs_host, const float* embs_host,
                                            const int32_t* frame_id_host, int64_t* ticket, void* stream) {
    return step_host_submit(t, n_det_host, boxes_host, confs_host, embs_host, frame_id_host, ticket, stream, false);
}

extern "C" int b200_tracker_step_pinned_async(b200_tracker* t, const int32_t* n_det_host, const double* boxes_pinned,
                                              const double* confs_pinned, const float* embs_pinned,
                                              const int32_t* frame_id_host, int64_t* ticket, void* stream) {
    return step_host_submit(t, n_det_host, boxes_pinned, confs_pinned, embs_pinned, frame_id_host, ticket, stream, true);
}

extern "C" int b200_tracker_step_result(b200_tracker* t, int64_t ticket, int32_t* result_host) {
    B200_REQUIRE(t && result_host, "tracker_step_result: null pointer");
    const int slot = (int)(ticket % b200_tracker::kRing);
    B200_REQUIRE(ticket >= 0 && t->ticket_of[slot] == ticket, "tracker_step_result: ticket %lld is not in flight (at most %d steps may be pending)",
                 (long long)ticket, b200_tracker::kRing);
    B200_CUDA(cudaEventSynchronize(t->done[slot]));
    const char* pin = static_cast<const char*>(t->pinned) + (size_t)slot * t->slot_bytes;
    memcpy(result_host, pin + ((t->in_bytes + 255) & ~(size_t)255), t->res_bytes);
    t->ticket_of[slot] = -1;
    return B200_OK;
}

extern "C" int b200_tracker_step_host(b200_tracker* t, const int32_t* n_det_host, const double* boxes_host,
                                      const double* confs_host, const float* embs_host, const int32_t* frame_id_host,
                                      int32_t* result_host, void* stream) {
    B200_REQUIRE(result_host, "tracker_step_host: null pointer");
    int64_t ticket = -1;
    const int rc = step_host_submit(t, n_det_host, boxes_host, confs_host, embs_host, frame_id_host, &ticket, stream, false, true);
    if (rc) return rc;
    return b200_tracker_step_result(t, ticket, result_host);
}

namespace {

int stage_stream_inputs(b200_tracker* t, int s, int n_det, const double* boxes_host, const double* confs_host,
                        const float* embs_host, int frame_id, cudaStream_t st, trk::Dev* d) {
    *d = t->d;
    B200_REQUIRE(n_det >= 0 && n_det <= d->MD, "tracker op: %d detections, capacity %d", n_det, d->MD);
    const size_t MD = d->MD;
    if (n_det > 0) {
        B200_REQUIRE(boxes_host && confs_host && embs_host, "tracker op: null detection arrays");
        B200_CUDA(cudaMemcpyAsync(t->in_boxes + (size_t)s * MD * 4, boxes_host, sizeof(double) * 4 * n_det, cudaMemcpyHostToDevice, st));
        B200_CUDA(cudaMemcpyAsync(t->in_confs + (size_t)s * MD, confs_host, sizeof(double) * n_det, cudaMemcpyHostToDevice, st));
        B200_CUDA(cudaMemcpyAsync(t->in_embs + (size_t)s * MD * 128, embs_host, sizeof(float) * 128 * n_det, cudaMemcpyHostToDevice, st));
    }
    B200_CUDA(cudaMemcpyAsync(t->in_frame + s, &frame_id, sizeof(int), cudaMemcpyHostToDevice, st));
    d->n_det = t->in_ndet; d->boxes = t->in_boxes; d->confs = t->in_confs; d->embs = t->in_embs; d->frame_id = t->in_frame;
    d->result = t->dev_result;
    return B200_OK;
}

int upload_ints(const int32_t* host, int n, int** dev, cudaStream_t st) {
    *dev = nullptr;
    if (n <= 0) return B200_OK;
    B200_CUDA(cudaMallocAsync(reinterpret_cast<void**>(dev), sizeof(int) * (size_t)n, st));
    B200_CUDA(cudaMemcpyAsync(*dev, host, sizeof(int) * (size_t)n, cudaMemcpyHostToDevice, st));
    return B200_OK;
}

}

#define B200_STREAM_ARG(fn)                                                                                  \
    B200_REQUIRE(t, fn ": null handle");                                                                     \
    B200_REQUIRE(stream_idx >= 0 && stream_idx < t->d.S, fn ": stream %d out of range", stream_idx);         \
    cudaStream_t st = as_stream(stream)

extern "C" int b200_tracker_predict_all(b200_tracker* t, int stream_idx, void* stream) {
    B200_STREAM_ARG("tracker_predict_all");
    trk::op_predict_kernel<<<1, trk::kThreads, 0, st>>>(t->d, stream_idx);
    int rc = check_launch("trk op_predict_kernel");
    if (rc) return rc;
    B200_CUDA(cudaStreamSynchronize(st));
    return B200_OK;
}

extern "C" int b200_tracker_mark_missed(b200_tracker* t, int stream_idx, const int32_t* track_ids_host, int n, void* stream) {
    B200_STREAM_ARG("tracker_mark_missed");
    B200_REQUIRE(n >= 0 && (n == 0 || track_ids_host), "tracker_mark_missed: bad id list");
    if (n == 0) return B200_OK;
    int* ids = nullptr;
    int rc = upload_ints(track_ids_host, n, &ids, st);
    if (rc) return rc;
    trk::op_mark_missed_kernel<<<1, trk::kThreads, 0, st>>>(t->d, stream_idx, ids, n);
    rc = check_launch("trk op_mark_missed_kernel");
    cudaFreeAsync(ids, st);
    if (rc) return rc;
    B200_CUDA(cudaStreamSynchronize(st));
    return B200_OK;
}

extern "C" int b200_tracker_purge_dead(b200_tracker* t, int stream_idx, void* stream) {
    B200_STREAM_ARG("tracker_purge_dead");
    trk::op_purge_kernel<<<1, trk::kThreads, 0, st>>>(t->d, stream_idx);
    int rc = check_launch("trk op_purge_kernel");
    if (rc) return rc;
    B200_CUDA(cudaStreamSynchronize(st));
    return B200_OK;
}

extern "C" int b200_tracker_create_tracks(b200_tracker* t, int stream_idx, const int32_t* det_ids_host, int n_ids,
                                          const double* boxes_host, const double* confs_host, const float* embs_host,
                                          int n_det, int frame_id, void* stream) {
    B200_STREAM_ARG("tracker_create_tracks");
    B200_REQUIRE(n_ids >= 0 && (n_ids == 0 || det_ids_host), "tracker_create_tracks: bad id list");
    for (int i = 0; i < n_ids; ++i)
        B200_REQUIRE(det_ids_host[i] >= 0 && det_ids_host[i] < n_det, "tracker_create_tracks: detection index %d out of range", det_ids_host[i]);
    if (n_ids == 0) return 0;
    B200_REQUIRE(n_ids <= t->d.MD, "tracker_create_tracks: %d ids, capacity %d", n_ids, t->d.MD);
    trk::Dev d;
    int rc = stage_stream_inputs(t, stream_idx, n_det, boxes_host, confs_host, embs_host, frame_id, st, &d);
    if (rc) return rc;
    int* ids = nullptr;
    if ((rc = upload_ints(det_ids_host, n_ids + 2, &ids, st))) return rc;
    trk::op_create_kernel<<<1, trk::kThreads, 0, st>>>(d, stream_idx, ids, n_ids, n_det, ids + n_ids);
    rc = check_launch("trk op_create_kernel");
    int out[2] = {0, 0};
    if (rc == B200_OK && cudaMemcpyAsync(out, ids + n_ids, sizeof(out), cudaMemcpyDeviceToHost, st) != cudaSuccess) rc = B200_ECUDA;
    if (rc == B200_OK && cudaStreamSynchronize(st) != cudaSuccess) rc = B200_ECUDA;
    cudaFreeAsync(ids, st);
    if (rc) return rc == B200_ECUDA ? fail(B200_ECUDA, "tracker_create_tracks: %s", cudaGetErrorString(cudaGetLastError())) : rc;
    if (out[1] == B200_ECAPACITY) return fail(B200_ECAPACITY, "tracker_create_tracks: the handle is full (max_tracks %d)", t->d.MT);
    return out[0];
}

extern "C" int b200_tracker_update_matched(b200_tracker* t, int stream_idx, const int32_t* match_tid_host,
                                           const int32_t* match_det_host, const float* match_cost_host, int n_matches,
                                           const double* boxes_host, const double* confs_host, const float* embs_host,
                                           int n_det, int frame_id, double ema_alpha, double conf_update_min,
                                           double cost_update_max, double maha_thr, void* stream) {
    B200_STREAM_ARG("tracker_update_matched");
    B200_REQUIRE(n_matches >= 0 && n_matches <= t->d.MT, "tracker_update_matched: %d matches, capacity %d", n_matches, t->d.MT);
    if (n_matches == 0) return B200_OK;
    B200_REQUIRE(match_tid_host && match_det_host && match_cost_host, "tracker_update_matched: null match arrays");
    trk::Dev d;
    int rc = stage_stream_inputs(t, stream_idx, n_det, boxes_host, confs_host, embs_host, frame_id, st, &d);
    if (rc) return rc;
    d.ema_a = (float)ema_alpha;
    d.ema_b = (float)(1.0 - ema_alpha);
    d.conf_update_min = conf_update_min; d.cost_update_max = cost_update_max; d.maha_thr = maha_thr;
    int* buf = nullptr;
    const size_t n = (size_t)n_matches;
    B200_CUDA(cudaMallocAsync(reinterpret_cast<void**>(&buf), sizeof(int) * (3 * n + 2), st));
    cudaMemcpyAsync(buf, match_tid_host, sizeof(int) * n, cudaMemcpyHostToDevice, st);
    cudaMemcpyAsync(buf + n, match_det_host, sizeof(int) * n, cudaMemcpyHostToDevice, st);
    cudaMemcpyAsync(buf + 2 * n, match_cost_host, sizeof(float) * n, cudaMemcpyHostToDevice, st);
    trk::op_queue_matches_kernel<<<1, trk::kThreads, 0, st>>>(d, stream_idx, buf, buf + n, reinterpret_cast<const float*>(buf + 2 * n),
                                                              n_matches, n_det, buf + 3 * n);
    rc = check_launch("trk op_queue_matches_kernel");
    if (rc == B200_OK) {
        trk::update_kernel<<<t->upd_grid, trk::kUpdWarps * 32, 0, st>>>(d);
        rc = check_launch("trk update_kernel");
    }
    int out[2] = {0, 0};
    if (rc == B200_OK && cudaMemcpyAsync(out, buf + 3 * n, sizeof(out), cudaMemcpyDeviceToHost, st) != cudaSuccess) rc = B200_ECUDA;
    if (rc == B200_OK && cudaStreamSynchronize(st) != cudaSuccess) rc = B200_ECUDA;
    cudaFreeAsync(buf, st);
    if (rc) return rc == B200_ECUDA ? fail(B200_ECUDA, "tracker_update_matched: %s", cudaGetErrorString(cudaGetLastError())) : rc;
    if (out[1]) return fail(B200_EINVAL, "tracker_update_matched: a match names a track id that is not live or a detection index out of range");
    return B200_OK;
}

// ... 89 lines not shown
```

Before: 271,000.

## Stage detections and track banks in shared memory via bulk-copy pipeline in front kernel

The tracker front kernel now stages detection boxes, z-vectors, confidences and unit-normalised embeddings in shared memory. A dedicated producer warp streams each surviving track's embedding bank into a ring of shared buffers using bulk async copies and full/empty mbarriers, while consumer warps compute appearance costs. Gating is done first so tracks with no gated detections skip the bank load. Kalman predict is restructured to load and store P in double2 pairs with a fused element update. Shared mbarrier and bulk-load helpers move into common.cuh. Grid sizing is also reworked. The cost is more shared memory per CTA, an extra warp, and more complex synchronisation.

```diff
diff --git a/a-lightweight-unsupervised-feature-extractor-_b200/csrc/app_cost_tc.cu b/a-lightweight-unsupervised-feature-extractor-_b200/csrc/app_cost_tc.cu
--- a/a-lightweight-unsupervised-feature-extractor-_b200/csrc/app_cost_tc.cu
+++ b/a-lightweight-unsupervised-feature-extractor-_b200/csrc/app_cost_tc.cu
@@ -62,26 +62,6 @@
     }
 }
 
-__device__ __forceinline__ unsigned smem_u32(const void* p) { return (unsigned)__cvta_generic_to_shared(p); }
-__device__ __forceinline__ void tc_mbar_init(unsigned bar, unsigned count) {
-    asm volatile("mbarrier.init.shared::cta.b64 [%0], %1;\n" ::"r"(bar), "r"(count) : "memory");
-}
-__device__ __forceinline__ void tc_mbar_expect_tx(unsigned bar, unsigned bytes) {
-    asm volatile("mbarrier.arrive.expect_tx.shared::cta.b64 _, [%0], %1;\n" ::"r"(bar), "r"(bytes) : "memory");
-}
-__device__ __forceinline__ void tc_mbar_wait(unsigned bar, unsigned parity) {
-    asm volatile(
-        "{\n\t.reg .pred p;\n\t"
-        "WAIT_%=:\n\t"
-        "mbarrier.try_wait.parity.shared::cta.b64 p, [%0], %1;\n\t"
-        "@p bra DONE_%=;\n\t"
-        "bra WAIT_%=;\n\t"
-        "DONE_%=:\n\t}\n" ::"r"(bar), "r"(parity) : "memory");
-}
-__device__ __forceinline__ void tc_bulk_load(unsigned dst, const void* src, unsigned bytes, unsigned bar) {
-    asm volatile("cp.async.bulk.shared::cluster.global.mbarrier::complete_tx::bytes [%0], [%1], %2, [%3];\n"
-                 ::"r"(dst), "l"(src), "r"(bytes), "r"(bar) : "memory");
-}
 __device__ __forceinline__ unsigned long long umma_desc(unsigned smem_addr, int lbo = kLBO) {
     return (unsigned long long)((smem_addr >> 4) & 0x3fffu) | ((unsigned long long)((lbo >> 4) & 0x3fff) << 16) |
            ((unsigned long long)((kSBO >> 4) & 0x3fff) << 32) | (1ull << 46);
@@ -105,8 +85,8 @@
         asm volatile("tcgen05.relinquish_alloc_permit.cta_group::1.sync.aligned;\n" ::: "memory");
     }
     if (threadIdx.x == 32) {
-        tc_mbar_init(bar_load, 1);
-        tc_mbar_init(bar_mma, 1);
+        mbar_init(bar_load, 1);
+        mbar_init(bar_mma, 1);
         asm volatile("fence.mbarrier_init.release.cluster;\n" ::: "memory");
     }
     asm volatile("tcgen05.fence::before_thread_sync;\n" ::: "memory");
@@ -115,10 +95,10 @@
     const unsigned tmem = *tmem_slot;
 
     if (threadIdx.x == 0) {
-        tc_mbar_expect_tx(bar_load, 2u * kImageBytes);
-        tc_bulk_load(smem_u32(sA), imgA + (size_t)tile_m * kImageBytes, kImageBytes, bar_load);
-        tc_bulk_load(smem_u32(sB), imgB + (size_t)tile_n * kImageBytes, kImageBytes, bar_load);
-        tc_mbar_wait(bar_load, 0);
+        mbar_expect_tx(bar_load, 2u * kImageBytes);
+        bulk_load(smem_u32(sA), imgA + (size_t)tile_m * kImageBytes, kImageBytes, bar_load);
+        bulk_load(smem_u32(sB), imgB + (size_t)tile_n * kImageBytes, kImageBytes, bar_load);
+        mbar_wait(bar_load, 0);
         asm volatile("tcgen05.fence::after_thread_sync;\n" ::: "memory");
         const int pa[6] = {2, 0, 1, 1, 0, 0}, pb[6] = {0, 2, 1, 0, 1, 0};
         unsigned accumulate = 0;
@@ -139,7 +119,7 @@
         asm volatile("tcgen05.commit.cta_group::1.mbarrier::arrive::one.shared::cluster.b64 [%0];\n" ::"r"(bar_mma) : "memory");
     }
     __syncwarp();
-    tc_mbar_wait(bar_mma, 0);
+    mbar_wait(bar_mma, 0);
     asm volatile("tcgen05.fence::after_thread_sync;\n" ::: "memory");
 
     const int m = tile_m * (kRows / kTrackRows) + warp;
@@ -221,10 +201,6 @@
 constexpr int kWalkSmem = kImageBytes + 2 * kWalkImageBytes + kWalkScratch + 96;
 constexpr unsigned kIdescWalk = (1u << 4) | (1u << 7) | (1u << 10) | ((unsigned)(kWalkCols >> 3) << 17) | ((unsigned)(kRows >> 4) << 24);
 
-__device__ __forceinline__ void tc_mbar_arrive(unsigned bar) {
-    asm volatile("mbarrier.arrive.shared::cta.b64 _, [%0];\n" ::"r"(bar) : "memory");
-}
-
 __global__ void __launch_bounds__(kWalkThreads, 1)
 app_tc_walk_kernel(const unsigned char* __restrict__ imgA, const unsigned char* __restrict__ imgB,
                    const int32_t* __restrict__ bank_len, int has_fallback, int M, int N, int T, int topk, int topk_mean,
@@ -249,11 +225,11 @@
         asm volatile("tcgen05.relinquish_alloc_permit.cta_group::1.sync.aligned;\n" ::: "memory");
     }
     if (tid == 32) {
-        tc_mbar_init(bar0, 1);
-        tc_mbar_init(bar0 + 8, 1); tc_mbar_init(bar0 + 16, 1);
-        tc_mbar_init(bar0 + 24, 1); tc_mbar_init(bar0 + 32, 1);
-        tc_mbar_init(bar0 + 40, kWalkEpiWarps); tc_mbar_init(bar0 + 48, kWalkEpiWarps);
-        tc_mbar_init(bar0 + 56, nrank); tc_mbar_init(bar0 + 64, nrank);
+        mbar_init(bar0, 1);
+        mbar_init(bar0 + 8, 1); mbar_init(bar0 + 16, 1);
+        mbar_init(bar0 + 24, 1); mbar_init(bar0 + 32, 1);
+        mbar_init(bar0 + 40, kWalkEpiWarps); mbar_init(bar0 + 48, kWalkEpiWarps);
+        mbar_init(bar0 + 56, nrank); mbar_init(bar0 + 64, nrank);
         asm volatile("fence.mbarrier_init.release.cluster;\n" ::: "memory");
     }
     asm volatile("tcgen05.fence::before_thread_sync;\n" ::: "memory");
@@ -269,7 +245,7 @@
         auto load_b = [&](int step) {
             const int buf = step & 1;
             const int tile_n = (first_tile + step) % n_steps;
-            tc_mbar_expect_tx(bar0 + 8 + 8 * buf, (unsigned)kWalkImageBytes);
+            mbar_expect_tx(bar0 + 8 + 8 * buf, (unsigned)kWalkImageBytes);
             if (nrank > 1) {
                 const unsigned part = (unsigned)kWalkImageBytes / nrank;
                 const unsigned dst = smem_u32(sB + buf * kWalkImageBytes) + rank * part;
@@ -277,24 +253,24 @@
                 asm volatile("cp.async.bulk.shared::cluster.global.mbarrier::complete_tx::bytes.multicast::cluster [%0], [%1], %2, [%3], %4;\n"
                              ::"r"(dst), "l"(src), "r"(part), "r"(bar0 + 8 + 8 * buf), "h"(cta_mask) : "memory");
             } else {
-                tc_bulk_load(smem_u32(sB + buf * kWalkImageBytes), imgB + (size_t)tile_n * kWalkImageBytes, kWalkImageBytes,
+                bulk_load(smem_u32(sB + buf * kWalkImageBytes), imgB + (size_t)tile_n * kWalkImageBytes, kWalkImageBytes,
                              bar0 + 8 + 8 * buf);
             }
         };
         if (leader) {
-            tc_mbar_expect_tx(bar0, (unsigned)kImageBytes);
-            tc_bulk_load(smem_u32(sA), imgA + (size_t)tile_m * kImageBytes, kImageBytes, bar0);
+            mbar_expect_tx(bar0, (unsigned)kImageBytes);
+            bulk_load(smem_u32(sA), imgA + (size_t)tile_m * kImageBytes, kImageBytes, bar0);
             load_b(0);
             if (n_steps > 1) load_b(1);
         }
         __syncwarp();
-        tc_mbar_wait(bar0, 0);
+        mbar_wait(bar0, 0);
         const unsigned long long dA = umma_desc(smem_u32(sA));
         for (int step = 0; step < n_steps; ++step) {
             const int buf = step & 1;
             const unsigned use = (unsigned)((step >> 1) & 1);
-            if (step >= 2) tc_mbar_wait(bar0 + 40 + 8 * buf, use ^ 1u);
-            tc_mbar_wait(bar0 + 8 + 8 * buf, use);
+            if (step >= 2) mbar_wait(bar0 + 40 + 8 * buf, use ^ 1u);
+            mbar_wait(bar0 + 8 + 8 * buf, use);
             asm volatile("tcgen05.fence::after_thread_sync;\n" ::: "memory");
             const int pa[6] = {2, 0, 1, 1, 0, 0}, pb[6] = {0, 2, 1, 0, 1, 0};
             const unsigned acc = tm + (unsigned)(buf * kWalkCols);
@@ -323,8 +299,8 @@
             }
             __syncwarp();
             if (step >= 1 && step + 1 < n_steps) {
-                if (nrank > 1) tc_mbar_wait(bar0 + 56 + 8 * (buf ^ 1), (unsigned)(((step - 1) >> 1) & 1));
-                else tc_mbar_wait(bar0 + 24 + 8 * (buf ^ 1), (unsigned)(((step - 1) >> 1) & 1));
+                if (nrank > 1) mbar_wait(bar0 + 56 + 8 * (buf ^ 1), (unsigned)(((step - 1) >> 1) & 1));
+                else mbar_wait(bar0 + 24 + 8 * (buf ^ 1), (unsigned)(((step - 1) >> 1) & 1));
                 if (leader) load_b(step + 1);
                 __syncwarp();
             }
@@ -342,7 +318,7 @@
         float* tile = scratch + warp * (32 * 33);
         for (int step = 0; step < n_steps; ++step) {
             const int buf = step & 1;
-            tc_mbar_wait(bar0 + 24 + 8 * buf, (unsigned)((step >> 1) & 1));
+            mbar_wait(bar0 + 24 + 8 * buf, (unsigned)((step >> 1) & 1));
             asm volatile("tcgen05.fence::after_thread_sync;\n" ::: "memory");
             unsigned r[32];
             const unsigned taddr = tmem + ((unsigned)(q * 32) << 16) + (unsigned)(buf * kWalkCols + half * 32);
@@ -359,7 +335,7 @@
             asm volatile("tcgen05.wait::ld.sync.aligned;\n" ::: "memory");
             asm volatile("tcgen05.fence::before_thread_sync;\n" ::: "memory");
             __syncwarp();
-            if (lane == 0) tc_mbar_arrive(bar0 + 40 + 8 * buf);
+            if (lane == 0) mbar_arrive(bar0 + 40 + 8 * buf);
 #pragma unroll
             for (int j = 0; j < 32; ++j) tile[lane * 33 + j] = __uint_as_float(r[j]);
             __syncwarp();
diff --git a/a-lightweight-unsupervised-feature-extractor-_b200/csrc/common.cuh b/a-lightweight-unsupervised-feature-extractor-_b200/csrc/common.cuh
--- a/a-lightweight-unsupervised-feature-extractor-_b200/csrc/common.cuh
+++ b/a-lightweight-unsupervised-feature-extractor-_b200/csrc/common.cuh
@@ -55,6 +55,29 @@
     return v;
 }
 
+__device__ __forceinline__ unsigned smem_u32(const void* p) { return (unsigned)__cvta_generic_to_shared(p); }
+__device__ __forceinline__ void mbar_init(unsigned bar, unsigned count) {
+    asm volatile("mbarrier.init.shared::cta.b64 [%0], %1;\n" ::"r"(bar), "r"(count) : "memory");
+}
+__device__ __forceinline__ void mbar_expect_tx(unsigned bar, unsigned bytes) {
+    asm volatile("mbarrier.arrive.expect_tx.shared::cta.b64 _, [%0], %1;\n" ::"r"(bar), "r"(bytes) : "memory");
+}
+__device__ __forceinline__ void mbar_arrive(unsigned bar) {
+    asm volatile("mbarrier.arrive.shared::cta.b64 _, [%0];\n" ::"r"(bar) : "memory");
+}
+__device__ __forceinline__ void mbar_wait(unsigned bar, unsigned parity) {
+    asm volatile(
+        "{\n\t.reg .pred p;\n\t"
+        "WAIT_%=:\n\t"
+        "mbarrier.try_wait.parity.shared::cta.b64 p, [%0], %1;\n\t"
+        "@p bra DONE_%=;\n\t"
+        "bra WAIT_%=;\n\t"
+        "DONE_%=:\n\t}\n" ::"r"(bar), "r"(parity) : "memory");
+}
+__device__ __forceinline__ void bulk_load(unsigned dst, const void* src, unsigned bytes, unsigned bar) {
+    asm volatile("cp.async.bulk.shared::cluster.global.mbarrier::complete_tx::bytes [%0], [%1], %2, [%3];\n"
+                 ::"r"(dst), "l"(src), "r"(bytes), "r"(bar) : "memory");
+}
 
 #ifdef B200_TRK_TIMING
 static __device__ unsigned long long g_span[128];
diff --git a/a-lightweight-unsupervised-feature-extractor-_b200/csrc/kalman.cuh b/a-lightweight-unsupervised-feature-extractor-_b200/csrc/kalman.cuh
--- a/a-lightweight-unsupervised-feature-extractor-_b200/csrc/kalman.cuh
+++ b/a-lightweight-unsupervised-feature-extractor-_b200/csrc/kalman.cuh
@@ -31,26 +31,65 @@
     for (int i = 0; i < 4; ++i) { P[i * 9] = 10.0; P[(i + 4) * 9] = 1000.0; }
 }
 
+template <typename TP>
+__device__ __forceinline__ void predict_elem(double& a, double& b, double& c, double& dd, bool diag, float qa, float qd) {
+    const TP a1 = (TP)a + (TP)c, b1 = (TP)b + (TP)dd;
+    const TP a2 = a1 + b1, c2 = (TP)c + (TP)dd;
+    a = diag ? (double)(a2 + (TP)qa) : (double)a2;
+    b = (double)b1;
+    c = (double)c2;
+    if (diag) dd = (double)((TP)dd + (TP)qd);
+}
+
+template <typename TX>
+__device__ __forceinline__ void predict_x_t(double* x) {
+#pragma unroll
+    for (int i = 0; i < 4; ++i) x[i] = (double)((TX)x[i] + (TX)x[i + 4]);
+}
+
 template <typename TX, typename TP>
 __device__ __forceinline__ void predict_t(double* x, double* P, const float* q) {
-#pragma unroll
-    for (int i = 0; i < 4; ++i) x[i] = (double)((TX)x[i] + (TX)x[i + 4]);
-#pragma unroll
-    for (int i = 0; i < 4; ++i)
-#pragma unroll
-        for (int j = 0; j < 8; ++j) P[i * 8 + j] = (double)((TP)P[i * 8 + j] + (TP)P[(i + 4) * 8 + j]);
-#pragma unroll
-    for (int i = 0; i < 8; ++i)
-#pragma unroll
-        for (int j = 0; j < 4; ++j) P[i * 8 + j] = (double)((TP)P[i * 8 + j] + (TP)P[i * 8 + j + 4]);
-#pragma unroll
-    for (int i = 0; i < 8; ++i) P[i * 9] = (double)((TP)P[i * 9] + (TP)q[i]);
+    predict_x_t<TX>(x);
+#pragma unroll
+    for (int i = 0; i < 4; ++i)
+#pragma unroll
+        for (int j = 0; j < 4; ++j)
+            predict_elem<TP>(P[i * 8 + j], P[i * 8 + j + 4], P[(i + 4) * 8 + j], P[(i + 4) * 8 + j + 4], i == j, q[i], q[i + 4]);
 }
 
 __device__ __forceinline__ void predict(double* x, double* P, int stage, const float* q) {
     if (stage == 0) predict_t<float, float>(x, P, q);
     else if (stage == 1) predict_t<float, double>(x, P, q);
     else predict_t<double, double>(x, P, q);
+}
+
+template <typename TX, typename TP>
+__device__ __forceinline__ void predict_global_t(double* gx, double* gP, const float* q, double* x, double* P) {
+    double2* vx = reinterpret_cast<double2*>(gx);
+    double2* vP = reinterpret_cast<double2*>(gP);
+#pragma unroll
+    for (int k = 0; k < 4; ++k) { const double2 v = vx[k]; x[2 * k] = v.x; x[2 * k + 1] = v.y; }
+    predict_x_t<TX>(x);
+#pragma unroll
+    for (int k = 0; k < 2; ++k) vx[k] = make_double2(x[2 * k], x[2 * k + 1]);
+#pragma unroll
+    for (int i = 0; i < 4; ++i)
+#pragma unroll
+        for (int j = 0; j < 4; j += 2) {
+            double2 a = vP[(i * 8 + j) / 2], b = vP[(i * 8 + j + 4) / 2];
+            double2 c = vP[((i + 4) * 8 + j) / 2], e = vP[((i + 4) * 8 + j + 4) / 2];
+            predict_elem<TP>(a.x, b.x, c.x, e.x, i == j, q[i], q[i + 4]);
+            predict_elem<TP>(a.y, b.y, c.y, e.y, i == j + 1, q[i], q[i + 4]);
+            vP[(i * 8 + j) / 2] = a; vP[(i * 8 + j + 4) / 2] = b;
+            vP[((i + 4) * 8 + j) / 2] = c; vP[((i + 4) * 8 + j + 4) / 2] = e;
+            P[i * 8 + j] = a.x; P[i * 8 + j + 1] = a.y;
+        }
+}
+
+__device__ __forceinline__ void predict_global(double* gx, double* gP, int stage, const float* q, double* x, double* P) {
+    if (stage == 0) predict_global_t<float, float>(gx, gP, q, x, P);
+    else if (stage == 1) predict_global_t<float, double>(gx, gP, q, x, P);
+    else predict_global_t<double, double>(gx, gP, q, x, P);
 }
 
 template <typename T>
diff --git a/a-lightweight-unsupervised-feature-extractor-_b200/csrc/roi_align.cu b/a-lightweight-unsupervised-feature-extractor-_b200/csrc/roi_align.cu
--- a/a-lightweight-unsupervised-feature-extractor-_b200/csrc/roi_align.cu
+++ b/a-lightweight-unsupervised-feature-extractor-_b200/csrc/roi_align.cu
@@ -747,21 +747,6 @@
     static_assert(kTabBytes % 16 == 0 && kOffOut % 16 == 0 && kOffBar % 8 == 0, "bulk-copy alignment");
 };
 
-__device__ __forceinline__ void mbar_init(unsigned bar, unsigned count) {
-    asm volatile("mbarrier.init.shared::cta.b64 [%0], %1;\n" ::"r"(bar), "r"(count) : "memory");
-}
-__device__ __forceinline__ void mbar_expect_tx(unsigned bar, unsigned bytes) {
-    asm volatile("mbarrier.arrive.expect_tx.shared::cta.b64 _, [%0], %1;\n" ::"r"(bar), "r"(bytes) : "memory");
-}
-__device__ __forceinline__ void mbar_wait(unsigned bar, unsigned parity) {
-    asm volatile(
-        "{\n\t.reg .pred p;\n\t"
-        "WAIT_%=:\n\t"
-        "mbarrier.try_wait.parity.shared::cta.b64 p, [%0], %1;\n\t"
-        "@p bra DONE_%=;\n\t"
-        "bra WAIT_%=;\n\t"
-        "DONE_%=:\n\t}\n" ::"r"(bar), "r"(parity) : "memory");
-}
 __device__ __forceinline__ void tma_box_4d(unsigned dst, const CUtensorMap* tm, int x, int y, int c, int b, unsigned bar) {
 #if B200_ROI_L2_HINT >= 2
     asm volatile("cp.async.bulk.tensor.4d.shared::cluster.global.tile.mbarrier::complete_tx::bytes.L2::cache_hint [%0], [%1, {%2, %3, %4, %5}], [%6], %7;\n"
@@ -770,10 +755,6 @@
     asm volatile("cp.async.bulk.tensor.4d.shared::cluster.global.tile.mbarrier::complete_tx::bytes [%0], [%1, {%2, %3, %4, %5}], [%6];\n"
                  ::"r"(dst), "l"(tm), "r"(x), "r"(y), "r"(c), "r"(b), "r"(bar) : "memory");
 #endif
-}
-__device__ __forceinline__ void bulk_load(unsigned dst, const void* src, unsigned bytes, unsigned bar) {
-    asm volatile("cp.async.bulk.shared::cluster.global.mbarrier::complete_tx::bytes [%0], [%1], %2, [%3];\n"
-                 ::"r"(dst), "l"(src), "r"(bytes), "r"(bar) : "memory");
 }
 
 __device__ __forceinline__ int tma_tile_rows(const int4 h0, const int4 h1) {
diff --git a/a-lightweight-unsupervised-feature-extractor-_b200/csrc/tracker.cu b/a-lightweight-unsupervised-feature-extractor-_b200/csrc/tracker.cu
--- a/a-lightweight-unsupervised-feature-extractor-_b200/csrc/tracker.cu
+++ b/a-lightweight-unsupervised-feature-extractor-_b200/csrc/tracker.cu
@@ -59,6 +59,7 @@
     double maha_thr, cost_max, conf_update_min, cost_update_max, reid_only_cost_max, init_conf_min;
     float ema_a, ema_b;
     int topk, max_age, lost_reid_after;
+    int front_bufs;
     const int* n_det;
     const double *boxes, *confs;
     const float* embs;
@@ -93,14 +94,6 @@
     return base;
 }
 
-__device__ __forceinline__ void load_kf(const Dev& d, size_t slot, double* x, double* P) {
-    const double2* px = reinterpret_cast<const double2*>(d.kf_x + slot * 8);
-    const double2* pP = reinterpret_cast<const double2*>(d.kf_P + slot * 64);
-#pragma unroll
-    for (int k = 0; k < 4; ++k) { const double2 v = px[k]; x[2 * k] = v.x; x[2 * k + 1] = v.y; }
-#pragma unroll
-    for (int k = 0; k < 32; ++k) { const double2 v = pP[k]; P[2 * k] = v.x; P[2 * k + 1] = v.y; }
-}
 __device__ __forceinline__ void store_kf(const Dev& d, size_t slot, const double* x, const double* P) {
     double2* px = reinterpret_cast<double2*>(d.kf_x + slot * 8);
     double2* pP = reinterpret_cast<double2*>(d.kf_P + slot * 64);
@@ -137,15 +130,15 @@
     for (int i = threadIdx.x; i < total; i += blockDim.x) work[base + i] = make_int2(s, (i / tiles) * 64 + i % tiles);
 }
 
-__device__ inline void prep_detections(const Dev& d, int s, int n, int part = 0, int nparts = 1) {
+__device__ inline void prep_detections(const Dev& d, int s, int n) {
     const size_t db = (size_t)s * d.MD;
     const int tid = threadIdx.x;
     const int nw = blockDim.x >> 5, nt = blockDim.x;
-    for (int j = part * nw + (tid >> 5); j < n; j += nparts * nw) {
+    for (int j = tid >> 5; j < n; j += nw) {
         const float4 v = reinterpret_cast<const float4*>(d.embs + (db + j) * cost::kD)[tid & 31];
         reinterpret_cast<float4*>(d.det_unit + (db + j) * cost::kD)[tid & 31] = cost::unit_row(v);
     }
-    for (int j = part * nt + tid; j < n; j += nparts * nt) {
+    for (int j = tid; j < n; j += nt) {
         double b[4];
         float z[4];
 #pragma unroll
@@ -158,22 +151,37 @@
     }
 }
 
-__device__ inline void predict_slot(const Dev& d, size_t slot) {
+struct RowRec {
+    double SI[16], xs[4];
+    float pb[4], pconf;
+    int stage, slot, T;
+    unsigned alive[8];
+    int any;
+};
+
+__device__ inline void predict_slot(const Dev& d, size_t slot, RowRec* rec = nullptr) {
     const float q[8] = {1.f, 1.f, 1.f, 1.f, 100.f, 100.f, 100.f, 100.f};
     const float rdiag[4] = {1.f, 1.f, 1.f, 1.f};
     double x[8], P[64], b[4];
-    load_kf(d, slot, x, P);
     const int st = d.kf_stage[slot];
-    kf::predict(x, P, st, q);
-    store_kf(d, slot, x, P);
+    kf::predict_global(d.kf_x + slot * 8, d.kf_P + slot * 64, st, q, x, P);
     kf::x_to_box(x, b);
+    const float pconf = (float)d.last_conf[slot];
 #pragma unroll
     for (int k = 0; k < 4; ++k) { d.last_bbox[slot * 4 + k] = b[k]; d.prev_boxf[slot * 4 + k] = (float)b[k]; }
-    d.prev_conff[slot] = (float)d.last_conf[slot];
+    d.prev_conff[slot] = pconf;
     kf::Gate g;
     kf::gate_prepare(x, P, st, rdiag, &g);
 #pragma unroll
     for (int k = 0; k < 16; ++k) d.gate_SI[slot * 16 + k] = g.SI[k];
+    if (rec) {
+#pragma unroll
+        for (int k = 0; k < 16; ++k) rec->SI[k] = g.SI[k];
+#pragma unroll
+        for (int k = 0; k < 4; ++k) { rec->xs[k] = x[k]; rec->pb[k] = (float)b[k]; }
+        rec->pconf = pconf;
+        rec->stage = st;
+    }
 }
 
 __global__ void __launch_bounds__(kThreads) begin_kernel(Dev d) {
@@ -420,7 +428,20 @@
     }
 }
 
-template <bool FLY>
+__device__ __forceinline__ float topk_cost(float sim, int kk) {
+    const float kNegInf = -__int_as_float(0x7f800000);
+    const int lane = threadIdx.x & 31;
+    float sum = 0.0f;
+    for (int q = 0; q < kk; ++q) {
+        const unsigned m = __reduce_max_sync(0xffffffffu, fkey(sim));
+        const unsigned who = __ballot_sync(0xffffffffu, fkey(sim) == m);
+        if (lane == __ffs(who) - 1) sim = kNegInf;
+        const unsigned bits = m ^ ((m >> 31) ? 0x80000000u : 0xffffffffu);
+        sum = __fadd_rn(sum, __uint_as_float(bits));
+    }
+    return __fsub_rn(1.0f, __fdiv_rn(sum, (float)kk));
+}
+
 __device__ __forceinline__ void cost1_row32(const Dev& d, int s, int r, size_t slot, int N, int lane) {
     const float kNegInf = -__int_as_float(0x7f800000);
     const size_t sb = (size_t)s * d.MT, db = (size_t)s * d.MD;
@@ -445,28 +466,11 @@
     for (int j0 = 0; j0 < N; j0 += 32) {
         const int j = j0 + lane;
         bool alive = false;
-        float zl[4], bf[4];
-        float cf = 0.0f;
-        if (j < N) {
-            if (FLY) {
-                double b[4];
-#pragma unroll
-                for (int k = 0; k < 4; ++k) { b[k] = d.boxes[(db + j) * 4 + k]; bf[k] = (float)b[k]; }
-                kf::box_to_z(b, zl);
-                cf = (float)d.confs[db + j];
-                alive = !(kf::gate_d2(SI, xs, stage, zl) > d.maha_thr);
-            } else {
-                alive = !(kf::gate_d2(SI, xs, stage, d.det_z + (db + j) * 4) > d.maha_thr);
-            }
-        }
+        if (j < N) alive = !(kf::gate_d2(SI, xs, stage, d.det_z + (db + j) * 4) > d.maha_thr);
         unsigned todo = __ballot_sync(0xffffffffu, alive);
         float c_app = 0.0f;
         float4 dv_first = make_float4(0, 0, 0, 0);
-        if (todo) {
-            const int jf = __ffs(todo) - 1;
-            if (FLY) dv_first = reinterpret_cast<const float4*>(d.embs + (db + j0 + jf) * cost::kD)[lane];
-            else dv_first = reinterpret_cast<const float4*>(d.det_unit + (db + j0 + jf) * cost::kD)[lane];
-        }
+        if (todo) dv_first = reinterpret_cast<const float4*>(d.det_unit + (db + j0 + __ffs(todo) - 1) * cost::kD)[lane];
         if (todo && !have_bank) {
             float q[32];
 #pragma unroll
@@ -487,12 +491,8 @@
             const int jl = __ffs(todo) - 1;
             todo &= todo - 1;
             float4 dv = dv_first;
-            if (!first) {
-                if (FLY) dv = reinterpret_cast<const float4*>(d.embs + (db + j0 + jl) * cost::kD)[lane];
-                else dv = reinterpret_cast<const float4*>(d.det_unit + (db + j0 + jl) * cost::kD)[lane];
-            }
+            if (!first) dv = reinterpret_cast<const float4*>(d.det_unit + (db + j0 + jl) * cost::kD)[lane];
             first = false;
-            if (FLY) dv = cost::unit_row(dv);
             float p[32];
 #pragma unroll
             for (int t = 0; t < 32; ++t) {
@@ -501,24 +501,12 @@
                 p[t] = a;
             }
             transpose_reduce32(p);
-            float sim = lane < T ? p[0] * inv : kNegInf;
-            float sum = 0.0f;
-            for (int q = 0; q < kk; ++q) {
-                const unsigned m = __reduce_max_sync(0xffffffffu, fkey(sim));
-                const unsigned who = __ballot_sync(0xffffffffu, fkey(sim) == m);
-                if (lane == __ffs(who) - 1) sim = kNegInf;
-                const unsigned bits = m ^ ((m >> 31) ? 0x80000000u : 0xffffffffu);
-                sum = __fadd_rn(sum, __uint_as_float(bits));
-            }
-            const float ca = __fsub_rn(1.0f, __fdiv_rn(sum, (float)kk));
+            const float ca = topk_cost(lane < T ? p[0] * inv : kNegInf, kk);
             if (lane == jl) c_app = ca;
         }
         if (j < N) {
             float total_c = 1e9f;
-            if (alive) {
-                if (FLY) total_c = cost::pair_cost(pb, bf, pconf, cf, d.pw, c_app).total;
-                else total_c = cost::pair_cost(pb, d.det_boxf + (db + j) * 4, pconf, d.det_conff[db + j], d.pw, c_app).total;
-            }
+            if (alive) total_c = cost::pair_cost(pb, d.det_boxf + (db + j) * 4, pconf, d.det_conff[db + j], d.pw, c_app).total;
             d.C1[(sb + r) * d.MD + j] = total_c;
             d.C1T[(db + j) * d.MT + r] = total_c;
             rmin.see(total_c, j);
@@ -536,7 +524,7 @@
         const int2 item = d.work1[wi];
         const int s = item.x, r = item.y >> 6;
         const size_t sb = (size_t)s * d.MT;
-        cost1_row32<false>(d, s, r, sb + d.rows_main[sb + r], d.n_det[s], lane);
+        cost1_row32(d, s, r, sb + d.rows_main[sb + r], d.n_det[s], lane);
     }
 }
 
@@ -841,21 +829,97 @@
     assign_body<STAGE, false, false>(d, blockIdx.x, smem_raw, smem_matrix_floats);
 }
 
-#ifndef B200_TRK_FRONT_WARPS
-#define B200_TRK_FRONT_WARPS 4
+constexpr int kFrontWarps = 4;
+constexpr int kFrontThreads = (kFrontWarps + 1) * 32;
+#ifndef B200_TRK_FRONT_ROWS
+#define B200_TRK_FRONT_ROWS 128
 #endif
-constexpr int kFrontWarps = B200_TRK_FRONT_WARPS;
-
-__global__ void __launch_bounds__(kFrontWarps * 32, 2) front_kernel(Dev d) {
+#ifndef B200_TRK_FRONT_BUFS
+#define B200_TRK_FRONT_BUFS 8
+#endif
+constexpr int kFrontRows = B200_TRK_FRONT_ROWS;
+constexpr int kFrontMaxBufs = B200_TRK_FRONT_BUFS;
+constexpr size_t kFrontSmemMax = 226 * 1024;
+
+struct FrontLayout {
+    size_t bank, emb, box, z, conf, rec, rows, list, bar, total;
+    __host__ __device__ FrontLayout(int MT, int MD, int HIST, int nbuf) {
+        const int nrec = MT < kFrontRows ? MT : kFrontRows;
+        bank = 0;
+        emb = bank + (size_t)nbuf * HIST * cost::kD * sizeof(float);
+        box = emb + (size_t)MD * cost::kD * sizeof(float);
+        z = box + (size_t)MD * 4 * sizeof(float);
+        conf = z + (size_t)MD * 4 * sizeof(float);
+        rec = (conf + (size_t)MD * sizeof(float) + 15) & ~(size_t)15;
+        rows = rec + (size_t)nrec * sizeof(RowRec);
+        list = rows + (size_t)2 * MT * sizeof(int);
+        bar = (list + (size_t)nrec * sizeof(int) + 7) & ~(size_t)7;
+        total = bar + (size_t)(1 + 2 * nbuf) * 8;
+    }
+};
+
+__device__ __forceinline__ void cost1_row_staged(const Dev& d, int s, int r, const RowRec& rc, int N, const float4* bank,
+                                                 const float4* emb, const float* box, const float* conf, int lane) {
+    const float kNegInf = -__int_as_float(0x7f800000);
+    const size_t sb = (size_t)s * d.MT, db = (size_t)s * d.MD;
+    const int T = rc.T > 0 ? rc.T : 1;
+    const int kk = min(d.topk, T);
+    float inv = 0.0f;
+    if (rc.any) {
+        float q[32];
+#pragma unroll
+        for (int t = 0; t < 32; ++t) {
+            const float4 v = t < T ? bank[t * 32 + lane] : make_float4(0, 0, 0, 0);
+            float a = v.x * v.x;
+            a = fmaf(v.y, v.y, a); a = fmaf(v.z, v.z, a); a = fmaf(v.w, v.w, a);
+            q[t] = a;
+        }
+        transpose_reduce32(q);
+        inv = __fdiv_rn(1.0f, __fadd_rn(sqrtf(q[0]), 1e-12f));
+    }
+    RowMin rmin;
+    for (int j0 = 0; j0 < N; j0 += 32) {
+        const int j = j0 + lane;
+        unsigned todo = rc.alive[j0 >> 5];
+        const bool alive = (todo >> lane) & 1u;
+        float c_app = 0.0f;
+        while (todo) {
+            const int jl = __ffs(todo) - 1;
+            todo &= todo - 1;
+            const float4 dv = emb[(j0 + jl) * 32 + lane];
+            float p[32];
+#pragma unroll
+            for (int t = 0; t < 32; ++t) {
+                const float4 v = t < T ? bank[t * 32 + lane] : make_float4(0, 0, 0, 0);
+                float a = v.x * dv.x;
+                a = fmaf(v.y, dv.y, a); a = fmaf(v.z, dv.z, a); a = fmaf(v.w, dv.w, a);
+                p[t] = a;
+            }
+            transpose_reduce32(p);
+            const float ca = topk_cost(lane < T ? p[0] * inv : kNegInf, kk);
+            if (lane == jl) c_app = ca;
+        }
+        if (j < N) {
+            float total_c = 1e9f;
+            if (alive) total_c = cost::pair_cost(rc.pb, box + j * 4, rc.pconf, conf[j], d.pw, c_app).total;
+            d.C1[(sb + r) * d.MD + j] = total_c;
+            d.C1T[(db + j) * d.MT + r] = total_c;
+            rmin.see(total_c, j);
+        }
+    }
+    rmin.finish(d.row_fc + sb + r, d.row_fv + sb + r, lane);
+}
+
+__global__ void __maxnreg__(128) front_kernel(Dev d) {
     Span span((d.frame_id[0] & 7) * 6 + 0);
-    extern __shared__ __align__(16) int s_rows[];
+    extern __shared__ __align__(16) unsigned char fsm[];
     __shared__ int scratch[kThreads / 32];
     const int s = blockIdx.y, g = blockIdx.x, G = gridDim.x, tid = threadIdx.x, warp = tid >> 5, lane = tid & 31;
     TRK_GSTAMP(0);
     int* hdr = d.hdr + s * kHdr;
     int* cnt = d.cnt + s * kHdr;
     int* res = d.result + (size_t)s * d.res_stride;
-    const size_t sb = (size_t)s * d.MT;
+    const size_t sb = (size_t)s * d.MT, db = (size_t)s * d.MD;
     const int n = d.n_det[s], nl = hdr[H_NLIVE];
     const int* order = d.order + sb;
     if (s == 0 && g == 0 && tid == 0) d.wcount[2] = 0;
@@ -886,8 +950,27 @@
         }
         return;
     }
-    int* rm = s_rows;
-    int* rr = s_rows + d.MT;
+    const int nbuf = d.front_bufs;
+    const FrontLayout L(d.MT, d.MD, d.HIST, nbuf);
+    const size_t bank_floats = (size_t)d.HIST * cost::kD;
+    float* sBank = reinterpret_cast<float*>(fsm + L.bank);
+    float* sEmb = reinterpret_cast<float*>(fsm + L.emb);
+    float* sBox = reinterpret_cast<float*>(fsm + L.box);
+    float* sZ = reinterpret_cast<float*>(fsm + L.z);
+    float* sConf = reinterpret_cast<float*>(fsm + L.conf);
+    RowRec* rec = reinterpret_cast<RowRec*>(fsm + L.rec);
+    int* rm = reinterpret_cast<int*>(fsm + L.rows);
+    int* rr = rm + d.MT;
+    int* list = reinterpret_cast<int*>(fsm + L.list);
+    const unsigned bar_emb = smem_u32(fsm + L.bar), bar_full = bar_emb + 8, bar_empty = bar_full + 8 * nbuf;
+    if (tid == 0) {
+        mbar_init(bar_emb, 1);
+        for (int b = 0; b < nbuf; ++b) { mbar_init(bar_full + 8 * b, 1); mbar_init(bar_empty + 8 * b, 1); }
+        asm volatile("fence.mbarrier_init.release.cluster;\n" ::: "memory");
+        const unsigned bytes = (unsigned)n * cost::kD * sizeof(float);
+        mbar_expect_tx(bar_emb, bytes);
+        bulk_load(smem_u32(sEmb), d.embs + db * cost::kD, bytes, bar_emb);
+    }
     const int M1 = block_compact(nl, [&](int i) { return d.miss[sb + order[i]] <= d.lost_reid_after; },
                                  [&](int pos, int i) { rm[pos] = order[i]; }, scratch);
     const int M2 = block_compact(nl, [&](int i) { return d.miss[sb + order[i]] > d.lost_reid_after; },
@@ -901,15 +984,94 @@
         }
     }
     TRK_GSTAMP(1);
-    prep_detections(d, s, n, g, G);
+    for (int j = tid; j < n; j += blockDim.x) {
+        double b[4];
+        float z[4];
+#pragma unroll
+        for (int k = 0; k < 4; ++k) b[k] = d.boxes[(db + j) * 4 + k];
+        kf::box_to_z(b, z);
+        const float cf = (float)d.confs[db + j];
+        const float4 bf = make_float4((float)b[0], (float)b[1], (float)b[2], (float)b[3]), zf = make_float4(z[0], z[1], z[2], z[3]);
+        reinterpret_cast<float4*>(sBox)[j] = bf;
+        reinterpret_cast<float4*>(sZ)[j] = zf;
+        sConf[j] = cf;
+        if (j % G == g) {
+            reinterpret_cast<float4*>(d.det_boxf + db * 4)[j] = bf;
+            reinterpret_cast<float4*>(d.det_z + db * 4)[j] = zf;
+            d.det_conff[db + j] = cf;
+            d.det_used[db + j] = 0;
+        }
+    }
     const int own1 = M1 > g ? (M1 - g + G - 1) / G : 0, own2 = M2 > g ? (M2 - g + G - 1) / G : 0;
-    for (int i = tid; i < own1 + own2; i += blockDim.x)
-        predict_slot(d, sb + (i < own1 ? rm[g + i * G] : rr[g + (i - own1) * G]));
+    for (int i = tid; i < own1 + own2; i += blockDim.x) {
+        if (i < own1) {
+            const size_t slot = sb + rm[g + i * G];
+            predict_slot(d, slot, &rec[i]);
+            rec[i].slot = (int)slot;
+            rec[i].T = d.bank_len[slot];
+        } else {
+            predict_slot(d, sb + rr[g + (i - own1) * G]);
+        }
+    }
     __syncthreads();
     TRK_GSTAMP(2);
-    for (int i = warp; i < own1; i += kFrontWarps) {
-        const int r = g + i * G;
-        cost1_row32<true>(d, s, r, sb + rm[r], n, lane);
+    for (int i = warp; i < own1; i += kFrontWarps + 1) {
+        RowRec& rc = rec[i];
+        double SI[16], xs[4];
+#pragma unroll
+        for (int k = 0; k < 16; ++k) SI[k] = rc.SI[k];
+#pragma unroll
+        for (int k = 0; k < 4; ++k) xs[k] = rc.xs[k];
+        const int stage = rc.stage;
+        unsigned any = 0;
+        for (int j0 = 0; j0 < n; j0 += 32) {
+            const int j = j0 + lane;
+            const bool alive = j < n && !(kf::gate_d2(SI, xs, stage, sZ + j * 4) > d.maha_thr);
+            const unsigned m = __ballot_sync(0xffffffffu, alive);
+            if (lane == 0) rc.alive[j0 >> 5] = m;
+            any |= m;
+        }
+        if (lane == 0) rc.any = any != 0;
+    }
+    __syncthreads();
+    const int nsurv = block_compact(own1, [&](int i) { return rec[i].any != 0; }, [&](int pos, int i) { list[pos] = i; },
+                                    scratch);
+    if (warp == kFrontWarps) {
+        if (lane == 0) {
+            for (int k = 0, b = 0, use = 0; k < nsurv; ++k, b = b + 1 == nbuf ? 0 : b + 1, use += b == 0) {
+                if (use > 0) mbar_wait(bar_empty + 8 * b, (unsigned)(use - 1) & 1u);
+                asm volatile("fence.proxy.async.shared::cta;\n" ::: "memory");
+                const RowRec& rc = rec[list[k]];
+                const float* src = rc.T > 0 ? d.bank + (size_t)rc.slot * bank_floats : d.ema + (size_t)rc.slot * cost::kD;
+                const unsigned bytes = (unsigned)(rc.T > 0 ? rc.T : 1) * cost::kD * sizeof(float);
+                mbar_expect_tx(bar_full + 8 * b, bytes);
+                bulk_load(smem_u32(sBank + b * bank_floats), src, bytes, bar_full + 8 * b);
+            }
+        }
+    } else {
+        mbar_wait(bar_emb, 0);
+        for (int j = warp; j < n; j += kFrontWarps) {
+            float4* e = reinterpret_cast<float4*>(sEmb + (size_t)j * cost::kD) + lane;
+            const float4 u = cost::unit_row(*e);
+            *e = u;
+            if (j % G == g) reinterpret_cast<float4*>(d.det_unit + (db + j) * cost::kD)[lane] = u;
+        }
+        asm volatile("bar.sync 1, %0;" ::"r"(kFrontWarps * 32) : "memory");
+        const float4* emb = reinterpret_cast<const float4*>(sEmb);
+        for (int i = warp; i < own1; i += kFrontWarps)
+            if (!rec[i].any) cost1_row_staged(d, s, g + i * G, rec[i], n, nullptr, emb, sBox, sConf, lane);
+        int b = warp % nbuf;
+        unsigned par = (unsigned)(warp / nbuf) & 1u;
+        for (int k = warp; k < nsurv; k += kFrontWarps) {
+            const int i = list[k];
+            mbar_wait(bar_full + 8 * b, par);
+            cost1_row_staged(d, s, g + i * G, rec[i], n, reinterpret_cast<const float4*>(sBank + b * bank_floats), emb,
+                             sBox, sConf, lane);
+            __syncwarp();
+            if (lane == 0) mbar_arrive(bar_empty + 8 * b);
+            for (int step = 0; step < kFrontWarps; ++step)
+                if (++b == nbuf) { b = 0; par ^= 1u; }
+        }
     }
     TRK_GSTAMP(3);
 }
@@ -1126,7 +1288,7 @@
     size_t assign_smem = 0;
     int smem_matrix_floats = 0;
     int chain = 6;
-    int front_resident = 0;
+    int front_ctas = 0;
     size_t front_smem = 0, back_smem = 0;
 };
 
@@ -1191,6 +1353,10 @@
         return fail(B200_ECUDA, "tracker_create: cudaMalloc(%zu bytes): %s", c.off, cudaGetErrorString(e));
     }
     char* base = static_cast<char*>(t->arena);
+    if (reinterpret_cast<uintptr_t>(base) % 16 != 0) {
+        b200_tracker_destroy(t);
+        return fail(B200_ECUDA, "tracker_create: device allocation not 16 B-aligned");
+    }
     cudaMemset(base, 0, c.off);
 #define PTR(field, T) d.field = reinterpret_cast<T*>(base + o_##field)
     PTR(kf_x, double); PTR(kf_P, double); PTR(last_bbox, double); PTR(last_conf, double); PTR(last_cost, double);
@@ -1275,17 +1441,23 @@
             if (want == 6 || (fits && (want == 2 || want == 3))) t->chain = want;
         }
         if (t->chain != 6) {
-            t->front_smem = sizeof(int) * 2 * (size_t)max_tracks;
             size_t bs = t->assign_smem;
             if (cost::smem_bytes(d.HIST) > bs) bs = cost::smem_bytes(d.HIST);
             if (sizeof(double) * (trk::kThreads / 32) * 4 * 96 > bs) bs = sizeof(double) * (trk::kThreads / 32) * 4 * 96;
             t->back_smem = bs;
             cudaFuncSetAttribute(trk::back_kernel<true>, cudaFuncAttributeMaxDynamicSharedMemorySize, (int)budget);
             cudaFuncSetAttribute(trk::back_kernel<false>, cudaFuncAttributeMaxDynamicSharedMemorySize, (int)budget);
+            const size_t fixed = trk::FrontLayout(max_tracks, max_dets, d.HIST, 0).total;
+            const size_t per_buf = trk::FrontLayout(max_tracks, max_dets, d.HIST, 1).total - fixed;
+            int nbuf = (int)((trk::kFrontSmemMax - fixed) / per_buf);
+            d.front_bufs = nbuf < trk::kFrontMaxBufs ? nbuf : trk::kFrontMaxBufs;
+            t->front_smem = trk::FrontLayout(max_tracks, max_dets, d.HIST, d.front_bufs).total;
+            cudaFuncSetAttribute(trk::front_kernel, cudaFuncAttributeMaxDynamicSharedMemorySize, (int)trk::kFrontSmemMax);
             per_sm = 1;
-            cudaOccupancyMaxActiveBlocksPerMultiprocessor(&per_sm, trk::front_kernel, trk::kFrontWarps * 32, t->front_smem);
-            t->front_resident = sms * (per_sm > 0 ? per_sm : 1);
-            if (const char* e = getenv("B200TRACK_FRONT_CTAS")) t->front_resident = atoi(e) > 0 ? atoi(e) : t->front_resident;
+            cudaOccupancyMaxActiveBlocksPerMultiprocessor(&per_sm, trk::front_kernel, trk::kFrontThreads, t->front_smem);
+            const int gmin = (max_tracks + trk::kFrontRows - 1) / trk::kFrontRows, gmax = (max_tracks + 3) / 4;
+            int G = sms * (per_sm > 0 ? per_sm : 1) / n_streams;
+            t->front_ctas = G < gmin ? gmin : G > gmax ? gmax : G;
             if (const char* e = getenv("B200TRACK_UPD_CTAS")) t->upd_grid = atoi(e) > 0 ? atoi(e) : t->upd_grid;
         }
     }
@@ -1346,10 +1518,7 @@
     const int cost_grid = t->cost_grid;
     int rc;
     if (t->chain != 6) {
-        int G = t->front_resident / d.S;
-        const int gmax = (d.MT + 3) / 4;
-        G = G < 1 ? 1 : G > gmax ? gmax : G;
-        trk::front_kernel<<<dim3(G, d.S), trk::kFrontWarps * 32, t->front_smem, st>>>(d);
+        trk::front_kernel<<<dim3(t->front_ctas, d.S), trk::kFrontThreads, t->front_smem, st>>>(d);
         if ((rc = check_launch("trk front_kernel"))) return rc;
         if (t->chain == 3) {
             trk::back_kernel<false><<<d.S, trk::kThreads, t->assign_smem > cost::smem_bytes(d.HIST) ? t->assign_smem
```

Result: slower. 249,300, median of 6 (-8.0%).
